# zsc/MOSS-TTSD

Hardware: AMD Instinct MI355X
Metric: audio codec tokens/sec/node (decode, bf16, batch 32 @ 4k ctx) (higher is better)
Workload: dtype bf16; 1 GPU; configs[2]: batch 32 synthetic dialogues/GPU, 4k-token KV context, top-k/top-p sampling on 8 channels, decode steps at full context; batch_per_gpu=32, context=4096, prompt=512, layers=28, hidden=2048, parallelism=dp1 (batch shard, no per-step collective)

## Files before the change

### include/mtts.h

```cpp
#ifndef MTTS_H
#define MTTS_H

#include <stdint.h>

#ifdef __cplusplus
extern "C" {
#endif

#define MTTS_OK 0
#define MTTS_EINVAL (-1)
#define MTTS_EHIP (-2)
#define MTTS_ENOMEM (-3)
#define MTTS_ESTATE (-4)

#define MTTS_CHANNELS 8

typedef struct MttsConfig {
    int32_t vocab_size;
    int32_t hidden_size;
    int32_t intermediate_size;
    int32_t num_hidden_layers;
    int32_t num_attention_heads;
    int32_t num_key_value_heads;
    int32_t head_dim;
// ... 17 lines not shown
typedef struct MttsSamplerCfg {
    int32_t do_sample;
    int32_t top_k;
    float top_p;
    float one_minus_top_p;
    float temperature;
    float repetition_penalty;
} MttsSamplerCfg;

typedef struct MttsEngine MttsEngine;

const char* mtts_last_error(void);
int32_t mtts_version(void);

int32_t mtts_engine_create(const MttsConfig* cfg, int32_t device, MttsEngine** out);
int32_t mtts_engine_destroy(MttsEngine* e);

int32_t mtts_bind_weight(MttsEngine* e, const char* name, const void* dev_bf16,
                         int64_t rows, int64_t cols, void* stream);
int32_t mtts_bind_weight_lora(MttsEngine* e, const char* name, const void* dev_base, int64_t rows, int64_t cols,
                              const float* dev_lora_a, const float* dev_lora_b, int32_t r, float scaling, void* stream);
#define MTTS_MAX_ADAPTERS 16
#define MTTS_LORA_MAX_RANK 64
int32_t mtts_adapter_load(MttsEngine* e, int32_t adapter, const char* name, const float* dev_lora_a, const float* dev_lora_b,
                          int64_t rows, int64_t cols, int32_t r, float scaling, void* stream);
int32_t mtts_adapter_clear(MttsEngine* e, int32_t adapter);
int32_t mtts_set_row_adapters(MttsEngine* e, const int32_t* host_ids, int32_t n);
int32_t mtts_set_slot_adapter(MttsEngine* e, int32_t slot, int32_t adapter);
int32_t mtts_bind_rope(MttsEngine* e, const void* dev_cos_bf16, const void* dev_sin_bf16,
                       int32_t rows, void* stream);
int32_t mtts_weights_ready(MttsEngine* e);

int32_t mtts_generate(MttsEngine* e, const int64_t* host_input_ids, const uint8_t* host_attention_mask,
                      int32_t B, int32_t T, int32_t max_length,
                      const MttsSamplerCfg* sampler, uint64_t seed,
                      int64_t* host_out_ids, int32_t out_capacity, int32_t* out_len,
                      const int64_t* host_forced, int32_t forced_len, int64_t* host_decisions,
                      void* stream);

int32_t mtts_begin(MttsEngine* e, const int64_t* host_input_ids, const uint8_t* host_attention_mask,
                   int32_t B, int32_t T, int32_t max_length,
                   const MttsSamplerCfg* sampler, uint64_t seed, void* stream);
int32_t mtts_step(MttsEngine* e, int32_t n_steps, void* stream);
int32_t mtts_sync_state(MttsEngine* e, int32_t* steps_done, int32_t* all_finished, void* stream);
int32_t mtts_read_generated(MttsEngine* e, int64_t* host_gen, int32_t capacity_steps, int32_t* n_steps);
int32_t mtts_set_output_scores(MttsEngine* e, int32_t on);
int32_t mtts_read_scores(MttsEngine* e, float* host_lp, int32_t capacity_steps, int32_t* n_steps);
int32_t mtts_slot_read_scores(MttsEngine* e, int32_t slot, float* host_rows, int32_t capacity_steps, int32_t* n_steps);
int32_t mtts_score(MttsEngine* e, const int64_t* host_input_ids, const uint8_t* host_attention_mask,
                   const int64_t* host_labels, int32_t B, int32_t T, float* host_logp, void* stream);
#define MTTS_SCORE_MAX_TOPK 16
#define MTTS_SCORE_TOPK_ROWS 512
int32_t mtts_score_topk(MttsEngine* e, const int64_t* host_input_ids, const uint8_t* host_attention_mask,
                        const int64_t* host_labels, int32_t B, int32_t T, float* host_logp, int32_t k,
                        int32_t* host_top_ids, float* host_top_logp, void* stream);
int32_t mtts_read_logits(MttsEngine* e, uint16_t* host_logits0, uint16_t* host_logits17, void* stream);
int32_t mtts_read_logits_f32(MttsEngine* e, float* host_logits0, float* host_logits17, void* stream);
int32_t mtts_sched_open(MttsEngine* e, int32_t B, int32_t gen_cap, const MttsSamplerCfg* sampler, void* stream);
int32_t mtts_slot_submit(MttsEngine* e, int32_t slot, const int64_t* host_ids, int32_t T, int32_t max_length, uint64_t seed,
                         void* stream);
int32_t mtts_slot_submit_row(MttsEngine* e, int32_t slot, const int64_t* host_ids, int32_t T, int32_t max_length, uint64_t seed,
                             int32_t row_id, void* stream);
int32_t mtts_set_row_ids(MttsEngine* e, const int32_t* host_row_ids, int32_t n);
int32_t mtts_set_takes(MttsEngine* e, int32_t n);
int32_t mtts_slot_fork(MttsEngine* e, int32_t src_slot, int32_t dst_slot, uint64_t seed, int32_t row_id, void* stream);
int32_t mtts_slot_states(MttsEngine* e, int32_t* host_state, void* stream);
int32_t mtts_slot_read(MttsEngine* e, int32_t slot, int64_t* host_rows, int32_t capacity_steps, int32_t* n_steps);
int32_t mtts_read_seq_state(MttsEngine* e, int32_t* host_nas, int32_t* host_unfinished, int32_t* host_kv_len, void* stream);
int32_t mtts_slot_evict(MttsEngine* e, int32_t slot, void* stream);
int32_t mtts_kv_pool_state(MttsEngine* e, int32_t* total_pages, int32_t* free_pages, int32_t* max_pages_per_seq);
int32_t mtts_read_page_table(MttsEngine* e, int32_t* host_table, int32_t* host_n_pages);
int32_t mtts_set_forced_mode(MttsEngine* e, int32_t as_draw);
int32_t mtts_debug_read_device_page_table(MttsEngine* e, int32_t* host_table, void* stream);
int32_t mtts_export_codes(MttsEngine* e, int32_t first, int32_t n, int64_t* dev_codes, void* stream);
int32_t mtts_profile_enable(MttsEngine* e, int32_t on);
int32_t mtts_profile_read(MttsEngine* e, int32_t which, double* total_ms, int64_t* launches, int64_t* bytes);

int32_t mtts_debug_set_kv_len(MttsEngine* e, int32_t kv_len);
int32_t mtts_debug_kv_pack_stats(MttsEngine* e, int64_t* out6);
int32_t mtts_k_attn_bench(MttsEngine* e, int32_t phase, int32_t iters, float* avg_ms, int64_t* bytes_per_launch);
int32_t mtts_k_gemm_bench(int32_t N, int32_t K, int32_t epi, int32_t ksplit, int32_t waves, int32_t copies,
                          int32_t iters, float* avg_us);

int32_t mtts_k_gemm_bf16(const void* dev_w, const void* dev_x, void* dev_y,
                         int32_t M, int32_t N, int32_t K, int32_t ksplit, void* stream);
int64_t mtts_debug_gemm_depth_launches(void);
int64_t mtts_debug_attn_row_launches(void);
int32_t mtts_k_attn_section(const float* dev_slabs, int32_t ksplit, const void* dev_qnw, const void* dev_knw, const void* dev_cos,
                            const void* dev_sin, float eps, const void* dev_k, const void* dev_v, const int32_t* host_lens,
                            const int32_t* host_page_table, int32_t R, int32_t Lmax, int32_t nq, int32_t nkv, int32_t sealed,
                            int32_t path, void* dev_out, void* dev_kcache, void* dev_vcache, void* dev_kpack, void* dev_vpack,
                            void* stream);
int32_t mtts_k_attn_prefill(const float* dev_slabs, int32_t ksplit, const void* dev_qnw, const void* dev_knw, const void* dev_cos,
                            const void* dev_sin, float eps, const void* dev_k, const void* dev_v, const int32_t* host_lens,
                            const int32_t* host_cached, const int32_t* host_page_table, int32_t B, int32_t Lmax, int32_t nq,
                            int32_t nkv, void* dev_out, void* dev_q, void* dev_kcache, void* dev_vcache, void* stream);
int32_t mtts_k_gemm_swiglu_bf16(const void* dev_w, const void* dev_x, void* dev_y,
                                int32_t M, int32_t N, int32_t K, void* stream);
int32_t mtts_k_rmsnorm(const void* dev_x, const void* dev_w, void* dev_y,
                       int32_t rows, int32_t n, float eps, void* stream);
int32_t mtts_k_embed_norm(const int32_t* host_tokens, const int32_t* host_seq, const void* const* host_tables,
                          const int32_t* host_vocab, const void* dev_norm_w, int32_t R, int32_t H, float eps,
                          void* dev_x, void* dev_xn, void* stream);
int32_t mtts_k_resid_norm(const float* dev_slabs, int32_t ksplit, int32_t Npad, void* dev_x, const void* dev_norm_w,
                          const int32_t* host_seq, const int32_t* host_last, int32_t R, int32_t H, int32_t nseq, float eps,
                          void* dev_xn, void* dev_hlast, void* stream);
int32_t mtts_k_gemv_small(int32_t epi, int32_t pro, const void* dev_w, int32_t rows, int32_t N, int32_t K, int32_t want_ksplit,
                          const void* dev_x_in, const float* dev_slabs, int32_t slab_ksplit, const void* dev_norm_w, float eps,
                          void* dev_x_out, const float* dev_opart, const int32_t* host_seq, const int32_t* host_pos, int32_t nq,
                          int32_t nchunks_max, const void* dev_xrows, void* dev_y, int32_t* out_plan, void* stream);
int32_t mtts_k_gemm_tile(int32_t epi, const void* dev_w, const void* dev_x, void* dev_y, int32_t M, int32_t N, int32_t K,
                         int32_t ksplit, void* stream);
int32_t mtts_k_rope_kvwrite(const void* dev_qkv, const int32_t* host_pos, const void* dev_qnorm, const void* dev_knorm,
                            const void* dev_cos, const void* dev_sin, int32_t R, int32_t nq, int32_t nkv, float eps,
                            void* dev_q, void* dev_k, void* dev_v, void* stream);
int32_t mtts_k_paged_attn_decode(const void* dev_q, const void* dev_k, const void* dev_v, const int32_t* host_lens,
                                 const int32_t* host_page_table, int32_t R, int32_t Lmax, int32_t nq, int32_t nkv,
                                 void* dev_out, void* stream);
int32_t mtts_k_kv_seal(const void* dev_pages, int32_t npages, void* dev_sealed, int32_t as_k, void* stream);
int32_t mtts_k_head_ce(const void* dev_w, const void* dev_x, const int32_t* host_labels, int32_t M, int32_t N, int32_t K,
                       int32_t n_valid, int32_t segments, float* dev_logp, void* stream);
int32_t mtts_k_head_topk(const void* dev_w, const void* dev_x, int32_t M, int32_t N, int32_t K, int32_t n_valid,
                         int32_t segments, int32_t k, int32_t* dev_ids, float* dev_logp, void* stream);
int32_t mtts_k_lora_pack(const void* dev_base, int32_t rows, int32_t cols, const float* dev_lora_a, const float* dev_lora_b,
                         int32_t r, float scaling, int32_t rows_pad, int32_t row_mul, int32_t row_off, int32_t dtype,
                         void* dev_out, void* stream);
int32_t mtts_k_lora_delta(const void* dev_x, int32_t R, int32_t K, int32_t Npad, int32_t nseg, const int32_t* host_segs,
                          int32_t n_adapters, const void* const* host_a, const void* const* host_b, const int32_t* host_r,
                          const float* host_scaling, const int32_t* host_row_adapter, float* dev_slabs, int32_t ks, void* stream);
int32_t mtts_k_swiglu_slabs(const void* dev_w, const void* dev_x, const float* dev_delta, void* dev_y, float* dev_slab0_out,
                            int32_t M, int32_t N, int32_t K, void* stream);
int32_t mtts_k_sample(const void* dev_logits_bf16, int32_t rows, int32_t vocab,
                      const void* dev_history_bitmap, const MttsSamplerCfg* cfg,
                      int32_t mask_id, uint64_t seed, int32_t step, int32_t channel,
                      int32_t* dev_tokens, void* stream);
int32_t mtts_k_sample_scores(const void* dev_logits_bf16, int32_t rows, int32_t vocab,
                             const void* dev_history_bitmap, const MttsSamplerCfg* cfg,
                             int32_t mask_id, uint64_t seed, int32_t step, int32_t channel,
                             int32_t* dev_tokens, float* dev_logp, void* stream);

typedef struct MttsCodecConfig {
    int32_t nq, codebook_size, rvq_dim, quant_out_dim;
    int32_t adapter_layers, adapter_dim, adapter_heads, adapter_ffn, adapter_max_pos;
    int32_t up_stride;
    int32_t dec_layers, dec_dim, dec_heads, dec_ffn, dec_max_pos, mel_bins;
    int32_t voc_dim, voc_inter, voc_layers, n_fft, hop;
    int32_t mel_n_fft, mel_hop, mel_frames;
    int32_t enc_layers, enc_dim, enc_heads, enc_ffn, enc_max_pos;
    int32_t sem_adapter_layers, pre_rvq_layers, down_pool;
} MttsCodecConfig;

typedef struct MttsCodec MttsCodec;
const char* mtts_codec_last_error(void);
int32_t mtts_codec_create(const MttsCodecConfig* cfg, int32_t device, MttsCodec** out);
int32_t mtts_codec_destroy(MttsCodec* c);
int32_t mtts_codec_bind(MttsCodec* c, const char* role, const float* dev_f32, int64_t n, void* stream);
int32_t mtts_codec_detokenize(MttsCodec* c, const int64_t* dev_codes, const int32_t* host_lens, int32_t B, int32_t T,
                              float* dev_wav, void* stream);
int32_t mtts_codec_detokenize_async(MttsCodec* c, const int64_t* dev_codes, const int32_t* host_lens, int32_t B, int32_t T,
                                    float* dev_wav, void* stream);
int32_t mtts_codec_check(MttsCodec* c, void* stream);
int32_t mtts_codec_tokenize(MttsCodec* c, const float* dev_wav, const int32_t* host_lens, int32_t B, int32_t nsamp,
                            int64_t* dev_codes, int32_t* host_code_lens, void* stream);
int32_t mtts_k_gemm_f32(const float* dev_a, const float* dev_w, const float* dev_bias, float* dev_c,
                        int32_t M, int32_t N, int32_t K, int32_t act, void* stream);
int32_t mtts_k_gemm_planes_bench(int32_t M, int32_t N, int32_t K, int32_t flags, int32_t tile_code, int32_t iters,
// ... 7 lines not shown
```

### moss-ttsd_amd/build.py

```python
import os
import subprocess
import sys
from concurrent.futures import ThreadPoolExecutor

HERE = os.path.dirname(os.path.abspath(__file__))
SRC = ["gemm.hip", "layer.hip", "attn.hip", "sampler.hip", "f32path.hip", "score.hip", "adapter.hip", "multilora.hip", "engine.hip", "hooks.hip", "codec.hip", "codec_fused.hip"]
OUT = os.path.join(HERE, "lib", "libmtts.so")
OBJ = os.path.join(HERE, "build")
FLAGS = ["--offload-arch=gfx950", "-O3", "-std=c++17", "-fPIC", "-fno-gpu-rdc", "-Wno-unused-result", "-Wno-unused-value"]
FLAGS += os.environ.get("MTTS_BUILD_FLAGS", "").split()


def _newer(target, deps):
    return os.path.exists(target) and all(os.path.getmtime(target) >= os.path.getmtime(d) for d in deps)


def build(force=False, verbose=True):
    srcs = [os.path.join(HERE, "csrc", s) for s in SRC if os.path.exists(os.path.join(HERE, "csrc", s))]
    hdrs = [os.path.join(HERE, "csrc", "common.h"), os.path.join(HERE, "..", "include", "mtts.h")]
    hdrs += [os.path.join(HERE, "csrc", h) for h in os.listdir(os.path.join(HERE, "csrc")) if h.endswith(".h") and h != "common.h"]
    if not force and _newer(OUT, srcs + hdrs):
        return OUT
    os.makedirs(os.path.dirname(OUT), exist_ok=True)
    os.makedirs(OBJ, exist_ok=True)
    objs, jobs = [], []
    for s in srcs:
        o = os.path.join(OBJ, os.path.basename(s) + ".o")
        objs.append(o)
        if force or not _newer(o, [s] + hdrs):
            jobs.append(["hipcc"] + FLAGS + ["-c", s, "-o", o])

    def run(cmd):
        if verbose:
            print(" ".join(cmd), flush=True)
        subprocess.check_call(cmd)

    with ThreadPoolExecutor(max_workers=min(6, max(1, len(jobs)))) as ex:
        list(ex.map(run, jobs))
    run(["hipcc", "--offload-arch=gfx950", "-shared", "-fPIC", "-fno-gpu-rdc", "-o", OUT] + objs)
    return OUT


if __name__ == "__main__":
    build(force="--force" in sys.argv)
```

### moss-ttsd_amd/csrc/attn.hip

```cpp
#include "launch.h"
#include <algorithm>
#include <atomic>
#include <cstdlib>
#ifndef MTTS_PK_WAVES
#define MTTS_PK_WAVES 0
#endif
#if MTTS_PK_WAVES
#define PK_OCC(PK) __attribute__((amdgpu_waves_per_eu((PK) ? MTTS_PK_WAVES : 1, (PK) ? MTTS_PK_WAVES : 8)))
#else
#define PK_OCC(PK)
#endif

__device__ __forceinline__ uint32_t u4c(const u32x4_t& v, int c) { return c == 0 ? v.x : c == 1 ? v.y : c == 2 ? v.z : v.w; }
__device__ __forceinline__ void pk_unit(const u32x4_t* pk, int j, uint32_t w[4]) {
    const uint32_t L0 = u4c(pk[j >> 1], 2 * (j & 1)), L1 = u4c(pk[j >> 1], 2 * (j & 1) + 1);
    const uint32_t N = u4c(pk[8 + (j >> 2)], j & 3);
    const uint32_t lo = pk[12].x, hi = pk[12].y;
    const uint32_t HA = ((N & 0x08080808u) << 4) | __builtin_amdgcn_perm(hi, lo, N & 0x07070707u);
    const uint32_t HB = (N & 0x80808080u) | __builtin_amdgcn_perm(hi, lo, (N >> 4) & 0x07070707u);
    w[0] = __builtin_amdgcn_perm(HA, L0, 0x05010400u);
    w[1] = __builtin_amdgcn_perm(HA, L0, 0x07030602u);
    w[2] = __builtin_amdgcn_perm(HB, L1, 0x05010400u);
    w[3] = __builtin_amdgcn_perm(HB, L1, 0x07030602u);
}

__host__ __device__ constexpr int pk_order(int i) { return i == 0 ? 12 : (i - 1) % 3 == 0 ? 8 + (i - 1) / 3 : 2 * ((i - 1) / 3) + (i - 1) % 3 - 1; }
__device__ bool seal_encode(const u32x4_t (&v)[16], u32x4_t* __restrict__ pk, uint32_t spare, bool unfit) {
    unsigned long long b0 = 0ull, b1 = 0ull;
#pragma unroll
    for (int j = 0; j < 16; ++j)
#pragma unroll
        for (int c = 0; c < 4; ++c)
#pragma unroll
            for (int h = 0; h < 2; ++h) {
                const uint32_t e = (u4c(v[j], c) >> (8 + 16 * h)) & 0x7fu;
                if (e & 64u) b1 |= 1ull << (e & 63u);
                else b0 |= 1ull << e;
            }
    const int n0 = __popcll(b0), n = n0 + __popcll(b1);
    if (n > 8 || unfit) {
        pk[12 * 64] = u32x4_t{0u, 0u, spare, 1u};
        return false;
    }
    unsigned long long dict = 0ull;
    {
        unsigned long long t0 = b0, t1 = b1;
        for (int i = 0; i < n; ++i) {
            uint32_t e;
            if (t0) { e = __ffsll((long long)t0) - 1; t0 &= t0 - 1; }
            else { e = 64 + __ffsll((long long)t1) - 1; t1 &= t1 - 1; }
            dict |= (unsigned long long)e << (8 * i);
        }
    }
    auto code = [&](uint32_t half) -> uint32_t {
        const uint32_t e = (half >> 8) & 0x7fu;
        const uint32_t rank = (e & 64u) ? n0 + __popcll(b1 & ((1ull << (e & 63u)) - 1ull)) : __popcll(b0 & ((1ull << e) - 1ull));
        return ((half >> 12) & 8u) | rank;
    };
    uint32_t lowp[32], nib[16];
#pragma unroll
    for (int j = 0; j < 16; ++j) {
        uint32_t N = 0u;
#pragma unroll
        for (int g = 0; g < 2; ++g) {
            uint32_t L = 0u;
#pragma unroll
            for (int k = 0; k < 4; ++k) {
                const uint32_t half = (u4c(v[j], 2 * g + (k >> 1)) >> (16 * (k & 1))) & 0xffffu;
                L |= (half & 0xffu) << (8 * k);
                N |= code(half) << (8 * k + 4 * g);
            }
            lowp[2 * j + g] = L;
        }
        nib[j] = N;
    }
#pragma unroll
    for (int u = 0; u < 8; ++u) pk[u * 64] = u32x4_t{lowp[4 * u], lowp[4 * u + 1], lowp[4 * u + 2], lowp[4 * u + 3]};
#pragma unroll
    for (int u = 0; u < 4; ++u) pk[(8 + u) * 64] = u32x4_t{nib[4 * u], nib[4 * u + 1], nib[4 * u + 2], nib[4 * u + 3]};
    pk[12 * 64] = u32x4_t{(uint32_t)dict, (uint32_t)(dict >> 32), spare, 0u};
    return true;
}
__device__ bool seal_lane(const u32x4_t* __restrict__ raw, u32x4_t* __restrict__ pk) {
    u32x4_t v[16];
#pragma unroll
    for (int j = 0; j < 16; ++j) v[j] = raw[j * 64];
    return seal_encode(v, pk, 0u, false);
}
__device__ bool seal_lane_k(const u32x4_t* __restrict__ raw, u32x4_t* __restrict__ pk, uint8_t* __restrict__ lds, int lane) {
    u32x4_t v[16];
#pragma unroll
    for (int j = 0; j < 16; ++j) v[j] = raw[j * 64];
    __builtin_amdgcn_wave_barrier();
    uint32_t* row = (uint32_t*)(lds + lane * 128);
#pragma unroll
    for (int j = 0; j < 16; ++j)
#pragma unroll
        for (int c = 0; c < 4; c += 2) {
            const uint32_t a = u4c(v[j], c), b = u4c(v[j], c + 1);
            row[2 * j + (c >> 1)] = ((a >> 7) & 0xffu) | (((a >> 23) & 0xffu) << 8) | (((b >> 7) & 0xffu) << 16) | (((b >> 23) & 0xffu) << 24);
        }
    __builtin_amdgcn_wave_barrier();
    uint32_t a0 = 0u, a1 = 0u, n0 = 0u, n1 = 0u;
    for (int t = 0; t < 64; ++t) {
        const uint32_t e = *(const uint16_t*)(lds + t * 128 + 2 * lane);
        a0 += e & 0xffu; n0 += (e & 0xffu) ? 1u : 0u;
        a1 += e >> 8; n1 += (e >> 8) ? 1u : 0u;
    }
    const int s0 = n0 ? min(max((int)((a0 + n0 / 2) / n0) - 125, -127), 127) : 0;
    const int s1 = n1 ? min(max((int)((a1 + n1 / 2) / n1) - 125, -127), 127) : 0;
    int8_t* sv = (int8_t*)(lds + 8192);
    sv[2 * lane] = (int8_t)s0;
    sv[2 * lane + 1] = (int8_t)s1;
    __builtin_amdgcn_wave_barrier();
    bool unfit = false;
#pragma unroll
    for (int j = 0; j < 16; ++j) {
        uint32_t w[4] = {v[j].x, v[j].y, v[j].z, v[j].w};
#pragma unroll
        for (int c = 0; c < 4; ++c) {
            const uint32_t sh = *(const uint16_t*)(sv + 8 * j + 2 * c);
            uint32_t out = 0u;
#pragma unroll
            for (int h = 0; h < 2; ++h) {
                uint32_t b = (w[c] >> (16 * h)) & 0xffffu;
                const int sft = (int)(int8_t)((sh >> (8 * h)) & 0xffu);
                const int e = (int)((b >> 7) & 0xffu);
                if (e == 0) {
                    if ((b & 0x7fu) && sft) unfit = true;
                } else {
                    const int e2 = e - sft;
                    if (e == 255 ? sft != 0 : (e2 < 1 || e2 > 254)) unfit = true;
                    else b = (b - ((uint32_t)sft << 7)) & 0xffffu;
                }
                out |= b << (16 * h);
            }
            w[c] = out;
        }
        v[j] = u32x4_t{w[0], w[1], w[2], w[3]};
    }
    return seal_encode(v, pk, ((uint32_t)s0 & 0xffu) | (((uint32_t)s1 & 0xffu) << 8), unfit);
}
__device__ bool seal_lane_v(const u32x4_t* __restrict__ raw, u32x4_t* __restrict__ pk, uint8_t* __restrict__ lds, int lane) {
    u32x4_t v[16];
#pragma unroll
    for (int j = 0; j < 16; ++j) v[j] = raw[j * 64];
    const int sub = lane >> 5;
    __builtin_amdgcn_wave_barrier();
    uint32_t* row = (uint32_t*)(lds + lane * 128);
#pragma unroll
    for (int it = 0; it < 16; ++it)
#pragma unroll
        for (int h = 0; h < 2; ++h) {
            uint32_t sum = 0u, cnt = 0u;
#pragma unroll
            for (int c = 0; c < 4; ++c) {
                const uint32_t e = (u4c(v[it], c) >> (7 + 16 * h)) & 0xffu;
                sum += e;
                cnt += e ? 1u : 0u;
            }
            row[2 * it + h] = sum | (cnt << 16);
        }
    __builtin_amdgcn_wave_barrier();
    int mean;
    {
        const int t = lane, st = (t >> 1) & 1, j = 2 * (t >> 2) + (t & 1);
        uint32_t tot = 0u, cn = 0u;
        for (int d = 0; d < 32; ++d) {
            const uint32_t w = ((const uint32_t*)(lds + (st * 32 + d) * 128))[j];
            tot += w & 0xffffu;
            cn += w >> 16;
// ... 1214 lines not shown
```

### moss-ttsd_amd/csrc/engine.h

```cpp
#pragma once
#include <hip/hip_runtime.h>

#include <algorithm>
#include <cstdarg>
#include <cstdio>
#include <cstdlib>
#include <cstring>
#include <memory>
#include <string>
#include <vector>

#include "launch.h"

#define MTTS_LOCAL __attribute__((visibility("hidden")))
extern MTTS_LOCAL thread_local char g_err[512];
#define HIPCHK(x)                                                                          \
    do {                                                                                   \
        hipError_t _e = (x);                                                               \
        if (_e != hipSuccess) return fail(MTTS_EHIP, "%s: %s (%s:%d)", #x, hipGetErrorString(_e), __FILE__, __LINE__); \
    } while (0)
#define TRY(x)             \
    do {                   \
        int _r = (x);      \
        if (_r) return _r; \
    } while (0)

static inline int round_up(int a, int b) { return (a + b - 1) / b * b; }
static inline hipStream_t S(void* s) { return (hipStream_t)s; }
static inline int gemm_depth_env() {
    const char* g = getenv("MTTS_GEMM_DEPTH");
    return (g && atoi(g) == 0) ? 0 : 1;
}

template <typename T>
static int dalloc(T** p, size_t n, bool zero = true) {
    HIPCHK(hipMalloc((void**)p, n * sizeof(T)));
    if (zero) HIPCHK(hipMemset(*p, 0, n * sizeof(T)));
    return 0;
}

struct DevBufs {
    struct Buf { void* p; bool pinned; };
    std::vector<Buf> bufs;
    std::string free_error;
    DevBufs() = default;
    DevBufs(const DevBufs&) = delete;
    DevBufs& operator=(const DevBufs&) = delete;
    ~DevBufs() { free_all(); }
    template <typename T>
    int get(T** out, size_t n, bool zero = true) {
        TRY(dalloc(out, n, zero));
        bufs.push_back({(void*)*out, false});
        return 0;
    }
    template <typename T>
    int get_pinned(T** out, size_t n) {
        HIPCHK(hipHostMalloc((void**)out, n * sizeof(T)));
        bufs.push_back({(void*)*out, true});
        memset((void*)*out, 0, n * sizeof(T));
        return 0;
    }
    template <typename T>
    void release(T*& p) {
        if (!p) return;
        auto it = std::find_if(bufs.begin(), bufs.end(), [&](const Buf& b) { return b.p == (void*)p; });
        if (it == bufs.end()) note(hipErrorInvalidValue, (void*)p);
        else { free_one(*it); bufs.erase(it); }
        p = nullptr;
    }
    void free_all() {
        for (const Buf& b : bufs) free_one(b);
        bufs.clear();
    }
private:
    void free_one(const Buf& b) {
        const hipError_t r = b.pinned ? hipHostFree(b.p) : hipFree(b.p);
        if (r != hipSuccess) note(r, b.p);
    }
    void note(hipError_t r, void* p) {
        if (!free_error.empty()) return;
        char msg[160];
        snprintf(msg, sizeof(msg), "freeing %p: %s", p, hipGetErrorString(r));
        free_error = msg;
    }
};

static inline int full_cap_for(int vocab) { int p = 1; while (p < vocab) p <<= 1; return vocab > SAMP_CAND ? p : 0; }
static inline int alloc_scratch(DevBufs& m, SampleScratch& sc, int rows, int vocab) {
    const int fc = full_cap_for(vocab);
    TRY(m.get(&sc.overflow, (size_t)rows));
    if (fc) {
        TRY(m.get(&sc.full_val, (size_t)rows * fc, false));
        TRY(m.get(&sc.full_idx, (size_t)rows * fc, false));
        TRY(m.get(&sc.nuc_cnt, (size_t)rows * 2048));
        TRY(m.get(&sc.nuc_mass, (size_t)rows * 2048));
    }
    TRY(m.get(&sc.hist, (size_t)rows * 2048));
    TRY(m.get(&sc.slice_val, (size_t)rows * SAMP_NS));
    TRY(m.get(&sc.slice_idx, (size_t)rows * SAMP_NS));
    TRY(m.get(&sc.cand_val, (size_t)rows * SAMP_CAND));
    TRY(m.get(&sc.cand_idx, (size_t)rows * SAMP_CAND));
    TRY(m.get(&sc.cand_n, (size_t)rows));
    return 0;
}
static inline int alloc_lp_scratch(DevBufs& m, SampleScratch& sc, int rows) {
    if (sc.lp) return 0;
    TRY(m.get(&sc.slice_sum, (size_t)rows * SAMP_NS));
    TRY(m.get(&sc.lp, (size_t)rows * 8));
    return 0;
}

struct Layer {
    void *wqkv = nullptr, *wo = nullptr, *wgu = nullptr, *wd = nullptr;
    void *ln_in = nullptr, *ln_post = nullptr, *qn = nullptr, *kn = nullptr;
    int bound = 0;
};

enum { PROF_SCORES = 0, PROF_PV = 1, PROF_GEMM = 2, PROF_STEP = 3,
       PROF_CE = 4,
       PROF_N = 5 };

struct MttsEngine {
    DevBufs mem;
    MttsConfig cfg;
    int device = 0;
    int H, I, L, nq, nkv, V0, Vs, Vs_pad, V0_pad, qkv_rows;
    std::vector<Layer> layers;
    void* emb[8] = {nullptr};
    void* head0 = nullptr;
    void* heads17 = nullptr;
    void* final_norm = nullptr;
    uint16_t *rope_cos = nullptr, *rope_sin = nullptr;
    int rope_rows = 0;
    int emb_bound = 0, norm_bound = 0;
    const uint16_t** d_tables = nullptr;
    GemmPlan p_qkv, p_o, p_gu, p_d, p_h0, p_h17;
    float* partial = nullptr;
    float* partial2 = nullptr;
    void *x2 = nullptr, *act_rm = nullptr;
    int small_rows = SMALL_RP;
    int gemm_depth = 1;
    void *x = nullptr, *xn = nullptr, *attn_p = nullptr, *act_p = nullptr, *qbuf = nullptr, *hlast = nullptr, *xh = nullptr;
    void *logits0 = nullptr, *logits17 = nullptr, *join_logits0 = nullptr, *join_logits17 = nullptr;
    void* scores = nullptr;
    float *stats = nullptr, *opart = nullptr;
    void *kcache = nullptr, *vcache = nullptr;
    size_t layer_stride = 0;
    int total_pages = 0, max_pages = 0, nchunks_max = 0;
    int32_t* d_page_table = nullptr;
    KvPool pool;
    std::vector<char> slot_live;
    int forced_draw = 0;
    std::vector<int32_t> next_row_ids;
    int next_takes = 1;
    int takes = 1;
    bool f32 = false;
    int h16 = 0;
    struct LayerF32 { float *wqkv = nullptr, *wo = nullptr, *wgu = nullptr, *wd = nullptr, *ln_in = nullptr, *ln_post = nullptr, *qn = nullptr, *kn = nullptr; };
    std::vector<LayerF32> lf;
    float* embf[8] = {nullptr};
    const float** d_tables_f = nullptr;
    float *final_norm_f = nullptr, *rope_cos_f = nullptr, *rope_sin_f = nullptr;
    float *kcache_f = nullptr, *vcache_f = nullptr;
    float *xf = nullptr, *xnf = nullptr, *qkvf = nullptr, *qbuf_f = nullptr, *attnf = nullptr, *yf = nullptr, *guf = nullptr,
          *actf = nullptr, *hlast_f = nullptr, *scores_f = nullptr;
    SeqState* d_seqs = nullptr;
    RowMeta* d_meta = nullptr;
    LoopState* d_ls = nullptr;
    LoopState* h_ls = nullptr;
    SeqState* h_seqs = nullptr;
    int32_t *d_decisions = nullptr, *d_cur = nullptr, *d_gen = nullptr, *d_declog = nullptr, *d_forced = nullptr,
            *d_tf = nullptr;
    uint32_t* d_bitmaps = nullptr;
    int bm_words = 0;
    MttsSamplerCfg* d_scfg = nullptr;
    SampleScratch sscr;
    int ch0_sampled = 0;
    float* d_lp = nullptr;
    int lp_cap = 0;
    int scores_next = 0;
    int scores_on = 0;
    bool run_open = false;
    int32_t* d_sc_labels = nullptr;
    float* d_sc_logp = nullptr;
    size_t sc_cap_rows = 0;
    float* sc_part = nullptr;
    float* sc_logits = nullptr;
    int32_t* d_sc_top_ids = nullptr;
    float* d_sc_top_logp = nullptr;
    size_t sc_top_cap = 0;
    uint32_t* sc_cand = nullptr;
    std::vector<LoraEnt> bank;
    LoraEnt* d_bank = nullptr;
    int bank_pairs[MTTS_MAX_ADAPTERS] = {0};
    int32_t* d_seq_adapter = nullptr;
    std::vector<int32_t> seq_adapter = std::vector<int32_t>(MTTS_RCAP, -1);
    std::vector<int32_t> next_slot_adapter = std::vector<int32_t>(MTTS_RCAP, -1);
    std::vector<int32_t> next_row_adapters;
    bool row_adapters_pending = false;
    int32_t* d_pf_tokens = nullptr;
    RowMeta* d_pf_meta = nullptr;
    size_t pf_cap_rows = 0;
    int gen_cap = 0;
    int B = 0, T = 0, base_length = 0, max_length = 0, max_steps = 0, steps_issued = 0;
    bool continuous = false;
    std::vector<int> join_step;
    std::vector<int> n_real;
    int max_real = 0;
    uint64_t seed = 0;
    bool began = false, has_forced = false;
    struct StepGraph { int B, pages, forced, ch0, scores, row, lora; hipGraphExec_t exec; };
    std::vector<StepGraph> graphs;
    hipStream_t cap_stream = nullptr;
    bool use_graphs = true;
    int kv_pack = 1;
    void *kpack = nullptr, *vpack = nullptr;
    size_t pk_layer_stride = 0;
    unsigned long long *d_seal_cnt = nullptr, *h_seal_cnt = nullptr;
    std::vector<char> pack_k_on, pack_v_on;
    int pack_min_work = 512;
    int fuse_qkv_max = 2560;
    int attn_row = 1;
    int n_cus = 0;
    int pf_mfma_pages = 0;
// ... 22 lines not shown
```

### moss-ttsd_amd/csrc/engine.hip

```cpp
#include "engine.h"
#include "staging.h"

#define FLUSH_STEPS 7
#define LINGER_STEPS 14
static inline int linger_bound(int B) { return 6 * B + 8; }

thread_local char g_err[512] = "";
int fail(int code, const char* fmt, ...) {
    va_list ap;
    va_start(ap, fmt);
    vsnprintf(g_err, sizeof(g_err), fmt, ap);
    va_end(ap);
    return code;
}

const char* mtts_last_error(void) { return g_err; }
int32_t mtts_version(void) { return 202; }

static auto ship_on(MttsEngine* e, hipStream_t st) {
    return [e, st](const PageEdits& ed) -> int {
        launch_set_pages(e->d_page_table, ed, st);
        HIPCHK(hipGetLastError());
        return 0;
    };
// ... 60 lines not shown

static void drop_graphs(MttsEngine* e) {
    for (auto& g : e->graphs) hipGraphExecDestroy(g.exec);
    e->graphs.clear();
}

int32_t mtts_engine_create(const MttsConfig* c, int32_t device, MttsEngine** out) {
    if (!c || !out) return fail(MTTS_EINVAL, "null argument");
    if (c->head_dim != MTTS_HD) return fail(MTTS_EINVAL, "head_dim must be 128 (got %d)", c->head_dim);
    if (c->channels != 8) return fail(MTTS_EINVAL, "channels must be 8");
    if (c->hidden_size % 16 || c->intermediate_size % 16) return fail(MTTS_EINVAL, "hidden/intermediate must be multiples of 16");
    if (c->hidden_size > 8192) return fail(MTTS_EINVAL, "hidden_size > 8192 not built (resid_norm keeps a row in registers)");
    if (c->num_attention_heads % c->num_key_value_heads) return fail(MTTS_EINVAL, "bad GQA ratio");
    int G = c->num_attention_heads / c->num_key_value_heads;
    if (G != 1 && G != 2 && G != 4) return fail(MTTS_EINVAL, "GQA group %d not built (1,2,4)", G);
    if (c->max_batch < 1 || c->max_batch > MTTS_RCAP) return fail(MTTS_EINVAL, "max_batch must be 1..128");
    if (c->vocab_size <= 152694 || c->speech_vocab_size <= 1024)
        return fail(MTTS_EINVAL, "vocab too small for the reference's hard-coded mask ids 152694 / 1024");
    if (c->dtype != MTTS_DTYPE_BF16 && c->dtype != MTTS_DTYPE_F32 && c->dtype != MTTS_DTYPE_F16)
        return fail(MTTS_EINVAL, "dtype %d not built (bf16 = 0, fp32 = 1, fp16 = 2)", c->dtype);
    if (c->kv_pool_pages < 0) return fail(MTTS_EINVAL, "kv_pool_pages must be >= 0");
    HIPCHK(hipSetDevice(device));
    struct Destroy {
        void operator()(MttsEngine* p) const {
            const std::string keep = g_err;
            mtts_engine_destroy(p);
            snprintf(g_err, sizeof(g_err), "%s", keep.c_str());
        }
    };
    std::unique_ptr<MttsEngine, Destroy> holder(new MttsEngine());
    MttsEngine* e = holder.get();
    DevBufs& m = e->mem;
    e->cfg = *c;
    e->device = device;
    if (const char* g = getenv("MTTS_GRAPHS")) e->use_graphs = atoi(g) != 0;
    if (const char* g = getenv("MTTS_FUSE_QKV_MAX")) e->fuse_qkv_max = atoi(g);
    if (const char* g = getenv("MTTS_KV_PACK")) e->kv_pack = atoi(g);
    if (const char* g = getenv("MTTS_KV_PACK_MIN")) e->pack_min_work = atoi(g);
    if (const char* g = getenv("MTTS_PREFILL_MFMA_PAGES")) e->pf_mfma_pages = atoi(g);
    if (const char* g = getenv("MTTS_ATTN_ROW")) e->attn_row = std::min(std::max(atoi(g), 0), 2);
    HIPCHK(hipDeviceGetAttribute(&e->n_cus, hipDeviceAttributeMultiprocessorCount, device));
    if (e->attn_row && attn_row_prepare()) {
        if (e->attn_row == 2) return fail(MTTS_EINVAL, "attn_row_kernel: the dynamic LDS limit could not be raised");
        e->attn_row = 0;
    }
    if (const char* g = getenv("MTTS_SMALL_ROWS")) e->small_rows = std::min(std::max(atoi(g), 0), SMALL_RP);
    e->gemm_depth = gemm_depth_env();
    e->H = c->hidden_size; e->I = c->intermediate_size; e->L = c->num_hidden_layers;
    e->nq = c->num_attention_heads; e->nkv = c->num_key_value_heads;
    e->V0 = c->vocab_size; e->Vs = c->speech_vocab_size;
    e->V0_pad = round_up(e->V0, 32); e->Vs_pad = round_up(e->Vs, 32);
    e->qkv_rows = (e->nq + 2 * e->nkv) * MTTS_HD;
    e->layers.resize(e->L);
    const int H = e->H, I = e->I;
    e->f32 = c->dtype != MTTS_DTYPE_BF16;
    e->h16 = c->dtype == MTTS_DTYPE_F16;
    if (e->f32) TRY(create_f32(e));
    if (!e->f32) {
        for (auto& l : e->layers) {
            TRY(m.get((uint16_t**)&l.wqkv, (size_t)e->qkv_rows * H));
            TRY(m.get((uint16_t**)&l.wo, (size_t)H * e->nq * MTTS_HD));
            TRY(m.get((uint16_t**)&l.wgu, (size_t)2 * I * H));
            TRY(m.get((uint16_t**)&l.wd, (size_t)round_up(H, 32) * I));
            TRY(m.get((uint16_t**)&l.ln_in, (size_t)H));
            TRY(m.get((uint16_t**)&l.ln_post, (size_t)H));
            TRY(m.get((uint16_t**)&l.qn, (size_t)MTTS_HD));
            TRY(m.get((uint16_t**)&l.kn, (size_t)MTTS_HD));
        }
        TRY(m.get((uint16_t**)&e->emb[0], (size_t)e->V0 * H, false));
        for (int ch = 1; ch < 8; ++ch) TRY(m.get((uint16_t**)&e->emb[ch], (size_t)e->Vs * H, false));
        TRY(m.get((uint16_t**)&e->head0, (size_t)e->V0_pad * H));
        TRY(m.get((uint16_t**)&e->heads17, (size_t)7 * e->Vs_pad * H));
        TRY(m.get((uint16_t**)&e->final_norm, (size_t)H));
        TRY(m.get(&e->d_tables, 8));
        HIPCHK(hipMemcpy((void*)e->d_tables, e->emb, 8 * sizeof(void*), hipMemcpyHostToDevice));
    }
    e->p_qkv = mtts_plan_gemm(e->qkv_rows, H, 0);
    e->p_o = mtts_plan_gemm(round_up(H, 32), e->nq * MTTS_HD, 0);
    e->p_gu = mtts_plan_gemm(2 * I, H, 1);
    e->p_d = mtts_plan_gemm(round_up(H, 32), I, 0);
    e->p_h0 = mtts_plan_gemm(e->V0_pad, H, 1);
    e->p_h17 = mtts_plan_gemm(7 * e->Vs_pad, H, 1);
    for (GemmPlan* p : {&e->p_qkv, &e->p_o, &e->p_gu, &e->p_d, &e->p_h0, &e->p_h17}) p->depth = e->gemm_depth;
    size_t pmax = (size_t)8 * std::max(e->qkv_rows, round_up(H, 32));
    if (!e->f32) {
        TRY(m.get(&e->partial, pmax * MTTS_PFCAP));
        TRY(m.get(&e->partial2, (size_t)8 * round_up(H, 32) * MTTS_PFCAP));
        TRY(m.get((uint16_t**)&e->x2, (size_t)MTTS_MAXR * H));
        TRY(m.get((uint16_t**)&e->act_rm, (size_t)MTTS_MAXR * I));
        TRY(m.get((uint16_t**)&e->x, (size_t)MTTS_PFCAP * H));
        TRY(m.get((uint16_t**)&e->xn, (size_t)MTTS_PFCAP * H));
        TRY(m.get((uint16_t**)&e->xh, (size_t)MTTS_RCAP * H));
        TRY(m.get((uint16_t**)&e->hlast, (size_t)MTTS_RCAP * H));
        TRY(m.get((uint16_t**)&e->attn_p, (size_t)MTTS_PFCAP * e->nq * MTTS_HD));
        TRY(m.get((uint16_t**)&e->act_p, (size_t)MTTS_PFCAP * I));
        TRY(m.get((uint16_t**)&e->qbuf, (size_t)MTTS_PFCAP * e->nq * MTTS_HD));
        TRY(m.get((uint16_t**)&e->logits0, (size_t)MTTS_RCAP * e->V0_pad));
        TRY(m.get((uint16_t**)&e->logits17, (size_t)MTTS_RCAP * 7 * e->Vs_pad));
        TRY(m.get((uint16_t**)&e->join_logits0, (size_t)MTTS_MAXR * e->V0_pad));
        TRY(m.get((uint16_t**)&e->join_logits17, (size_t)MTTS_MAXR * 7 * e->Vs_pad));
    }
    e->max_pages = pages_for(c->max_seq_len) + 1;
    e->total_pages = c->kv_pool_pages > 0 ? c->kv_pool_pages : e->max_pages * c->max_batch;
    e->nchunks_max = (e->max_pages + ATT_PB - 1) / ATT_PB;
    e->layer_stride = (size_t)e->total_pages * e->nkv * MTTS_PAGE * MTTS_HD;
    if (e->f32) {
        TRY(m.get(&e->kcache_f, e->layer_stride * e->L));
        TRY(m.get(&e->vcache_f, e->layer_stride * e->L));
        TRY(m.get(&e->scores_f, (size_t)MTTS_PF32CAP * e->nq * e->max_pages * MTTS_PAGE, false));
    } else {
        TRY(m.get((uint16_t**)&e->kcache, e->layer_stride * e->L));
        TRY(m.get((uint16_t**)&e->vcache, e->layer_stride * e->L));
        if (e->kv_pack) {
            e->pk_layer_stride = (size_t)e->total_pages * e->nkv * MTTS_PKU * 64 * 16;
            size_t free_b = 0, total_b = 0;
            const size_t need = 2 * e->pk_layer_stride * e->L;
            if (hipMemGetInfo(&free_b, &total_b) != hipSuccess || need + ((size_t)8 << 30) > free_b) {
                fprintf(stderr, "mtts: sealed KV pages off: %.1f GB needed, %.1f GB free (8 GB kept for the run)\n", need / 1e9, free_b / 1e9);
                e->kv_pack = 0;
            }
        }
        if (e->kv_pack) {
            TRY(m.get((uint8_t**)&e->kpack, e->pk_layer_stride * e->L));
            TRY(m.get((uint8_t**)&e->vpack, e->pk_layer_stride * e->L));
            TRY(m.get(&e->d_seal_cnt, (size_t)e->L * 4));
            TRY(m.get_pinned(&e->h_seal_cnt, (size_t)e->L * 4));
            e->pack_k_on.assign(e->L, 1);
            e->pack_v_on.assign(e->L, 1);
        }
    }
    TRY(m.get(&e->d_page_table, (size_t)c->max_batch * e->max_pages));
    e->slot_live.assign(c->max_batch, 0);
    const char* shuffle = getenv("MTTS_PAGE_SHUFFLE");
    const uint64_t shuffle_seed = shuffle ? (uint64_t)atoll(shuffle) : 0;
    e->pool.init(e->total_pages, e->max_pages, c->max_batch, c->max_seq_len, shuffle ? &shuffle_seed : nullptr);
    if (!e->f32) {
        TRY(m.get((uint16_t**)&e->scores, (size_t)MTTS_PFCAP * e->nq * e->max_pages * MTTS_PAGE));
        TRY(m.get(&e->stats, (size_t)MTTS_PFCAP * e->nq * e->max_pages * 2));
        TRY(m.get(&e->opart, (size_t)MTTS_PFCAP * e->nq * ((e->max_pages + ATT_PF - 1) / ATT_PF) * MTTS_HD));
    }
    TRY(m.get(&e->d_seqs, MTTS_RCAP));
    TRY(m.get(&e->d_meta, MTTS_RCAP));
    TRY(m.get(&e->d_ls, 1));
    TRY(m.get_pinned(&e->h_ls, 1));
    TRY(m.get_pinned(&e->h_seqs, MTTS_RCAP));
    TRY(m.get(&e->d_decisions, MTTS_RCAP * 8));
    TRY(m.get(&e->d_cur, MTTS_RCAP * 8));
    TRY(m.get(&e->d_tf, MTTS_RCAP * 7 * 8));
    e->bm_words = (e->V0 + 31) / 32;
    TRY(m.get(&e->d_bitmaps, (size_t)MTTS_RCAP * 8 * e->bm_words));
    TRY(m.get(&e->d_scfg, 8));
    TRY(alloc_scratch(m, e->sscr, c->max_batch, e->V0));
    *out = holder.release();
    return MTTS_OK;
}

int32_t mtts_engine_destroy(MttsEngine* e) {
    if (!e) return MTTS_OK;
    hipSetDevice(e->device);
    hipDeviceSynchronize();
    drop_graphs(e);
    if (e->cap_stream) hipStreamDestroy(e->cap_stream);
    for (int w = 0; w < PROF_N; ++w) for (auto& pr : e->ev[w]) { hipEventDestroy(pr.first); hipEventDestroy(pr.second); }
    e->mem.free_all();
    const std::string err = e->mem.free_error;
    delete e;
    return err.empty() ? MTTS_OK : fail(MTTS_EHIP, "mtts_engine_destroy: %s", err.c_str());
}

struct WeightSlot {
    int64_t rows = 0, cols = 0;
    void* copy_to = nullptr;
    void* pack_to = nullptr;
    int rows_pad = 0, row_mul = 1, row_off = 0;
    float* f32_to = nullptr;
    int64_t f32_row = 0;
    int* bound = nullptr;
    int bit = 0;
    bool proj = false;
    int layer = -1, proj_idx = -1;
};

static int resolve_weight(MttsEngine* e, const char* name_c, WeightSlot& w) {
    const std::string name(name_c);
    const int64_t H = e->H, I = e->I, D = MTTS_HD, Hp = round_up(e->H, 32), QD = e->nq * D, KD = e->nkv * D;
    int ch = -1;
    if (sscanf(name_c, "model.embedding_list.%d.weight", &ch) == 1 && name.size() > 7 && name.compare(name.size() - 7, 7, ".weight") == 0) {
        if (ch < 0 || ch > 7) return fail(MTTS_EINVAL, "bad channel in %s", name_c);
        w.rows = ch == 0 ? e->V0 : e->Vs; w.cols = H;
        w.copy_to = e->emb[ch]; w.f32_to = e->embf[ch];
        w.pack_to = ch == 0 ? e->head0 : e->heads17;
        w.rows_pad = ch == 0 ? e->V0_pad : 7 * e->Vs_pad;
        w.row_off = ch == 0 ? 0 : (ch - 1) * e->Vs_pad;
        w.bound = &e->emb_bound; w.bit = 1 << ch;
        return MTTS_OK;
    }
    if (name == "model.language_model.norm.weight") {
        w.rows = H; w.cols = 1; w.copy_to = e->final_norm; w.f32_to = e->final_norm_f; w.bound = &e->norm_bound; w.bit = 1;
        return MTTS_OK;
    }
    if (name.find("lm_heads.") == 0 || name == "model.language_model.embed_tokens.weight") return MTTS_OK;
    int n = -1;
    char rest[128];
    if (sscanf(name_c, "model.language_model.layers.%d.%127s", &n, rest) != 2) return fail(MTTS_EINVAL, "unknown tensor %s", name_c);
    if (n < 0 || n >= e->L) return fail(MTTS_EINVAL, "layer index out of range in %s", name_c);
    Layer& l = e->layers[n];
    const MttsEngine::LayerF32 f = e->f32 ? e->lf[n] : MttsEngine::LayerF32{};
    const struct { const char* name; int64_t rows, cols; void* bf; float* f32; int rows_pad, row_mul, row_off; int64_t f32_row; } t[] = {
        {"input_layernorm.weight", H, 1, l.ln_in, f.ln_in, 0, 1, 0, 0},
        {"post_attention_layernorm.weight", H, 1, l.ln_post, f.ln_post, 0, 1, 0, 0},
        {"self_attn.q_norm.weight", D, 1, l.qn, f.qn, 0, 1, 0, 0},
        {"self_attn.k_norm.weight", D, 1, l.kn, f.kn, 0, 1, 0, 0},
        {"self_attn.q_proj.weight", QD, H, l.wqkv, f.wqkv, e->qkv_rows, 1, 0, 0},
        {"self_attn.k_proj.weight", KD, H, l.wqkv, f.wqkv, e->qkv_rows, 1, (int)QD, QD},
        {"self_attn.v_proj.weight", KD, H, l.wqkv, f.wqkv, e->qkv_rows, 1, (int)(QD + KD), QD + KD},
        {"self_attn.o_proj.weight", H, QD, l.wo, f.wo, (int)Hp, 1, 0, 0},
        {"mlp.gate_proj.weight", I, H, l.wgu, f.wgu, (int)(2 * I), 2, 0, 0},
        {"mlp.up_proj.weight", I, H, l.wgu, f.wgu, (int)(2 * I), 2, 1, I},
        {"mlp.down_proj.weight", H, I, l.wd, f.wd, (int)Hp, 1, 0, 0},
    };
    for (int i = 0; i < 11; ++i)
        if (!strcmp(rest, t[i].name)) {
            w.rows = t[i].rows; w.cols = t[i].cols;
            (t[i].cols == 1 ? w.copy_to : w.pack_to) = t[i].bf;
            w.rows_pad = t[i].rows_pad; w.row_mul = t[i].row_mul; w.row_off = t[i].row_off;
            w.f32_to = t[i].f32; w.f32_row = t[i].f32_row;
            w.bound = &l.bound; w.bit = 1 << i;
            w.proj = t[i].cols != 1;
            w.layer = n; w.proj_idx = i - 4;
            return MTTS_OK;
        }
    return fail(MTTS_EINVAL, "unknown tensor %s", name_c);
}

int32_t mtts_bind_weight(MttsEngine* e, const char* name_c, const void* src, int64_t rows, int64_t cols, void* stream) {
    if (!e || !name_c || !src) return fail(MTTS_EINVAL, "null argument");
    HIPCHK(hipSetDevice(e->device));
    drop_graphs(e);
    hipStream_t st = S(stream);
    WeightSlot w;
    TRY(resolve_weight(e, name_c, w));
    if (!w.bound) return MTTS_OK;
    const bool shape_ok = w.cols == 1 ? (rows == w.rows && cols == 1) || (rows == 1 && cols == w.rows) : rows == w.rows && cols == w.cols;
    if (!shape_ok)
        return fail(MTTS_EINVAL, "%s: expected [%lld,%lld] got [%lld,%lld]", name_c, (long long)w.rows, (long long)w.cols, (long long)rows, (long long)cols);
    const size_t n = (size_t)w.rows * w.cols;
    if (e->f32) {
        HIPCHK(hipMemcpyAsync(w.f32_to + w.f32_row * w.cols, src, n * 4, hipMemcpyDeviceToDevice, st));
    } else {
        if (w.copy_to) HIPCHK(hipMemcpyAsync(w.copy_to, src, n * 2, hipMemcpyDeviceToDevice, st));
        if (w.pack_to) launch_pack_weight(src, w.pack_to, (int)w.rows, (int)w.cols, w.rows_pad, w.row_mul, w.row_off, st);
        HIPCHK(hipGetLastError());
    }
    *w.bound |= w.bit;
    return MTTS_OK;
}

static int run_still_open(MttsEngine* e, bool* open);
int32_t mtts_bind_weight_lora(MttsEngine* e, const char* name_c, const void* base, int64_t rows, int64_t cols, const float* lora_a,
                              const float* lora_b, int32_t r, float scaling, void* stream) {
    if (!e || !name_c || !base || !lora_a || !lora_b) return fail(MTTS_EINVAL, "null argument");
    if (r < 1 || r > 256) return fail(MTTS_EINVAL, "%s: adapter rank %d outside 1..256", name_c, r);
    if (((uintptr_t)base | (uintptr_t)lora_a | (uintptr_t)lora_b) & 15) return fail(MTTS_EINVAL, "%s: tensors must be 16-byte aligned", name_c);
    HIPCHK(hipSetDevice(e->device));
    WeightSlot w;
    TRY(resolve_weight(e, name_c, w));
    if (!w.proj) return fail(MTTS_EINVAL, "%s is not a projection weight of a layer: an adapter cannot target it", name_c);
    if (rows != w.rows || cols != w.cols)
        return fail(MTTS_EINVAL, "%s: expected [%lld,%lld] got [%lld,%lld]", name_c, (long long)w.rows, (long long)w.cols, (long long)rows, (long long)cols);
    bool open = false;
    TRY(run_still_open(e, &open));
    if (open) return fail(MTTS_ESTATE, "weights cannot change while a run is open (the rule of mtts_set_output_scores)");
    drop_graphs(e);
    hipStream_t st = S(stream);
    if (e->f32)
        launch_lora_rows_f32((const float*)base, lora_a, lora_b, r, scaling, w.f32_to + w.f32_row * w.cols, (int)w.rows, (int)w.cols,
                             e->h16 ? 1 : 0, st);
    else
        launch_lora_pack(base, lora_a, lora_b, r, scaling, w.pack_to, (int)w.rows, (int)w.cols, w.row_mul, w.row_off, st);
    HIPCHK(hipGetLastError());
    *w.bound |= w.bit;
    return MTTS_OK;
}

static size_t bank_partial_elems(const MttsEngine* e) {
    const size_t lin = std::max(e->qkv_rows, round_up(e->H, 32));
    return std::max(9 * lin, (size_t)4 * e->I) * MTTS_PFCAP;
}
static int bank_check(MttsEngine* e, int adapter, const char* what) {
    if (e->f32) return fail(MTTS_EINVAL, "%s: resident adapters exist on the bf16 engine only (this one is %s); merge one with mtts_bind_weight_lora", what, e->h16 ? "fp16" : "fp32");
    if (adapter < 0 || adapter >= MTTS_MAX_ADAPTERS) return fail(MTTS_EINVAL, "%s: adapter index %d outside 0..%d", what, adapter, MTTS_MAX_ADAPTERS - 1);
    bool open = false;
    TRY(run_still_open(e, &open));
    if (open) return fail(MTTS_ESTATE, "%s: the adapter bank cannot change while a run is open (the rule of mtts_bind_weight_lora)", what);
    return MTTS_OK;
}
static int adapter_id_check(MttsEngine* e, int id, const char* what, int at) {
    if (id == -1) return MTTS_OK;
    if (id < -1 || id >= MTTS_MAX_ADAPTERS) return fail(MTTS_EINVAL, "%s %d: adapter id %d outside -1..%d", what, at, id, MTTS_MAX_ADAPTERS - 1);
    if (!e->bank_pairs[id]) return fail(MTTS_EINVAL, "%s %d: adapter %d is empty (mtts_adapter_load)", what, at, id);
    return MTTS_OK;
}
static int bank_upload(MttsEngine* e, size_t first, size_t n, hipStream_t st) {
    HIPCHK(hipMemcpyAsync(e->d_bank + first, e->bank.data() + first, n * sizeof(LoraEnt), hipMemcpyHostToDevice, st));
    HIPCHK(hipStreamSynchronize(st));
    return MTTS_OK;
}

int32_t mtts_adapter_load(MttsEngine* e, int32_t adapter, const char* name_c, const float* lora_a, const float* lora_b, int64_t rows,
                          int64_t cols, int32_t r, float scaling, void* stream) {
    if (!e || !name_c || !lora_a || !lora_b) return fail(MTTS_EINVAL, "null argument");
    HIPCHK(hipSetDevice(e->device));
    TRY(bank_check(e, adapter, "mtts_adapter_load"));
    if (r < 1 || r > MTTS_LORA_MAX_RANK) return fail(MTTS_EINVAL, "%s: adapter rank %d outside 1..%d", name_c, r, MTTS_LORA_MAX_RANK);
    if (((uintptr_t)lora_a | (uintptr_t)lora_b) & 15) return fail(MTTS_EINVAL, "%s: tensors must be 16-byte aligned", name_c);
    WeightSlot w;
    TRY(resolve_weight(e, name_c, w));
    if (!w.proj) return fail(MTTS_EINVAL, "%s is not a projection weight of a layer: an adapter cannot target it", name_c);
    if (rows != w.rows || cols != w.cols)
        return fail(MTTS_EINVAL, "%s: expected [%lld,%lld] got [%lld,%lld]", name_c, (long long)w.rows, (long long)w.cols, (long long)rows, (long long)cols);
    if (cols > LORA_MAX_K) return fail(MTTS_EINVAL, "%s: rows of %lld elements, the delta kernel stages at most %d", name_c, (long long)cols, LORA_MAX_K);
    drop_graphs(e);
    hipStream_t st = S(stream);
    const size_t per = (size_t)e->L * 7;
    if (!e->d_bank) {
        HIPCHK(hipDeviceSynchronize());
        float* wider = nullptr;
        int32_t* ids = nullptr;
        LoraEnt* tab = nullptr;
        int rc = e->mem.get(&wider, bank_partial_elems(e));
        if (!rc) rc = e->mem.get(&ids, MTTS_RCAP, false);
        if (!rc) rc = e->mem.get(&tab, MTTS_MAX_ADAPTERS * per);
        if (!rc && hipMemset(ids, 0xff, MTTS_RCAP * sizeof(int32_t)) != hipSuccess) rc = fail(MTTS_EHIP, "mtts_adapter_load: hipMemset of the per-slot adapter ids failed");
        if (rc) { e->mem.release(wider); e->mem.release(ids); e->mem.release(tab); return rc; }
        e->mem.release(e->partial);
        e->partial = wider;
        e->d_seq_adapter = ids;
        e->bank.assign(MTTS_MAX_ADAPTERS * per, LoraEnt{nullptr, nullptr, 0, 0.f});
        e->d_bank = tab;
    }
    float *a = nullptr, *b = nullptr;
    TRY(e->mem.get(&a, (size_t)r * cols, false));
    if (const int rc = e->mem.get(&b, (size_t)rows * r, false)) { e->mem.release(a); return rc; }
    if (hipMemcpyAsync(a, lora_a, (size_t)r * cols * 4, hipMemcpyDeviceToDevice, st) != hipSuccess ||
        hipMemcpyAsync(b, lora_b, (size_t)rows * r * 4, hipMemcpyDeviceToDevice, st) != hipSuccess) {
        e->mem.release(a); e->mem.release(b);
        return fail(MTTS_EHIP, "%s: copying the adapter matrices failed", name_c);
    }
    const size_t at = adapter * per + (size_t)w.layer * 7 + w.proj_idx;
    LoraEnt& ent = e->bank[at];
    if (ent.r) {
        HIPCHK(hipDeviceSynchronize());
        float *oa = const_cast<float*>(ent.A), *ob = const_cast<float*>(ent.B);
        e->mem.release(oa); e->mem.release(ob);
    } else e->bank_pairs[adapter]++;
    ent = LoraEnt{a, b, r, scaling};
    return bank_upload(e, at, 1, st);
}

int32_t mtts_adapter_clear(MttsEngine* e, int32_t adapter) {
    if (!e) return fail(MTTS_EINVAL, "null engine");
    HIPCHK(hipSetDevice(e->device));
    TRY(bank_check(e, adapter, "mtts_adapter_clear"));
    drop_graphs(e);
    if (!e->d_bank || !e->bank_pairs[adapter]) return MTTS_OK;
    HIPCHK(hipDeviceSynchronize());
    const size_t per = (size_t)e->L * 7;
    for (size_t i = adapter * per; i < (adapter + 1) * per; ++i) {
        float *oa = const_cast<float*>(e->bank[i].A), *ob = const_cast<float*>(e->bank[i].B);
        e->mem.release(oa); e->mem.release(ob);
        e->bank[i] = LoraEnt{nullptr, nullptr, 0, 0.f};
    }
    e->bank_pairs[adapter] = 0;
    return bank_upload(e, adapter * per, per, nullptr);
}

int32_t mtts_set_row_adapters(MttsEngine* e, const int32_t* host_ids, int32_t n) {
    if (!e || (n > 0 && !host_ids) || n < 0 || n > MTTS_RCAP) return fail(MTTS_EINVAL, "set_row_adapters: bad argument");
    if (e->f32) return fail(MTTS_EINVAL, "mtts_set_row_adapters: resident adapters exist on the bf16 engine only (this one is %s)", e->h16 ? "fp16" : "fp32");
    e->next_row_adapters.assign(host_ids, host_ids + n);
    e->row_adapters_pending = n > 0;
    return MTTS_OK;
}

int32_t mtts_set_slot_adapter(MttsEngine* e, int32_t slot, int32_t adapter) {
    if (!e) return fail(MTTS_EINVAL, "null engine");
    if (e->f32) return fail(MTTS_EINVAL, "mtts_set_slot_adapter: resident adapters exist on the bf16 engine only (this one is %s)", e->h16 ? "fp16" : "fp32");
    if (slot < 0 || slot >= MTTS_RCAP) return fail(MTTS_EINVAL, "set_slot_adapter: slot %d out of range", slot);
    if (adapter < -1 || adapter >= MTTS_MAX_ADAPTERS) return fail(MTTS_EINVAL, "set_slot_adapter: adapter id %d outside -1..%d", adapter, MTTS_MAX_ADAPTERS - 1);
    e->next_slot_adapter[slot] = adapter;
    return MTTS_OK;
}
static int set_seq_adapter(MttsEngine* e, int slot, int id, hipStream_t st) {
    e->seq_adapter[slot] = id;
    if (e->d_seq_adapter) HIPCHK(hipMemcpyAsync(e->d_seq_adapter + slot, &e->seq_adapter[slot], sizeof(int32_t), hipMemcpyHostToDevice, st));
    return MTTS_OK;
}
static std::vector<int32_t> take_row_adapters(MttsEngine* e) {
    std::vector<int32_t> v;
    v.swap(e->next_row_adapters);
    e->row_adapters_pending = false;
    return v;
}
static bool rows_carry_adapters(const MttsEngine* e) {
    for (int b = 0; b < e->B; ++b)
        if (e->seq_adapter[b] >= 0) return true;
    return false;
}

template <typename T>
static int bind_rope_tables(MttsEngine* e, T*& c, T*& s, const void* cosb, const void* sinb, int rows, hipStream_t st) {
    e->mem.release(c);
    e->mem.release(s);
    TRY(e->mem.get(&c, (size_t)rows * 64, false));
    TRY(e->mem.get(&s, (size_t)rows * 64, false));
    HIPCHK(hipMemcpyAsync(c, cosb, (size_t)rows * 64 * sizeof(T), hipMemcpyDeviceToDevice, st));
    HIPCHK(hipMemcpyAsync(s, sinb, (size_t)rows * 64 * sizeof(T), hipMemcpyDeviceToDevice, st));
    e->rope_rows = rows;
    return MTTS_OK;
}
int32_t mtts_bind_rope(MttsEngine* e, const void* cosb, const void* sinb, int32_t rows, void* stream) {
    if (!e || !cosb || !sinb || rows < 1) return fail(MTTS_EINVAL, "bad rope table");
    HIPCHK(hipSetDevice(e->device));
    drop_graphs(e);
    if (e->f32) return bind_rope_tables(e, e->rope_cos_f, e->rope_sin_f, cosb, sinb, rows, S(stream));
    return bind_rope_tables(e, e->rope_cos, e->rope_sin, cosb, sinb, rows, S(stream));
}

int32_t mtts_weights_ready(MttsEngine* e) {
    if (!e) return fail(MTTS_EINVAL, "null engine");
    if (e->emb_bound != 0xff) return fail(MTTS_ESTATE, "embedding tables missing (mask %x)", e->emb_bound);
    if (!e->norm_bound) return fail(MTTS_ESTATE, "final norm missing");
    if (!e->rope_rows) return fail(MTTS_ESTATE, "rope table missing");
    for (int n = 0; n < e->L; ++n)
        if (e->layers[n].bound != 2047) return fail(MTTS_ESTATE, "layer %d incomplete (mask %x)", n, e->layers[n].bound);
    return MTTS_OK;
}

static void prof_begin(MttsEngine* e, int which, hipStream_t st, hipEvent_t* a) {
    if (!e->prof) return;
    hipEvent_t s0, s1;
    hipEventCreate(&s0); hipEventCreate(&s1);
    hipEventRecord(s0, st);
    e->ev[which].push_back({s0, s1});
    *a = s1;
}
static void prof_end(MttsEngine* e, hipStream_t st, hipEvent_t a) {
    if (!e->prof) return;
    hipEventRecord(a, st);
}

static int pack_policy_reset(MttsEngine* e, hipStream_t st) {
    if (!e->d_seal_cnt) return 0;
    HIPCHK(hipMemsetAsync(e->d_seal_cnt, 0, (size_t)e->L * 4 * sizeof(unsigned long long), st));
    bool changed = false;
    for (int n = 0; n < e->L; ++n) { changed |= !e->pack_k_on[n] || !e->pack_v_on[n]; e->pack_k_on[n] = 1; e->pack_v_on[n] = 1; }
    if (changed) drop_graphs(e);
    return 0;
}
static int attend_layer(MttsEngine* e, int n, const RowMeta* d_meta, int R, int pages_bound, int ks_qkv, int nphases, bool prefill,
                        bool fused, bool sealed, hipStream_t st, int64_t kv_tokens_hint) {
    static const AttnPhase decode_ph[3] = {ATTN_SCORES, ATTN_PV, ATTN_COMBINE}, prefill_ph[3] = {ATTN_PF_SCORES, ATTN_PF_PV, ATTN_PF_COMBINE};
    Layer& l = e->layers[n];
    const float eps = e->cfg.rms_norm_eps, scale = 1.0f / sqrtf((float)MTTS_HD);
    uint16_t* kc = (uint16_t*)e->kcache + e->layer_stride * n;
    uint16_t* vc = (uint16_t*)e->vcache + e->layer_stride * n;
    const QkvFuse fz{e->partial, ks_qkv, e->qkv_rows, (const uint16_t*)l.qn, (const uint16_t*)l.kn, e->rope_cos, e->rope_sin, eps};
    const KvPack pk = layer_pack(e, n, pages_bound);
    const KvPack* pkp = (sealed && (pk.k || pk.v)) ? &pk : nullptr;
    if (!prefill && sealed && nphases == 3 && attn_row_shape(e, pages_bound) && attn_row_fits(e->nq / e->nkv, &fz, pkp, pages_bound)) {
        hipEvent_t ev = nullptr;
        prof_begin(e, PROF_SCORES, st, &ev);
        if (const int rc = launch_attn(e->qbuf, kc, vc, e->d_page_table, d_meta, e->scores, e->stats, e->opart, e->attn_p, R, pages_bound,
                                       e->max_pages, e->total_pages, e->nchunks_max, e->nq, e->nkv, scale, &fz, ATTN_ROW, st, pkp))
            return fail(MTTS_EINVAL, rc == -2 ? "the whole-row attention kernel does not take this launch" : "attention group size not built");
        prof_end(e, st, ev);
        if (e->prof) e->prof_bytes[PROF_SCORES] += 2 * kv_tokens_hint * e->nkv * MTTS_HD * 2;
        return 0;
    }
    if (!fused)
        launch_qkv_post(e->partial, ks_qkv, e->qkv_rows, d_meta, l.qn, l.kn, e->rope_cos, e->rope_sin, e->qbuf,
                        kc, vc, e->d_page_table, e->max_pages, e->total_pages, R, e->nq, e->nkv, eps, st);
    for (int i = 0; i < nphases; ++i) {
        hipEvent_t ev = nullptr;
        if (i < 2) prof_begin(e, i == 0 ? PROF_SCORES : PROF_PV, st, &ev);
        if (launch_attn(e->qbuf, kc, vc, e->d_page_table, d_meta, e->scores, e->stats, e->opart, e->attn_p, R,
                        pages_bound, e->max_pages, e->total_pages, e->nchunks_max, e->nq, e->nkv, scale,
                        fused ? &fz : nullptr, (prefill ? prefill_ph : decode_ph)[i], st, pkp))
            return fail(MTTS_EINVAL, "attention group size not built");
        if (i < 2) prof_end(e, st, ev);
    }
    if (e->prof) {
        e->prof_bytes[PROF_SCORES] += kv_tokens_hint * e->nkv * MTTS_HD * 2;
        e->prof_bytes[PROF_PV] += kv_tokens_hint * e->nkv * MTTS_HD * 2;
    }
    return 0;
}
static bool small_path_fits(MttsEngine* e) {
    const int H = e->H;
    if (H > 8192 || H % 8 || e->I % 8) return false;
    const int lim = 64 * 1024 - 33 * 1024;
    return mtts_small_lds_bytes(e->p_qkv, H, PRO_NORM) <= lim && mtts_small_lds_bytes(e->p_d, e->I, PRO_ROWS) <= lim &&
           mtts_small_lds_bytes(e->p_o, e->nq * MTTS_HD, PRO_COMBINE) <= lim;
}
static int forward_small(MttsEngine* e, const RowMeta* d_meta, int pages_bound, hipStream_t st, int64_t kv_tokens_hint) {
    const int H = e->H, I = e->I, nq = e->nq, nkv = e->nkv, Hp = round_up(H, 32), R = MTTS_MAXR;
    const float eps = e->cfg.rms_norm_eps;
    uint16_t* xa = (uint16_t*)e->x;
    uint16_t* xb = (uint16_t*)e->x2;
    SmallPro base{};
    base.rows = e->B; base.eps = eps; base.slab_npad = Hp;
    for (int n = 0; n < e->L; ++n) {
        Layer& l = e->layers[n];
        SmallPro pq = base;
        pq.x_in = xa; pq.x_out = xb; pq.slabs = e->partial2; pq.ksplit = n ? e->p_d.ksplit : 0; pq.norm_w = (const uint16_t*)l.ln_in;
        launch_gemv_small(EPI_PARTIAL, PRO_NORM, e->p_qkv, l.wqkv, H, e->qkv_rows, e->qkv_rows, e->partial, nullptr, pq, st);
        TRY(attend_layer(e, n, d_meta, R, pages_bound, e->p_qkv.ksplit, 2, false, e->B * pages_bound <= e->fuse_qkv_max, true, st,
                         kv_tokens_hint));
        SmallPro po = base;
        po.opart = e->opart; po.meta = d_meta; po.nchunks_max = e->nchunks_max; po.nq = nq; po.pages_per_chunk = ATT_PB;
        launch_gemv_small(EPI_PARTIAL, PRO_COMBINE, e->p_o, l.wo, nq * MTTS_HD, Hp, Hp, e->partial2, nullptr, po, st);
        SmallPro pg = base;
        pg.x_in = xb; pg.x_out = xa; pg.slabs = e->partial2; pg.ksplit = e->p_o.ksplit; pg.norm_w = (const uint16_t*)l.ln_post;
        launch_gemv_small(EPI_SILU_RM, PRO_NORM, e->p_gu, l.wgu, H, 2 * I, 2 * I, nullptr, (uint16_t*)e->act_rm, pg, st);
        SmallPro pd = base;
        pd.xrows = (const uint16_t*)e->act_rm;
        launch_gemv_small(EPI_PARTIAL, PRO_ROWS, e->p_d, l.wd, I, Hp, Hp, e->partial2, nullptr, pd, st);
    }
    if (e->kpack)
        launch_kv_seal_rows(e->kcache, e->vcache, e->kpack, e->vpack, e->d_page_table, d_meta, R, e->max_pages, e->total_pages, nkv, e->L, e->d_seal_cnt, st);
    SmallPro ph = base;
    ph.x_in = xa; ph.x_out = nullptr; ph.slabs = e->partial2; ph.ksplit = e->p_d.ksplit; ph.norm_w = (const uint16_t*)e->final_norm;
    launch_gemv_small(EPI_BF16, PRO_NORM, e->p_h0, e->head0, H, e->V0_pad, e->V0, nullptr, (uint16_t*)e->logits0, ph, st);
    launch_gemv_small(EPI_BF16, PRO_NORM, e->p_h17, e->heads17, H, 7 * e->Vs_pad, 7 * e->Vs_pad, nullptr, (uint16_t*)e->logits17, ph, st);
    HIPCHK(hipGetLastError());
    return MTTS_OK;
}

static int forward_rows(MttsEngine* e, const int32_t* d_tokens, const RowMeta* d_meta, int R, int pages_bound,
                        int heads, bool lora, hipStream_t st, int64_t kv_tokens_hint) {
    const int H = e->H, I = e->I, nq = e->nq, nkv = e->nkv;
    const float eps = e->cfg.rms_norm_eps;
    const int Hp = round_up(H, 32);
    const int mb = (R + 31) / 32;
    const bool tiled = heads != 1;
    if (e->f32) return forward_rows_f32(e, d_tokens, d_meta, heads == 1 ? e->B : R, heads, st);
    launch_embed_norm(d_tokens, d_meta, e->d_tables, e->layers[0].ln_in, e->x, e->xn, R, H, eps, st);
    if (heads == 1 && !lora && e->B <= e->small_rows && small_path_fits(e)) return forward_small(e, d_meta, pages_bound, st, kv_tokens_hint);
    if (lora && !e->d_bank) return fail(MTTS_ESTATE, "a pass with adapters on an engine without a bank");
    const int QD = nq * MTTS_HD, KD = nkv * MTTS_HD, EL = e->L * 7;
    const LoraJob j_qkv{3, e->qkv_rows, H, EL, {{0, QD, 1, 0}, {QD, KD, 1, 1}, {QD + KD, KD, 1, 2}}};
    const LoraJob j_o{1, Hp, QD, EL, {{0, H, 1, 3}}}, j_gu{2, 2 * I, H, EL, {{0, I, 2, 4}, {1, I, 2, 5}}}, j_d{1, Hp, I, EL, {{0, H, 1, 6}}};
    for (int n = 0; n < e->L; ++n) {
        Layer& l = e->layers[n];
        auto delta = [&](const LoraJob& job, const void* xp, int ks) {
            launch_lora_delta(xp, d_meta, e->d_seq_adapter, e->d_bank + (size_t)n * 7, job, e->partial + (size_t)ks * MTTS_PFCAP * job.Npad, R, st);
        };
        const int ex = lora ? 1 : 0;
        const int ks_qkv = tiled ? mtts_tile_ksplit(e->qkv_rows, H, 1024) : e->p_qkv.ksplit;
        const int ks_o = tiled ? mtts_tile_ksplit(Hp, nq * MTTS_HD, 1024) : e->p_o.ksplit;
        const int ks_d = tiled ? mtts_tile_ksplit(Hp, I, 1024) : e->p_d.ksplit;
        if (tiled) launch_gemm_tile(EPI_PARTIAL, R, ks_qkv, l.wqkv, e->xn, H, e->qkv_rows, e->qkv_rows, e->partial, nullptr, st);
        else launch_gemm(EPI_PARTIAL, mb, e->p_qkv, l.wqkv, e->xn, H, e->qkv_rows, e->qkv_rows, e->partial, nullptr, st);
        if (lora) delta(j_qkv, e->xn, ks_qkv);
        TRY(attend_layer(e, n, d_meta, R, pages_bound, ks_qkv + ex, 3, heads != 1 && pages_bound >= e->pf_mfma_pages,
                         heads == 1 && e->B * pages_bound <= e->fuse_qkv_max, heads == 1, st, kv_tokens_hint));
        if (tiled) launch_gemm_tile(EPI_PARTIAL, R, ks_o, l.wo, e->attn_p, nq * MTTS_HD, Hp, Hp, e->partial, nullptr, st);
        else launch_gemm(EPI_PARTIAL, mb, e->p_o, l.wo, e->attn_p, nq * MTTS_HD, Hp, Hp, e->partial, nullptr, st);
        if (lora) delta(j_o, e->attn_p, ks_o);
        launch_resid_norm(e->partial, ks_o + ex, Hp, e->x, l.ln_post, e->xn, nullptr, d_meta, R, H, eps, st);
        const int gu_epi = lora ? EPI_PARTIAL : EPI_SILU;
        float* gu_slab = lora ? e->partial : nullptr;
        if (tiled) launch_gemm_tile(gu_epi, R, 1, l.wgu, e->xn, H, 2 * I, 2 * I, gu_slab, (uint16_t*)e->act_p, st);
        else launch_gemm(gu_epi, mb, e->p_gu, l.wgu, e->xn, H, 2 * I, 2 * I, gu_slab, (uint16_t*)e->act_p, st);
        if (lora) {
            delta(j_gu, e->xn, 1);
            launch_swiglu_slabs(e->partial, e->partial + (size_t)MTTS_PFCAP * 2 * I, e->act_p, mb * 32, I, st);
        }
        if (tiled) launch_gemm_tile(EPI_PARTIAL, R, ks_d, l.wd, e->act_p, I, Hp, Hp, e->partial, nullptr, st);
        else launch_gemm(EPI_PARTIAL, mb, e->p_d, l.wd, e->act_p, I, Hp, Hp, e->partial, nullptr, st);
        if (lora) delta(j_d, e->act_p, ks_d);
        const bool lastl = (n == e->L - 1);
        const void* nw = lastl ? e->final_norm : e->layers[n + 1].ln_in;
        launch_resid_norm(e->partial, ks_d + ex, Hp, e->x, nw, e->xn, lastl ? e->hlast : nullptr, d_meta, R, H, eps, st);
    }
    if (e->kpack)
        launch_kv_seal_rows(e->kcache, e->vcache, e->kpack, e->vpack, e->d_page_table, d_meta, R, e->max_pages, e->total_pages, nkv, e->L, e->d_seal_cnt, st);
    if (heads) {
        const void* xin = e->xn;
        int hmb = mb;
        if (heads == 2) {
            hmb = (e->B + 31) / 32;
            launch_pack_rows(e->hlast, e->xh, e->B, H, hmb, st);
            xin = e->xh;
        }
        launch_gemm(EPI_BF16, hmb, e->p_h0, e->head0, xin, H, e->V0_pad, e->V0, nullptr, (uint16_t*)e->logits0, st);
        launch_gemm(EPI_BF16, hmb, e->p_h17, e->heads17, xin, H, 7 * e->Vs_pad, 7 * e->Vs_pad, nullptr, (uint16_t*)e->logits17, st);
    }
    HIPCHK(hipGetLastError());
    return MTTS_OK;
}

static int prefill_staged(MttsEngine* e, size_t Mpad, int pages_bound, int last_heads, bool lora, hipStream_t st) {
    const size_t pfcap = e->f32 ? MTTS_PF32CAP : MTTS_PFCAP;
    for (size_t off = 0; off < Mpad; off += pfcap) {
        const int rows = (int)std::min<size_t>(pfcap, Mpad - off);
        TRY(forward_rows(e, e->d_pf_tokens + off * 8, e->d_pf_meta + off, rows, pages_bound, off + rows >= Mpad ? last_heads : 0, lora, st, 0));
    }
    return 0;
}

static int ensure_gen_storage(MttsEngine* e, int steps) {
    if (steps <= e->gen_cap) return 0;
    e->mem.release(e->d_gen); e->mem.release(e->d_declog); e->mem.release(e->d_forced);
    drop_graphs(e);
    e->gen_cap = steps;
    const size_t n = (size_t)e->cfg.max_batch * steps * 8;
    TRY(e->mem.get(&e->d_gen, n));
    TRY(e->mem.get(&e->d_declog, n));
    TRY(e->mem.get(&e->d_forced, n, false));
    return 0;
}

static int start_scores(MttsEngine* e, hipStream_t st) {
    e->scores_on = e->scores_next;
    if (!e->scores_on) return 0;
    if (!e->sscr.lp) {
        drop_graphs(e);
        TRY(alloc_lp_scratch(e->mem, e->sscr, e->cfg.max_batch));
    }
    const size_t n = (size_t)e->cfg.max_batch * e->gen_cap * 8;
    if (!e->d_lp || e->lp_cap != e->gen_cap) {
        e->mem.release(e->d_lp);
        drop_graphs(e);
        TRY(e->mem.get(&e->d_lp, n, false));
        e->lp_cap = e->gen_cap;
    }
    HIPCHK(hipMemsetAsync(e->d_lp, 0xff, n * sizeof(float), st));
    return 0;
}

static int upload_staged(MttsEngine* e, const StagedRows& sr, bool on_stream, hipStream_t st) {
    if (sr.Mpad > e->pf_cap_rows) {
        e->mem.release(e->d_pf_tokens); e->mem.release(e->d_pf_meta);
        e->pf_cap_rows = 0;
        TRY(e->mem.get(&e->d_pf_tokens, sr.Mpad * 8, false));
        TRY(e->mem.get(&e->d_pf_meta, sr.Mpad, false));
        e->pf_cap_rows = sr.Mpad;
    }
    const size_t tb = sr.Mpad * 8 * 4, mb = sr.Mpad * sizeof(RowMeta);
    if (on_stream) {
        HIPCHK(hipMemcpyAsync(e->d_pf_tokens, sr.toks.data(), tb, hipMemcpyHostToDevice, st));
        HIPCHK(hipMemcpyAsync(e->d_pf_meta, sr.metas.data(), mb, hipMemcpyHostToDevice, st));
    } else {
        HIPCHK(hipMemcpy(e->d_pf_tokens, sr.toks.data(), tb, hipMemcpyHostToDevice));
        HIPCHK(hipMemcpy(e->d_pf_meta, sr.metas.data(), mb, hipMemcpyHostToDevice));
    }
    return 0;
}

static const SeqState IDLE_SEQ{-1, 0, 0, 0, 0, 0, 0, 0, 0};
static int reset_run_state(MttsEngine* e, const std::vector<SeqState>& seqs, bool continuous, const MttsSamplerCfg* sampler, hipStream_t st) {
    HIPCHK(hipMemcpyAsync(e->d_seqs, seqs.data(), seqs.size() * sizeof(SeqState), hipMemcpyHostToDevice, st));
    if (continuous) e->forced_draw = 0;
    LoopState ls{0, 0, continuous ? 1 : 0, e->B, 0, e->gen_cap, e->forced_draw, e->f32 ? 1 : 0};
    e->continuous = continuous;
    e->join_step.assign(MTTS_RCAP, 0);
    HIPCHK(hipMemcpyAsync(e->d_ls, &ls, sizeof(ls), hipMemcpyHostToDevice, st));
    *e->h_ls = ls;
    std::vector<RowMeta> dm(MTTS_RCAP, RowMeta{-1, 0, 0, 0});
    HIPCHK(hipMemcpyAsync(e->d_meta, dm.data(), dm.size() * sizeof(RowMeta), hipMemcpyHostToDevice, st));
    HIPCHK(hipMemcpyAsync(e->d_scfg, sampler, 8 * sizeof(MttsSamplerCfg), hipMemcpyHostToDevice, st));
    e->ch0_sampled = sampler[0].do_sample ? 1 : 0;
    HIPCHK(hipMemsetAsync(e->sscr.hist, 0, (size_t)e->cfg.max_batch * 2048 * 4, st));
    HIPCHK(hipMemsetAsync(e->sscr.cand_n, 0, (size_t)e->cfg.max_batch * 4, st));
    HIPCHK(hipMemsetAsync(e->sscr.overflow, 0, (size_t)e->cfg.max_batch * 4, st));
    HIPCHK(hipStreamSynchronize(st));
    return 0;
}

// ... 829 lines not shown
```

### moss-ttsd_amd/csrc/gemm.hip

```cpp
#include "launch.h"


template <int WAVES, int EPI, int MB>
__global__ __launch_bounds__(WAVES * 64) void gemm_skinny_kernel(
    const u32x4_t* __restrict__ Wp, const u32x4_t* __restrict__ Xp, int KT, int kt_per_split,
    int kt_per_wave, float* __restrict__ partial, uint16_t* __restrict__ out, int Npad, int n_valid) {
    __shared__ float red[WAVES][16][64];
    const int nt = blockIdx.x, ks = blockIdx.y;
    const int wave = threadIdx.x >> 6, lane = threadIdx.x & 63;
    int kt0 = ks * kt_per_split + wave * kt_per_wave;
    int kt1 = min(min(kt0 + kt_per_wave, (ks + 1) * kt_per_split), KT);
    f32x16_t acc[MB];
#pragma unroll
    for (int mb = 0; mb < MB; ++mb)
#pragma unroll
        for (int i = 0; i < 16; ++i) acc[mb][i] = 0.f;
    const u32x4_t* wp = Wp + ((size_t)nt * KT + kt0) * 64 + lane;
    const u32x4_t* xp = Xp + (size_t)kt0 * 64 + lane;
    const size_t xtile = (size_t)KT * 64;
    constexpr int U = (MB == 1) ? 8 : 4;
    int n = kt1 - kt0;
    int i = 0;
    for (; i + U <= n; i += U) {
        u32x4_t a[U], b[U][MB];
#pragma unroll
        for (int u = 0; u < U; ++u) a[u] = __builtin_nontemporal_load(wp + (size_t)(i + u) * 64);
#pragma unroll
        for (int u = 0; u < U; ++u)
#pragma unroll
            for (int mb = 0; mb < MB; ++mb) b[u][mb] = xp[(size_t)(i + u) * 64 + mb * xtile];
#pragma unroll
        for (int u = 0; u < U; ++u)
#pragma unroll
            for (int mb = 0; mb < MB; ++mb)
                acc[mb] = __builtin_amdgcn_mfma_f32_32x32x16_bf16(*(bf16x8_t*)&a[u], *(bf16x8_t*)&b[u][mb], acc[mb], 0, 0, 0);
    }
    for (; i < n; ++i) {
        u32x4_t a = __builtin_nontemporal_load(wp + (size_t)i * 64);
#pragma unroll
        for (int mb = 0; mb < MB; ++mb) {
            u32x4_t b = xp[(size_t)i * 64 + mb * xtile];
            acc[mb] = __builtin_amdgcn_mfma_f32_32x32x16_bf16(*(bf16x8_t*)&a, *(bf16x8_t*)&b, acc[mb], 0, 0, 0);
        }
    }
    const int l2 = threadIdx.x & 63;
#pragma unroll
    for (int mb = 0; mb < MB; ++mb) {
        if (mb) __syncthreads();
#pragma unroll
        for (int r = 0; r < 16; ++r) red[wave][r][lane] = acc[mb][r];
        __syncthreads();
        for (int q = threadIdx.x >> 6; q < 4; q += WAVES) {
            float v[4];
#pragma unroll
            for (int j = 0; j < 4; ++j) {
                float s = red[0][4 * q + j][l2];
#pragma unroll
                for (int w = 1; w < WAVES; ++w) s += red[w][4 * q + j][l2];
                v[j] = s;
            }
            const int row = mb * 32 + (l2 & 31);
            const int nl = 8 * q + 4 * (l2 >> 5);
            const int n0 = nt * 32 + nl;
            if (EPI == EPI_PARTIAL) {
                float4 o = make_float4(v[0], v[1], v[2], v[3]);
                *(float4*)(partial + ((size_t)ks * MTTS_PFCAP + row) * Npad + n0) = o;
            } else if (EPI == EPI_BF16) {
                uint16_t* o = out + (size_t)row * Npad + n0;
                if (n0 + 3 < n_valid) *(u32x2_t*)o = u32x2_t{pack2(v[0], v[1]), pack2(v[2], v[3])};
                else {
#pragma unroll
                    for (int j = 0; j < 4; ++j)
                        if (n0 + j < n_valid) o[j] = f2bf(v[j]);
                }
            } else {
#pragma unroll
                for (int j = 0; j < 2; ++j) {
                    float g = rbf(v[2 * j]), u = rbf(v[2 * j + 1]);
                    float a = rbf(g / (1.0f + expf(-g)));
                    int idx = (n0 >> 1) + j;
                    out[xpack_off(row, idx, Npad >> 1)] = f2bf(a * u);
                }
            }
        }
    }
}

template <int EPI>
__device__ __forceinline__ void skinny_store(const float (&v)[4], int row, int n0, int ks, float* __restrict__ partial,
                                             uint16_t* __restrict__ out, int Npad, int n_valid) {
    if (EPI == EPI_PARTIAL) {
        *(float4*)(partial + ((size_t)ks * MTTS_PFCAP + row) * Npad + n0) = make_float4(v[0], v[1], v[2], v[3]);
    } else if (EPI == EPI_BF16) {
        uint16_t* o = out + (size_t)row * Npad + n0;
        if (n0 + 3 < n_valid) *(u32x2_t*)o = u32x2_t{pack2(v[0], v[1]), pack2(v[2], v[3])};
        else {
#pragma unroll
            for (int j = 0; j < 4; ++j)
                if (n0 + j < n_valid) o[j] = f2bf(v[j]);
        }
    } else {
#pragma unroll
        for (int j = 0; j < 2; ++j) {
            float g = rbf(v[2 * j]), u = rbf(v[2 * j + 1]);
            float a = rbf(g / (1.0f + expf(-g)));
            out[xpack_off(row, (n0 >> 1) + j, Npad >> 1)] = f2bf(a * u);
        }
    }
}

template <int WAVES, int KTW, int EPI>
__global__ __launch_bounds__(WAVES * 64) void gemm_depth_kernel(
    const u32x4_t* __restrict__ Wp, const u32x4_t* __restrict__ Xp, int KT, float* __restrict__ partial,
    uint16_t* __restrict__ out, int Npad, int n_valid) {
    __shared__ float red[WAVES][16][64];
    const int nt = blockIdx.x, ks = blockIdx.y;
    const int wave = threadIdx.x >> 6, lane = threadIdx.x & 63;
    const int kt0 = (ks * WAVES + wave) * KTW;
    const u32x4_t* wp = Wp + ((size_t)nt * KT + kt0) * 64 + lane;
    const u32x4_t* xp = Xp + (size_t)kt0 * 64 + lane;
    u32x4_t a[KTW], b[KTW];
#pragma unroll
    for (int u = 0; u < KTW; ++u) b[u] = xp[(size_t)u * 64];
    __builtin_amdgcn_sched_barrier(0);
#pragma unroll
    for (int u = 0; u < KTW; ++u) {
        a[u] = __builtin_nontemporal_load(wp + (size_t)u * 64);
        __builtin_amdgcn_sched_barrier(0);
    }
    f32x16_t acc;
#pragma unroll
    for (int i = 0; i < 16; ++i) acc[i] = 0.f;
#pragma unroll
    for (int u = 0; u < KTW; ++u)
        acc = __builtin_amdgcn_mfma_f32_32x32x16_bf16(*(bf16x8_t*)&a[u], *(bf16x8_t*)&b[u], acc, 0, 0, 0);
#pragma unroll
    for (int r = 0; r < 16; ++r) red[wave][r][lane] = acc[r];
    __syncthreads();
    for (int q = wave; q < 4; q += WAVES) {
        float v[4];
#pragma unroll
        for (int j = 0; j < 4; ++j) {
            float s = red[0][4 * q + j][lane];
#pragma unroll
            for (int w = 1; w < WAVES; ++w) s += red[w][4 * q + j][lane];
            v[j] = s;
        }
        skinny_store<EPI>(v, lane & 31, nt * 32 + 8 * q + 4 * (lane >> 5), ks, partial, out, Npad, n_valid);
    }
}

template <int WAVES, int KTW>
__global__ __launch_bounds__(WAVES * 64) void gemm_gateup48_kernel(
    const u32x4_t* __restrict__ Wp, const u32x4_t* __restrict__ Xp, int KT, uint16_t* __restrict__ out, int Npad) {
    __shared__ float red[WAVES][24][64];
    const int p = blockIdx.x >> 1, o = blockIdx.x & 1;
    const int tf = 3 * p + 2 * o, th = 3 * p + 1;
    const int wave = threadIdx.x >> 6, lane = threadIdx.x & 63;
    const int kt0 = wave * KTW;
    const int hl = (((lane >> 4) & 1) == o) ? lane : (lane ^ 16);
    const u32x4_t* wp = Wp + ((size_t)tf * KT + kt0) * 64 + lane;
    const u32x4_t* hp = Wp + ((size_t)th * KT + kt0) * 64 + hl;
    const u32x4_t* xp = Xp + (size_t)kt0 * 64 + lane;
    u32x4_t a[KTW], h[KTW], b[KTW];
#pragma unroll
    for (int u = 0; u < KTW; ++u) b[u] = xp[(size_t)u * 64];
    __builtin_amdgcn_sched_barrier(0);
#pragma unroll
    for (int u = 0; u < KTW; ++u) {
        a[u] = __builtin_nontemporal_load(wp + (size_t)u * 64);
        h[u] = __builtin_nontemporal_load(hp + (size_t)u * 64);
        __builtin_amdgcn_sched_barrier(0);
    }
    f32x16_t acc, acch;
#pragma unroll
    for (int i = 0; i < 16; ++i) acc[i] = acch[i] = 0.f;
#pragma unroll
    for (int u = 0; u < KTW; ++u) {
        acc = __builtin_amdgcn_mfma_f32_32x32x16_bf16(*(bf16x8_t*)&a[u], *(bf16x8_t*)&b[u], acc, 0, 0, 0);
        acch = __builtin_amdgcn_mfma_f32_32x32x16_bf16(*(bf16x8_t*)&h[u], *(bf16x8_t*)&b[u], acch, 0, 0, 0);
    }
#pragma unroll
    for (int r = 0; r < 16; ++r) red[wave][r][lane] = acc[r];
#pragma unroll
    for (int r = 0; r < 8; ++r) red[wave][16 + r][lane] = o ? acch[8 + r] : acch[r];
    __syncthreads();
    for (int q6 = wave; q6 < 6; q6 += WAVES) {
        float v[4];
#pragma unroll
// ... 273 lines not shown
        size_t t = g >> 6;
        int kt = (int)(t % KT);
        int nt = (int)(t / KT);
        int p = nt * 32 + (lane & 31) - row_off;
        int k = kt * 16 + 8 * (lane >> 5);
        if (p < 0 || (p % row_mul) != 0) continue;
        int srow = p / row_mul;
        if (srow >= rows) continue;
        *(u32x4_t*)(dst + g * 8) = *(const u32x4_t*)(src + (size_t)srow * cols + k);
    }
}

__global__ void pack_rows_kernel(const uint16_t* __restrict__ src, uint16_t* __restrict__ dst, int R, int K, int tiles) {
    int per_tile = (K >> 4) * 64;
    int total = per_tile * tiles;
    for (int g = blockIdx.x * blockDim.x + threadIdx.x; g < total; g += gridDim.x * blockDim.x) {
        int tile = g / per_tile, gi = g % per_tile;
        int lane = gi & 63, kt = gi >> 6;
        int r = tile * 32 + (lane & 31), k = kt * 16 + 8 * (lane >> 5);
        u32x4_t v = {0u, 0u, 0u, 0u};
        if (r < R) v = *(const u32x4_t*)(src + (size_t)r * K + k);
        *(u32x4_t*)(dst + (size_t)g * 8) = v;
    }
}

__global__ void reduce_partial_bf16_kernel(const float* __restrict__ partial, uint16_t* __restrict__ out,
                                           int ksplit, int Npad, int n_valid, int R) {
    int idx = blockIdx.x * blockDim.x + threadIdx.x;
    if (idx >= R * n_valid) return;
    int r = idx / n_valid, n = idx % n_valid;
    float s = 0.f;
    for (int k = 0; k < ksplit; ++k) s += partial[((size_t)k * MTTS_PFCAP + r) * Npad + n];
    out[idx] = f2bf(s);
}

static GemmPlan plan_gemm(int Npad, int K, int want_ksplit) {
    GemmPlan p;
    int KT = K / 16, ntiles = Npad / 32;
    int ks = want_ksplit;
    if (ks <= 0) {
        ks = 1;
        while (ntiles * ks < 256 && ks < 8 && KT / (ks * 2) >= 16) ks *= 2;
    }
    p.ksplit = ks;
    p.kt_per_split = (KT + ks - 1) / ks;
    int w = 8;
    while (w > 1 && p.kt_per_split / w < 4) w >>= 1;
    p.waves = w;
    p.kt_per_wave = (p.kt_per_split + w - 1) / w;
    p.depth = 1;
    return p;
}

template <int EPI, int MB>
static void launch_gemm_epi(const GemmPlan& p, const void* Wp, const void* Xp, int K, int Npad, int n_valid,
                            float* partial, uint16_t* out, hipStream_t st) {
    dim3 grid(Npad / 32, p.ksplit);
    int KT = K / 16;
#define MTTS_GEMM_CASE(WV)                                                                            \
    case WV:                                                                                          \
        hipLaunchKernelGGL((gemm_skinny_kernel<WV, EPI, MB>), grid, dim3(WV * 64), 0, st,             \
                           (const u32x4_t*)Wp, (const u32x4_t*)Xp, KT, p.kt_per_split, p.kt_per_wave, \
                           partial, out, Npad, n_valid);                                              \
        break;
    switch (p.waves) {
        MTTS_GEMM_CASE(8)
        MTTS_GEMM_CASE(4)
        MTTS_GEMM_CASE(2)
        MTTS_GEMM_CASE(1)
    }
#undef MTTS_GEMM_CASE
}

template <int EPI>
static void launch_gemm_mb(int mb, const GemmPlan& p, const void* Wp, const void* Xp, int K, int Npad, int n_valid,
                           float* partial, uint16_t* out, hipStream_t st) {
    if (mb <= 1) launch_gemm_epi<EPI, 1>(p, Wp, Xp, K, Npad, n_valid, partial, out, st);
    else if (mb == 2) launch_gemm_epi<EPI, 2>(p, Wp, Xp, K, Npad, n_valid, partial, out, st);
    else launch_gemm_epi<EPI, 4>(p, Wp, Xp, K, Npad, n_valid, partial, out, st);
}

static long long g_depth_launches = 0;
long long mtts_gemm_depth_launches() { return g_depth_launches; }
static bool launch_gemm_depth(int epi, int mb, const GemmPlan& p, const void* Wp, const void* Xp, int K, int Npad,
                              int n_valid, float* partial, uint16_t* out, hipStream_t st) {
    const int KT = K / 16;
    if (!p.depth || mb > 1 || p.waves != 8 || K % 16 || KT != p.ksplit * 8 * p.kt_per_wave || p.kt_per_split != 8 * p.kt_per_wave)
        return false;
    if (epi == EPI_PARTIAL) {
        dim3 grid(Npad / 32, p.ksplit);
#define MTTS_DEPTH_CASE(KTW)                                                                                        \
    case KTW:                                                                                                       \
        hipLaunchKernelGGL((gemm_depth_kernel<8, KTW, EPI_PARTIAL>), grid, dim3(512), 0, st, (const u32x4_t*)Wp,    \
                           (const u32x4_t*)Xp, KT, partial, out, Npad, n_valid);                                    \
        ++g_depth_launches;                                                                                         \
        return true;
        switch (p.kt_per_wave) {
            MTTS_DEPTH_CASE(4)
            MTTS_DEPTH_CASE(12)
        }
#undef MTTS_DEPTH_CASE
        return false;
    }
    if (epi == EPI_SILU && p.ksplit == 1 && p.kt_per_wave == 16 && Npad % 96 == 0 && n_valid == Npad) {
        hipLaunchKernelGGL((gemm_gateup48_kernel<8, 16>), dim3(Npad / 48), dim3(512), 0, st, (const u32x4_t*)Wp,
                           (const u32x4_t*)Xp, KT, out, Npad);
        ++g_depth_launches;
        return true;
    }
    return false;
}

void launch_gemm(int epi, int mb, const GemmPlan& p, const void* Wp, const void* Xp, int K, int Npad, int n_valid,
                 float* partial, uint16_t* out, hipStream_t st) {
    if (launch_gemm_depth(epi, mb, p, Wp, Xp, K, Npad, n_valid, partial, out, st)) return;
    if (epi == EPI_PARTIAL) launch_gemm_mb<EPI_PARTIAL>(mb, p, Wp, Xp, K, Npad, n_valid, partial, out, st);
    else if (epi == EPI_BF16) launch_gemm_mb<EPI_BF16>(mb, p, Wp, Xp, K, Npad, n_valid, partial, out, st);
    else launch_gemm_mb<EPI_SILU>(mb, p, Wp, Xp, K, Npad, n_valid, partial, out, st);
}


int mtts_small_lds_bytes(const GemmPlan& p, int K, int pro) {
    const int kts = pro == PRO_NORM ? K / 16 : p.kt_per_split;
    return kts * 2 * SMALL_RP * 16;
}
template <int EPI, int PRO>
static void launch_small_epi(const GemmPlan& p0, const void* Wp, int K, int Npad, int n_valid, float* partial, uint16_t* out,
                             const SmallPro& pr, hipStream_t st) {
    GemmPlan p = p0;
    if (p.waves < 4) { p.waves = 4; p.kt_per_wave = (p.kt_per_split + 3) / 4; }
    dim3 grid(Npad / 32, p.ksplit);
    const int KT = K / 16;
    const size_t lds = (size_t)mtts_small_lds_bytes(p, K, PRO);
    if (p.waves == 8)
        hipLaunchKernelGGL((gemv_small_kernel<8, EPI, PRO>), grid, dim3(512), lds, st, (const u32x4_t*)Wp, KT, p.kt_per_split,
                           p.kt_per_wave, partial, out, Npad, n_valid, pr);
    else
        hipLaunchKernelGGL((gemv_small_kernel<4, EPI, PRO>), grid, dim3(256), lds, st, (const u32x4_t*)Wp, KT, p.kt_per_split,
                           p.kt_per_wave, partial, out, Npad, n_valid, pr);
}
void launch_gemv_small(int epi, int pro, const GemmPlan& p, const void* Wp, int K, int Npad, int n_valid, float* partial,
                       uint16_t* out, const SmallPro& pr, hipStream_t st) {
    if (epi == EPI_PARTIAL && pro == PRO_NORM) launch_small_epi<EPI_PARTIAL, PRO_NORM>(p, Wp, K, Npad, n_valid, partial, out, pr, st);
    else if (epi == EPI_PARTIAL && pro == PRO_COMBINE) launch_small_epi<EPI_PARTIAL, PRO_COMBINE>(p, Wp, K, Npad, n_valid, partial, out, pr, st);
    else if (epi == EPI_PARTIAL && pro == PRO_ROWS) launch_small_epi<EPI_PARTIAL, PRO_ROWS>(p, Wp, K, Npad, n_valid, partial, out, pr, st);
    else if (epi == EPI_SILU_RM && pro == PRO_NORM) launch_small_epi<EPI_SILU_RM, PRO_NORM>(p, Wp, K, Npad, n_valid, partial, out, pr, st);
    else if (epi == EPI_BF16 && pro == PRO_NORM) launch_small_epi<EPI_BF16, PRO_NORM>(p, Wp, K, Npad, n_valid, partial, out, pr, st);
}

int mtts_tile_ksplit(int Npad, int K, int R) {
    int blocks = ((Npad + 127) / 128) * ((R + 127) / 128), ks = 1;
    while (blocks * ks < 512 && ks < 8 && (K / 16) / (ks * 2) >= 16) ks *= 2;
    return ks;
}
void launch_gemm_tile(int epi, int R, int ksplit, const void* Wp, const void* Xp, int K, int Npad, int n_valid,
                      float* partial, uint16_t* out, hipStream_t st) {
    const int KT = K / 16, ntiles = Npad / 32, rtiles = (R + 31) / 32;
    const int kps = (KT + ksplit - 1) / ksplit;
    dim3 grid((ntiles + 3) / 4, (rtiles + 3) / 4, ksplit);
#define MTTS_TILE_CASE(E)                                                                                     \
    hipLaunchKernelGGL((gemm_tile_kernel<E>), grid, dim3(256), 0, st, (const u32x4_t*)Wp, (const u32x4_t*)Xp, \
                       KT, kps, ntiles, rtiles, partial, out, Npad, n_valid)
    if (epi == EPI_PARTIAL) MTTS_TILE_CASE(EPI_PARTIAL);
    else if (epi == EPI_BF16) MTTS_TILE_CASE(EPI_BF16);
    else MTTS_TILE_CASE(EPI_SILU);
#undef MTTS_TILE_CASE
// ... 32 lines not shown
```

### moss-ttsd_amd/csrc/hooks.hip

```cpp
#include "engine.h"

int32_t mtts_k_gemm_bf16(const void* w, const void* x, void* y, int32_t M, int32_t N, int32_t K, int32_t ksplit, void* stream) {
    if (!w || !x || !y || M < 1 || M > MTTS_PFCAP || K % 16 || N < 1) return fail(MTTS_EINVAL, "gemm: need 1<=M<=MTTS_PFCAP, K%%16==0");
    hipStream_t st = S(stream);
    int Npad = round_up(N, 32);
    void *wp = nullptr, *xp = nullptr;
    float* part = nullptr;
    GemmPlan p = mtts_plan_gemm(Npad, K, ksplit);
    p.depth = gemm_depth_env();
    DevBufs hb;
    TRY(hb.get((uint16_t**)&wp, (size_t)Npad * K));
    const bool tiled = M > MTTS_RCAP;
    const int ks = tiled ? (ksplit > 0 ? ksplit : mtts_tile_ksplit(Npad, K, M)) : p.ksplit;
    TRY(hb.get((uint16_t**)&xp, (size_t)MTTS_PFCAP * K));
    TRY(hb.get(&part, (size_t)ks * MTTS_PFCAP * Npad));
    launch_pack_weight(w, wp, N, K, Npad, 1, 0, st);
    const int tiles = (M + 31) / 32;
    launch_pack_rows(x, xp, M, K, tiles == 3 ? 4 : tiles, st);
    if (tiled) launch_gemm_tile(EPI_PARTIAL, M, ks, wp, xp, K, Npad, Npad, part, nullptr, st);
    else launch_gemm(EPI_PARTIAL, tiles, p, wp, xp, K, Npad, Npad, part, nullptr, st);
    launch_reduce_partial_bf16(part, y, ks, Npad, N, M, st);
    HIPCHK(hipGetLastError());
    HIPCHK(hipStreamSynchronize(st));
    return MTTS_OK;
// ... 684 lines not shown
    HIPCHK(hipDeviceSynchronize());
    const float scale = 1.0f / sqrtf((float)MTTS_HD);
    const int R = round_up(e->B, 32);
    const int len_bound = e->max_real + e->steps_issued + 1;
    const int pages_bound = pages_for(len_bound);
    if (phase == ATTN_ROW) {
        if (attn_row_prepare()) return fail(MTTS_EINVAL, "attn_row_kernel: the dynamic LDS limit could not be raised");
        const QkvFuse f0{e->partial, e->p_qkv.ksplit, e->qkv_rows, nullptr, nullptr, nullptr, nullptr, 0.f};
        for (int n = 0; n < e->L; ++n) {
            const KvPack pk = layer_pack(e, n, pages_bound);
            if (!attn_row_fits(e->nq / e->nkv, &f0, (pk.k || pk.v) ? &pk : nullptr, pages_bound))
                return fail(MTTS_EINVAL, "attn_bench: the whole-row kernel does not take this shape");
        }
    }
    hipEvent_t e0, e1;
    hipEventCreate(&e0); hipEventCreate(&e1);
    auto run = [&](int n) {
        for (int i = 0; i < n; ++i) {
            const int layer = i % e->L;
            uint16_t* kc = (uint16_t*)e->kcache + e->layer_stride * layer;
            uint16_t* vc = (uint16_t*)e->vcache + e->layer_stride * layer;
            const QkvFuse fz{e->partial, e->p_qkv.ksplit, e->qkv_rows, (const uint16_t*)e->layers[layer].qn,
                             (const uint16_t*)e->layers[layer].kn, e->rope_cos, e->rope_sin, e->cfg.rms_norm_eps};
            const KvPack pk = layer_pack(e, layer, pages_bound);
            launch_attn(e->qbuf, kc, vc, e->d_page_table, e->d_meta, e->scores, e->stats, e->opart, e->attn_p, R, pages_bound,
                        e->max_pages, e->total_pages, e->nchunks_max, e->nq, e->nkv, scale, (phase == ATTN_ROW || e->B * pages_bound <= e->fuse_qkv_max) ? &fz : nullptr, (AttnPhase)phase, nullptr,
                        (pk.k || pk.v) ? &pk : nullptr);
        }
    };
    run(e->L);
    hipEventRecord(e0, nullptr);
    run(iters);
    hipEventRecord(e1, nullptr);
    HIPCHK(hipEventSynchronize(e1));
    float ms = 0;
    hipEventElapsedTime(&ms, e0, e1);
    *avg_ms = ms / iters;
    if (bytes_per_launch) {
        std::vector<RowMeta> m(MTTS_RCAP);
        HIPCHK(hipMemcpy(m.data(), e->d_meta, m.size() * sizeof(RowMeta), hipMemcpyDeviceToHost));
        int64_t tok = 0;
        for (int b = 0; b < R; ++b) if (m[b].seq >= 0) tok += m[b].pos + 1;
        *bytes_per_launch = phase == ATTN_COMBINE ? 0 : tok * e->nkv * MTTS_HD * 2 * ((phase == ATTN_ALL || phase == ATTN_ROW) ? 2 : 1);
    }
    hipEventDestroy(e0); hipEventDestroy(e1);
    return MTTS_OK;
}

int32_t mtts_k_gemm_bench(int32_t N, int32_t K, int32_t epi, int32_t ksplit, int32_t waves, int32_t copies,
                                     int32_t iters, float* avg_us) {
    if (N % 32 || K % 16 || copies < 1 || iters < 1 || !avg_us) return fail(MTTS_EINVAL, "gemm_bench: bad argument");
    const int tile_rows = waves < 0 ? -waves : 0;
    if (tile_rows > MTTS_PFCAP) return fail(MTTS_EINVAL, "gemm_bench: at most MTTS_PFCAP rows");
    GemmPlan p = (ksplit > 0 && waves > 0) ? mtts_plan_gemm_forced(N, K, ksplit, waves) : mtts_plan_gemm(N, K, tile_rows ? std::max(ksplit, 1) : ksplit);
    if (tile_rows) p.ksplit = std::max(ksplit, 1);
    p.depth = gemm_depth_env();
    DevBufs hb;
    std::vector<uint16_t*> w(copies, nullptr);
    for (auto& q : w) { TRY(hb.get(&q, (size_t)N * K, false)); HIPCHK(hipMemset(q, 0x3c, (size_t)N * K * 2)); }
    uint16_t *x = nullptr, *out = nullptr;
    float* part = nullptr;
    TRY(hb.get(&x, (size_t)MTTS_PFCAP * K, false));
    HIPCHK(hipMemset(x, 0x3c, (size_t)MTTS_PFCAP * K * 2));
    TRY(hb.get(&out, (size_t)MTTS_PFCAP * N));
    TRY(hb.get(&part, (size_t)p.ksplit * MTTS_PFCAP * N));
    hipEvent_t e0, e1;
    hipEventCreate(&e0); hipEventCreate(&e1);
    auto go = [&](int i) {
        if (tile_rows) launch_gemm_tile(epi, tile_rows, p.ksplit, w[i % copies], x, K, N, N, part, out, nullptr);
        else launch_gemm(epi, 1, p, w[i % copies], x, K, N, N, part, out, nullptr);
    };
    for (int i = 0; i < copies; ++i) go(i);
    HIPCHK(hipDeviceSynchronize());
    hipEventRecord(e0, nullptr);
    for (int i = 0; i < iters; ++i) go(i);
    hipEventRecord(e1, nullptr);
    HIPCHK(hipEventSynchronize(e1));
    float ms = 0;
    hipEventElapsedTime(&ms, e0, e1);
    *avg_us = ms * 1000.f / iters;
    hipEventDestroy(e0); hipEventDestroy(e1);
    return MTTS_OK;
}
```

### moss-ttsd_amd/csrc/launch.h

```cpp
#pragma once
#include <type_traits>

#include "../../include/mtts.h"
#include "common.h"
#include "kvpool.h"

enum { EPI_PARTIAL = 0, EPI_BF16 = 1, EPI_SILU = 2,
       EPI_SILU_RM = 3 };
struct GemmPlan {
    int waves, ksplit, kt_per_split, kt_per_wave;
    int depth;
};
GemmPlan mtts_plan_gemm(int Npad, int K, int want_ksplit);
GemmPlan mtts_plan_gemm_forced(int Npad, int K, int ksplit, int waves);
void launch_gemm(int epi, int mb, const GemmPlan& p, const void* Wp, const void* Xp, int K, int Npad, int n_valid,
                 float* partial, uint16_t* out, hipStream_t st);
int mtts_tile_ksplit(int Npad, int K, int R);
void launch_gemm_tile(int epi, int R, int ksplit, const void* Wp, const void* Xp, int K, int Npad, int n_valid,
                      float* partial, uint16_t* out, hipStream_t st);
int mtts_small_lds_bytes(const GemmPlan& p, int K, int pro);
void launch_gemv_small(int epi, int pro, const GemmPlan& p, const void* Wp, int K, int Npad, int n_valid, float* partial,
                       uint16_t* out, const SmallPro& pr, hipStream_t st);
long long mtts_gemm_depth_launches();
void launch_pack_weight(const void* src, void* dst, int rows, int cols, int rows_pad, int row_mul, int row_off, hipStream_t st);
void launch_pack_rows(const void* src, void* dst, int R, int K, int tiles, hipStream_t st);
void launch_reduce_partial_bf16(const float* partial, void* out, int ksplit, int Npad, int n_valid, int R, hipStream_t st);

void launch_embed_norm(const int32_t* tokens, const RowMeta* meta, const uint16_t* const* tables, const void* norm_w,
                       void* x, void* xn_packed, int R, int H, float eps, hipStream_t st);
void launch_resid_norm(const float* partial, int ksplit, int Npad, void* x, const void* norm_w, void* xn_packed,
                       void* hlast, const RowMeta* meta, int R, int H, float eps, hipStream_t st);
void launch_qkv_post(const float* partial, int ksplit, int Npad, const RowMeta* meta, const void* qnw, const void* knw,
                     const void* cosb, const void* sinb, void* qbuf, void* kcache, void* vcache,
                     const int32_t* page_table, int max_pages, int total_pages, int R, int nq, int nkv, float eps,
                     hipStream_t st);
void launch_rmsnorm_rows(const void* x, const void* w, void* y, int rows, int n, float eps, hipStream_t st);
void launch_fill_random_bf16(void* p, size_t n, uint32_t seed, hipStream_t st);
void launch_set_pages(int32_t* table, const PageEdits& ed, hipStream_t st);
void launch_fork(void* kc, void* vc, size_t layer_bytes, size_t head_bytes, int blk_bytes, int L, int nkv, const ForkJob& job,
                 hipStream_t st);
void launch_pack_kv_pages(const void* K, const void* V, void* kcache, void* vcache, const int32_t* page_table, const int32_t* lens,
                          int S, int Lmax, int nkv, int max_pages, int total_pages, hipStream_t st);
void launch_bf16_to_f32(const void* a, float* b, size_t n, hipStream_t st);
void launch_unpack_rows(const void* packed, void* out, int R, int K, hipStream_t st);

enum AttnPhase { ATTN_ALL = 0, ATTN_SCORES = 1, ATTN_PV = 2, ATTN_COMBINE = 3,
                 ATTN_ROW = 4,
                 ATTN_PF_SCORES = 11, ATTN_PF_PV = 12, ATTN_PF_COMBINE = 13 };
int launch_attn(const void* qbuf, void* kcache, void* vcache, const int32_t* page_table,
                const RowMeta* meta, void* scores, float* stats, float* opart, void* out_packed, int R,
                int pages_bound, int max_pages, int total_pages, int nchunks_max, int nq, int nkv, float scale,
                const QkvFuse* fuse, AttnPhase phase, hipStream_t st, const KvPack* pack = nullptr);
bool attn_row_fits(int G, const QkvFuse* fuse, const KvPack* pack, int pages_bound);
int attn_row_prepare();
int attn_row_lds_limit();
long long mtts_attn_row_launches();
void launch_kv_seal_rows(const void* kcache, const void* vcache, void* kpack, void* vpack, const int32_t* page_table,
                         const RowMeta* meta, int R, int max_pages, int total_pages, int nkv, int L, unsigned long long* cnt, hipStream_t st);
void launch_kv_seal_all(const void* kcache, const void* vcache, void* kpack, void* vpack, int total_pages, int nkv, int L,
                        unsigned long long* cnt, hipStream_t st);
void launch_kv_seal_pages(const void* raw, void* pk, int npages, int as_k, hipStream_t st);
void launch_kv_pack_count(const void* kpack, const void* vpack, const int32_t* page_table, const int32_t* complete, int B, int max_pages,
                          int total_pages, int nkv, int L, unsigned long long* out, hipStream_t st);

struct SeqState {
    int32_t nas;
    int32_t unfinished;
    int32_t kv_len;
    int32_t step;
    int32_t base_length;
    int32_t max_length;
    int32_t row_id;
    int32_t active;
    uint64_t seed;
};

struct LoopState {
    int32_t step;
    int32_t done;
    int32_t continuous;
    int32_t B;
    int32_t error;
    int32_t gen_cap;
    int32_t forced_draw;
    int32_t logits_f32;
};
static_assert(sizeof(SeqState) == 40 && std::is_trivially_copyable<SeqState>::value, "SeqState layout");
static_assert(sizeof(LoopState) == 32 && std::is_trivially_copyable<LoopState>::value, "LoopState layout");

#define SAMP_CAND 4096
#define SAMP_NS 32
struct SampleScratch {
    uint32_t* hist = nullptr;
    float* slice_val = nullptr;
    int32_t* slice_idx = nullptr;
    float* cand_val = nullptr;
    int32_t* cand_idx = nullptr;
    uint32_t* cand_n = nullptr;
    int32_t* overflow = nullptr;
    float* full_val = nullptr;
    int32_t* full_idx = nullptr;
    uint32_t* nuc_cnt = nullptr;
    unsigned long long* nuc_mass = nullptr;
    float* slice_sum = nullptr;
    float* lp = nullptr;
};
void launch_sample(const void* logits0, const void* logits17, int V0, int Vs, int Vs_pad, const uint32_t* bitmaps,
                   int bm_words, const MttsSamplerCfg* cfgs, const LoopState* ls, const SeqState* seqs, uint64_t seed,
                   int32_t* decisions, int32_t* err, int B, const SampleScratch& sc, int ch0_sampled, int full_cap,
// ... 58 lines not shown
```

### moss-ttsd_amd/mtts/capi.py

```python
from __future__ import annotations

import ctypes as C
import os

_HERE = os.path.dirname(os.path.abspath(__file__))
LIB_PATH = os.path.join(os.path.dirname(_HERE), "lib", "libmtts.so")


class MttsConfig(C.Structure):
    _fields_ = [(n, C.c_int32) for n in (
        "vocab_size", "hidden_size", "intermediate_size", "num_hidden_layers", "num_attention_heads",
        "num_key_value_heads", "head_dim", "channels", "speech_vocab_size", "speech_pad_token",
        "speech_range_lo", "speech_range_hi", "eos_token_id", "max_position")] + [
        ("rms_norm_eps", C.c_float), ("max_batch", C.c_int32), ("max_seq_len", C.c_int32), ("kv_pool_pages", C.c_int32), ("dtype", C.c_int32)]


class MttsSamplerCfg(C.Structure):
    _fields_ = [("do_sample", C.c_int32), ("top_k", C.c_int32), ("top_p", C.c_float),
                ("one_minus_top_p", C.c_float), ("temperature", C.c_float), ("repetition_penalty", C.c_float)]


class MttsCodecConfig(C.Structure):
    _fields_ = [(n, C.c_int32) for n in (
        "nq", "codebook_size", "rvq_dim", "quant_out_dim",
        "adapter_layers", "adapter_dim", "adapter_heads", "adapter_ffn", "adapter_max_pos", "up_stride",
        "dec_layers", "dec_dim", "dec_heads", "dec_ffn", "dec_max_pos", "mel_bins",
        "voc_dim", "voc_inter", "voc_layers", "n_fft", "hop",
        "mel_n_fft", "mel_hop", "mel_frames", "enc_layers", "enc_dim", "enc_heads", "enc_ffn", "enc_max_pos",
        "sem_adapter_layers", "pre_rvq_layers", "down_pool")]


class MttsError(RuntimeError):
    def __init__(self, msg, code=0):
        super().__init__(msg)
        self.code = code


EINVAL = -1
ENOMEM = -3
ESTATE = -4


_lib = None

_SIGS = {
    "mtts_last_error": (C.c_char_p, []),
    "mtts_version": (C.c_int32, []),
    "mtts_engine_create": (C.c_int32, [C.POINTER(MttsConfig), C.c_int32, C.POINTER(C.c_void_p)]),
    "mtts_engine_destroy": (C.c_int32, [C.c_void_p]),
    "mtts_bind_weight": (C.c_int32, [C.c_void_p, C.c_char_p, C.c_void_p, C.c_int64, C.c_int64, C.c_void_p]),
    "mtts_bind_weight_lora": (C.c_int32, [C.c_void_p, C.c_char_p, C.c_void_p, C.c_int64, C.c_int64, C.c_void_p, C.c_void_p,
                                          C.c_int32, C.c_float, C.c_void_p]),
    "mtts_k_lora_pack": (C.c_int32, [C.c_void_p, C.c_int32, C.c_int32, C.c_void_p, C.c_void_p, C.c_int32, C.c_float,
                                     C.c_int32, C.c_int32, C.c_int32, C.c_int32, C.c_void_p, C.c_void_p]),
    "mtts_adapter_load": (C.c_int32, [C.c_void_p, C.c_int32, C.c_char_p, C.c_void_p, C.c_void_p, C.c_int64, C.c_int64, C.c_int32,
                                      C.c_float, C.c_void_p]),
    "mtts_adapter_clear": (C.c_int32, [C.c_void_p, C.c_int32]),
    "mtts_set_row_adapters": (C.c_int32, [C.c_void_p, C.c_void_p, C.c_int32]),
    "mtts_set_slot_adapter": (C.c_int32, [C.c_void_p, C.c_int32, C.c_int32]),
    "mtts_k_lora_delta": (C.c_int32, [C.c_void_p, C.c_int32, C.c_int32, C.c_int32, C.c_int32, C.c_void_p, C.c_int32] +
                          [C.c_void_p] * 6 + [C.c_int32, C.c_void_p]),
    "mtts_k_swiglu_slabs": (C.c_int32, [C.c_void_p] * 5 + [C.c_int32] * 3 + [C.c_void_p]),
    "mtts_bind_rope": (C.c_int32, [C.c_void_p, C.c_void_p, C.c_void_p, C.c_int32, C.c_void_p]),
    "mtts_weights_ready": (C.c_int32, [C.c_void_p]),
    "mtts_generate": (C.c_int32, [C.c_void_p, C.c_void_p, C.c_void_p, C.c_int32, C.c_int32, C.c_int32,
                                  C.POINTER(MttsSamplerCfg), C.c_uint64, C.c_void_p, C.c_int32,
                                  C.POINTER(C.c_int32), C.c_void_p, C.c_int32, C.c_void_p, C.c_void_p]),
    "mtts_begin": (C.c_int32, [C.c_void_p, C.c_void_p, C.c_void_p, C.c_int32, C.c_int32, C.c_int32,
                               C.POINTER(MttsSamplerCfg), C.c_uint64, C.c_void_p]),
    "mtts_step": (C.c_int32, [C.c_void_p, C.c_int32, C.c_void_p]),
    "mtts_sync_state": (C.c_int32, [C.c_void_p, C.POINTER(C.c_int32), C.POINTER(C.c_int32), C.c_void_p]),
    "mtts_read_generated": (C.c_int32, [C.c_void_p, C.c_void_p, C.c_int32, C.POINTER(C.c_int32)]),
    "mtts_set_output_scores": (C.c_int32, [C.c_void_p, C.c_int32]),
    "mtts_read_scores": (C.c_int32, [C.c_void_p, C.c_void_p, C.c_int32, C.POINTER(C.c_int32)]),
    "mtts_slot_read_scores": (C.c_int32, [C.c_void_p, C.c_int32, C.c_void_p, C.c_int32, C.POINTER(C.c_int32)]),
    "mtts_score": (C.c_int32, [C.c_void_p, C.c_void_p, C.c_void_p, C.c_void_p, C.c_int32, C.c_int32, C.c_void_p, C.c_void_p]),
    "mtts_score_topk": (C.c_int32, [C.c_void_p, C.c_void_p, C.c_void_p, C.c_void_p, C.c_int32, C.c_int32, C.c_void_p, C.c_int32,
                                    C.c_void_p, C.c_void_p, C.c_void_p]),
    "mtts_read_logits": (C.c_int32, [C.c_void_p, C.c_void_p, C.c_void_p, C.c_void_p]),
    "mtts_read_logits_f32": (C.c_int32, [C.c_void_p, C.c_void_p, C.c_void_p, C.c_void_p]),
    "mtts_sched_open": (C.c_int32, [C.c_void_p, C.c_int32, C.c_int32, C.POINTER(MttsSamplerCfg), C.c_void_p]),
    "mtts_slot_submit": (C.c_int32, [C.c_void_p, C.c_int32, C.c_void_p, C.c_int32, C.c_int32, C.c_uint64, C.c_void_p]),
    "mtts_slot_submit_row": (C.c_int32, [C.c_void_p, C.c_int32, C.c_void_p, C.c_int32, C.c_int32, C.c_uint64, C.c_int32, C.c_void_p]),
    "mtts_set_row_ids": (C.c_int32, [C.c_void_p, C.c_void_p, C.c_int32]),
    "mtts_set_takes": (C.c_int32, [C.c_void_p, C.c_int32]),
    "mtts_slot_fork": (C.c_int32, [C.c_void_p, C.c_int32, C.c_int32, C.c_uint64, C.c_int32, C.c_void_p]),
    "mtts_slot_states": (C.c_int32, [C.c_void_p, C.c_void_p, C.c_void_p]),
    "mtts_slot_read": (C.c_int32, [C.c_void_p, C.c_int32, C.c_void_p, C.c_int32, C.POINTER(C.c_int32)]),
    "mtts_read_seq_state": (C.c_int32, [C.c_void_p, C.c_void_p, C.c_void_p, C.c_void_p, C.c_void_p]),
    "mtts_slot_evict": (C.c_int32, [C.c_void_p, C.c_int32, C.c_void_p]),
    "mtts_kv_pool_state": (C.c_int32, [C.c_void_p, C.POINTER(C.c_int32), C.POINTER(C.c_int32), C.POINTER(C.c_int32)]),
    "mtts_read_page_table": (C.c_int32, [C.c_void_p, C.c_void_p, C.c_void_p]),
    "mtts_set_forced_mode": (C.c_int32, [C.c_void_p, C.c_int32]),
    "mtts_debug_read_device_page_table": (C.c_int32, [C.c_void_p, C.c_void_p, C.c_void_p]),
    "mtts_export_codes": (C.c_int32, [C.c_void_p, C.c_int32, C.c_int32, C.c_void_p, C.c_void_p]),
    "mtts_profile_enable": (C.c_int32, [C.c_void_p, C.c_int32]),
    "mtts_profile_read": (C.c_int32, [C.c_void_p, C.c_int32, C.POINTER(C.c_double), C.POINTER(C.c_int64),
                                      C.POINTER(C.c_int64)]),
    "mtts_debug_set_kv_len": (C.c_int32, [C.c_void_p, C.c_int32]),
    "mtts_debug_kv_pack_stats": (C.c_int32, [C.c_void_p, C.c_void_p]),
    "mtts_k_kv_seal": (C.c_int32, [C.c_void_p, C.c_int32, C.c_void_p, C.c_int32, C.c_void_p]),
    "mtts_k_attn_bench": (C.c_int32, [C.c_void_p, C.c_int32, C.c_int32, C.POINTER(C.c_float), C.POINTER(C.c_int64)]),
    "mtts_k_gemm_bench": (C.c_int32, [C.c_int32] * 7 + [C.POINTER(C.c_float)]),
    "mtts_k_gemm_bf16": (C.c_int32, [C.c_void_p, C.c_void_p, C.c_void_p, C.c_int32, C.c_int32, C.c_int32,
                                     C.c_int32, C.c_void_p]),
    "mtts_debug_gemm_depth_launches": (C.c_int64, []),
    "mtts_debug_attn_row_launches": (C.c_int64, []),
    "mtts_k_attn_section": (C.c_int32, [C.c_void_p, C.c_int32] + [C.c_void_p] * 4 + [C.c_float] + [C.c_void_p] * 4 +
                            [C.c_int32] * 6 + [C.c_void_p] * 6),
    "mtts_k_attn_prefill": (C.c_int32, [C.c_void_p, C.c_int32] + [C.c_void_p] * 4 + [C.c_float] + [C.c_void_p] * 5 +
                            [C.c_int32] * 4 + [C.c_void_p] * 5),
    "mtts_k_gemm_swiglu_bf16": (C.c_int32, [C.c_void_p, C.c_void_p, C.c_void_p, C.c_int32, C.c_int32, C.c_int32, C.c_void_p]),
    "mtts_k_rmsnorm": (C.c_int32, [C.c_void_p, C.c_void_p, C.c_void_p, C.c_int32, C.c_int32, C.c_float, C.c_void_p]),
    "mtts_k_embed_norm": (C.c_int32, [C.c_void_p] * 5 + [C.c_int32, C.c_int32, C.c_float] + [C.c_void_p] * 3),
    "mtts_k_resid_norm": (C.c_int32, [C.c_void_p, C.c_int32, C.c_int32] + [C.c_void_p] * 4 + [C.c_int32] * 3 + [C.c_float] +
                          [C.c_void_p] * 3),
    "mtts_k_gemv_small": (C.c_int32, [C.c_int32, C.c_int32, C.c_void_p] + [C.c_int32] * 4 + [C.c_void_p, C.c_void_p, C.c_int32,
                                      C.c_void_p, C.c_float] + [C.c_void_p] * 4 + [C.c_int32, C.c_int32] + [C.c_void_p] * 4),
    "mtts_k_gemm_tile": (C.c_int32, [C.c_int32] + [C.c_void_p] * 3 + [C.c_int32] * 4 + [C.c_void_p]),
    "mtts_k_rope_kvwrite": (C.c_int32, [C.c_void_p] * 6 + [C.c_int32, C.c_int32, C.c_int32, C.c_float] + [C.c_void_p] * 4),
    "mtts_k_paged_attn_decode": (C.c_int32, [C.c_void_p] * 5 + [C.c_int32] * 4 + [C.c_void_p, C.c_void_p]),
    "mtts_k_head_ce": (C.c_int32, [C.c_void_p, C.c_void_p, C.c_void_p] + [C.c_int32] * 5 + [C.c_void_p, C.c_void_p]),
    "mtts_k_head_topk": (C.c_int32, [C.c_void_p, C.c_void_p] + [C.c_int32] * 6 + [C.c_void_p, C.c_void_p, C.c_void_p]),
    "mtts_k_sample": (C.c_int32, [C.c_void_p, C.c_int32, C.c_int32, C.c_void_p, C.POINTER(MttsSamplerCfg),
                                  C.c_int32, C.c_uint64, C.c_int32, C.c_int32, C.c_void_p, C.c_void_p]),
    "mtts_k_sample_scores": (C.c_int32, [C.c_void_p, C.c_int32, C.c_int32, C.c_void_p, C.POINTER(MttsSamplerCfg),
                                         C.c_int32, C.c_uint64, C.c_int32, C.c_int32, C.c_void_p, C.c_void_p, C.c_void_p]),
    "mtts_codec_last_error": (C.c_char_p, []),
    "mtts_codec_create": (C.c_int32, [C.POINTER(MttsCodecConfig), C.c_int32, C.POINTER(C.c_void_p)]),
    "mtts_codec_destroy": (C.c_int32, [C.c_void_p]),
    "mtts_codec_bind": (C.c_int32, [C.c_void_p, C.c_char_p, C.c_void_p, C.c_int64, C.c_void_p]),
    "mtts_codec_detokenize": (C.c_int32, [C.c_void_p, C.c_void_p, C.c_void_p, C.c_int32, C.c_int32, C.c_void_p, C.c_void_p]),
    "mtts_codec_detokenize_async": (C.c_int32, [C.c_void_p, C.c_void_p, C.c_void_p, C.c_int32, C.c_int32, C.c_void_p, C.c_void_p]),
    "mtts_codec_check": (C.c_int32, [C.c_void_p, C.c_void_p]),
    "mtts_codec_tokenize": (C.c_int32, [C.c_void_p, C.c_void_p, C.c_void_p, C.c_int32, C.c_int32, C.c_void_p, C.c_void_p, C.c_void_p]),
    "mtts_k_gemm_f32": (C.c_int32, [C.c_void_p, C.c_void_p, C.c_void_p, C.c_void_p, C.c_int32, C.c_int32, C.c_int32,
                                    C.c_int32, C.c_void_p]),
    "mtts_k_gemm_planes_bench": (C.c_int32, [C.c_int32, C.c_int32, C.c_int32, C.c_int32, C.c_int32, C.c_int32,
                                             C.POINTER(C.c_float), C.POINTER(C.c_int32)]),
}


def exported_symbols():
    return sorted(_SIGS)


def lib():
    global _lib
    if _lib is None:
        if not os.path.exists(LIB_PATH):
            raise MttsError(f"{LIB_PATH} is missing: build it with `python moss-ttsd_amd/build.py` "
                            "(hipcc --offload-arch=gfx950); there is no CPU fallback")
        L = C.CDLL(LIB_PATH)
        for name, (res, args) in _SIGS.items():
            fn = getattr(L, name)
            fn.restype = res
            fn.argtypes = args
        _lib = L
    return _lib


def check(rc):
    if rc != 0:
        raise MttsError(f"libmtts error {rc}: {lib().mtts_last_error().decode()}", rc)
```

### moss-ttsd_amd/mtts/engine.py

```python
from __future__ import annotations

import ctypes as C

import numpy as np
import torch

from . import capi


def sampler_cfgs(layers=None, do_samples=None):
    arr = (capi.MttsSamplerCfg * 8)()
    for i in range(8):
        lc = (layers[i] if layers and i < len(layers) else {}) or {}
        s = arr[i]
        s.do_sample = 1 if (do_samples and do_samples[i]) else 0
        s.top_k = int(lc.get("top_k") or 0)
        tp = lc.get("top_p")
        s.top_p = float(tp) if tp is not None else 0.0
        s.one_minus_top_p = float(np.float32(1.0 - tp)) if tp is not None else 0.0
        t = lc.get("temperature")
        s.temperature = float(t) if t is not None else 0.0
        rp = lc.get("repetition_penalty")
        s.repetition_penalty = float(rp) if rp is not None else 0.0
    return arr
# ... 209 lines not shown
    def read_logits(self):
        V0, Vs = self.cfg["vocab_size"], self.cfg["speech_vocab_size"]
        if self.dtype != "bf16":
            l0 = np.zeros((self._B, V0), dtype=np.float32)
            l17 = np.zeros((7, self._B, Vs), dtype=np.float32)
            capi.check(self.lib.mtts_read_logits_f32(self._h, l0.ctypes.data, l17.ctypes.data, None))
            return l0, l17
        l0 = np.zeros((self._B, V0), dtype=np.uint16)
        l17 = np.zeros((7, self._B, Vs), dtype=np.uint16)
        capi.check(self.lib.mtts_read_logits(self._h, l0.ctypes.data, l17.ctypes.data, None))
        f = lambda u: (u.astype(np.uint32) << 16).view(np.float32)
        return f(l0), f(l17)

    def sched_open(self, slots, gen_cap, layers=None, do_samples=None, output_scores=False):
        self._B = int(slots)
        self.set_output_scores(output_scores)
        capi.check(self.lib.mtts_sched_open(self._h, int(slots), int(gen_cap), sampler_cfgs(layers, do_samples), None))

    def submit(self, slot, ids, max_length, seed=0, row_id=0, adapter=None):
        ids = np.ascontiguousarray(ids, dtype=np.int64)
        assert ids.ndim == 2 and ids.shape[1] == 8
        if adapter is not None and int(adapter) >= 0:
            capi.check(self.lib.mtts_set_slot_adapter(self._h, int(slot), int(adapter)))
        capi.check(self.lib.mtts_slot_submit_row(self._h, int(slot), ids.ctypes.data, ids.shape[0], int(max_length),
                                                 C.c_uint64(seed), int(row_id), None))

    def fork(self, src, dst, seed=0, row_id=0):
        capi.check(self.lib.mtts_slot_fork(self._h, int(src), int(dst), C.c_uint64(seed), int(row_id), None))

    def slot_states(self):
        st = np.zeros((self._B, 4), dtype=np.int32)
        capi.check(self.lib.mtts_slot_states(self._h, st.ctypes.data, None))
        return st

    def slot_read(self, slot, capacity):
        buf = np.zeros((int(capacity), 8), dtype=np.int64)
        n = C.c_int32(0)
        capi.check(self.lib.mtts_slot_read(self._h, int(slot), buf.ctypes.data, int(capacity), C.byref(n)))
        return buf[:n.value].copy()

    def slot_read_scores(self, slot, capacity):
        buf = np.zeros((max(int(capacity), 1), 8), dtype=np.float32)
        n = C.c_int32(0)
        capi.check(self.lib.mtts_slot_read_scores(self._h, int(slot), buf.ctypes.data, buf.shape[0], C.byref(n)))
        return buf[:n.value].copy()

    def evict(self, slot):
        capi.check(self.lib.mtts_slot_evict(self._h, int(slot), None))

    def kv_pool_state(self):
        a, b, c = C.c_int32(0), C.c_int32(0), C.c_int32(0)
        capi.check(self.lib.mtts_kv_pool_state(self._h, C.byref(a), C.byref(b), C.byref(c)))
        return a.value, b.value, c.value

    def page_table(self, max_batch):
        _, _, mp = self.kv_pool_state()
        t = np.zeros((int(max_batch), mp), dtype=np.int32)
        n = np.zeros(int(max_batch), dtype=np.int32)
        capi.check(self.lib.mtts_read_page_table(self._h, t.ctypes.data, n.ctypes.data))
        return t, n

    def device_page_table(self, max_batch):
        _, _, mp = self.kv_pool_state()
        t = np.zeros((int(max_batch), mp), dtype=np.int32)
        capi.check(self.lib.mtts_debug_read_device_page_table(self._h, t.ctypes.data, None))
        return t

    def seq_state(self):
        a, u, k = (np.zeros(self._B, dtype=np.int32) for _ in range(3))
        capi.check(self.lib.mtts_read_seq_state(self._h, a.ctypes.data, u.ctypes.data, k.ctypes.data, None))
        return a, u, k

    def export_codes(self, first, n, stream=None):
        out = torch.empty(8, self._B, n, dtype=torch.int64, device=self.device)
        sp = C.c_void_p(stream.cuda_stream) if stream is not None else None
        capi.check(self.lib.mtts_export_codes(self._h, int(first), int(n), out.data_ptr(), sp))
        return out

    def kv_pack_stats(self):
        o = np.zeros(6, dtype=np.int64)
        capi.check(self.lib.mtts_debug_kv_pack_stats(self._h, o.ctypes.data))
        return dict(zip(("k_pages", "k_unsealed", "v_pages", "v_unsealed", "k_layers_on", "v_layers_on"), (int(x) for x in o)))

    def debug_set_kv_len(self, n):
        capi.check(self.lib.mtts_debug_set_kv_len(self._h, int(n)))

    def attn_bench(self, phase, iters=112):
        ms, by = C.c_float(0), C.c_int64(0)
        capi.check(self.lib.mtts_k_attn_bench(self._h, int(phase), int(iters), C.byref(ms), C.byref(by)))
        return ms.value, by.value

    def profile(self, on=True):
        capi.check(self.lib.mtts_profile_enable(self._h, 1 if on else 0))

    def profile_read(self, which):
        ms, n, by = C.c_double(0), C.c_int64(0), C.c_int64(0)
        capi.check(self.lib.mtts_profile_read(self._h, which, C.byref(ms), C.byref(n), C.byref(by)))
        return ms.value, n.value, by.value
```

Measured before the change: 81630 codec_tokens/s.

## Add lossless sealed (exponent-dictionary compressed) weight format for MLP and head GEMMs

Introduces a compressed 'sealed' weight layout that encodes each bf16 group's exponents through a small per-group dictionary. It reuses the KV-cache sealing encoder, now shared in a header and templated for 12- or 16-unit groups. Gate/up, down and LM-head weights get sealed copies at weight load and LoRA bind time. A policy pass counts groups that do not fit and enables each sealed GEMM only when the unsealed fraction is below a per-kind threshold. The goal is fewer weight bytes read from HBM in the bandwidth-bound decode GEMMs, paid for with extra memory for the sealed copies, decode ALU work in the GEMM, and a fallback path for groups that do not fit.

New measurement: 82680 codec_tokens/s, median of 6. 1.3% higher.

```diff
diff --git a/include/mtts.h b/include/mtts.h
--- a/include/mtts.h
+++ b/include/mtts.h
@@ -123,6 +123,14 @@
 int32_t mtts_k_gemm_bench(int32_t N, int32_t K, int32_t epi, int32_t ksplit, int32_t waves, int32_t copies,
                           int32_t iters, float* avg_us);
 
+int32_t mtts_debug_wseal_stats(MttsEngine* e, int64_t* out12);
+int64_t mtts_debug_wseal_launches(void);
+int32_t mtts_k_gemm_sealed_bench(const void* dev_w, int32_t N, int32_t K, int32_t epi, int32_t ksplit, int32_t copies,
+                                 int32_t iters, int32_t sealed, int32_t head_form, float* avg_us, int64_t* out2);
+
+int32_t mtts_k_wseal(const void* dev_packed, int32_t ntiles, int32_t K, int32_t ktw, void* dev_sealed, void* stream);
+int32_t mtts_k_gemm_sealed(const void* dev_w, const void* dev_x, void* dev_out, int32_t M, int32_t N, int32_t K, int32_t epi,
+                           int32_t ksplit, int32_t sealed, int32_t head_form, int64_t* out2, void* stream);
 int32_t mtts_k_gemm_bf16(const void* dev_w, const void* dev_x, void* dev_y,
                          int32_t M, int32_t N, int32_t K, int32_t ksplit, void* stream);
 int64_t mtts_debug_gemm_depth_launches(void);
diff --git a/moss-ttsd_amd/build.py b/moss-ttsd_amd/build.py
--- a/moss-ttsd_amd/build.py
+++ b/moss-ttsd_amd/build.py
@@ -4,7 +4,7 @@
 from concurrent.futures import ThreadPoolExecutor
 
 HERE = os.path.dirname(os.path.abspath(__file__))
-SRC = ["gemm.hip", "layer.hip", "attn.hip", "sampler.hip", "f32path.hip", "score.hip", "adapter.hip", "multilora.hip", "engine.hip", "hooks.hip", "codec.hip", "codec_fused.hip"]
+SRC = ["gemm.hip", "gemm_sealed.hip", "layer.hip", "attn.hip", "sampler.hip", "f32path.hip", "score.hip", "adapter.hip", "multilora.hip", "engine.hip", "hooks.hip", "codec.hip", "codec_fused.hip"]
 OUT = os.path.join(HERE, "lib", "libmtts.so")
 OBJ = os.path.join(HERE, "build")
 FLAGS = ["--offload-arch=gfx950", "-O3", "-std=c++17", "-fPIC", "-fno-gpu-rdc", "-Wno-unused-result", "-Wno-unused-value"]
diff --git a/moss-ttsd_amd/csrc/attn.hip b/moss-ttsd_amd/csrc/attn.hip
--- a/moss-ttsd_amd/csrc/attn.hip
+++ b/moss-ttsd_amd/csrc/attn.hip
@@ -11,82 +11,8 @@
 #define PK_OCC(PK)
 #endif
 
-__device__ __forceinline__ uint32_t u4c(const u32x4_t& v, int c) { return c == 0 ? v.x : c == 1 ? v.y : c == 2 ? v.z : v.w; }
-__device__ __forceinline__ void pk_unit(const u32x4_t* pk, int j, uint32_t w[4]) {
-    const uint32_t L0 = u4c(pk[j >> 1], 2 * (j & 1)), L1 = u4c(pk[j >> 1], 2 * (j & 1) + 1);
-    const uint32_t N = u4c(pk[8 + (j >> 2)], j & 3);
-    const uint32_t lo = pk[12].x, hi = pk[12].y;
-    const uint32_t HA = ((N & 0x08080808u) << 4) | __builtin_amdgcn_perm(hi, lo, N & 0x07070707u);
-    const uint32_t HB = (N & 0x80808080u) | __builtin_amdgcn_perm(hi, lo, (N >> 4) & 0x07070707u);
-    w[0] = __builtin_amdgcn_perm(HA, L0, 0x05010400u);
-    w[1] = __builtin_amdgcn_perm(HA, L0, 0x07030602u);
-    w[2] = __builtin_amdgcn_perm(HB, L1, 0x05010400u);
-    w[3] = __builtin_amdgcn_perm(HB, L1, 0x07030602u);
-}
-
-__host__ __device__ constexpr int pk_order(int i) { return i == 0 ? 12 : (i - 1) % 3 == 0 ? 8 + (i - 1) / 3 : 2 * ((i - 1) / 3) + (i - 1) % 3 - 1; }
-__device__ bool seal_encode(const u32x4_t (&v)[16], u32x4_t* __restrict__ pk, uint32_t spare, bool unfit) {
-    unsigned long long b0 = 0ull, b1 = 0ull;
-#pragma unroll
-    for (int j = 0; j < 16; ++j)
-#pragma unroll
-        for (int c = 0; c < 4; ++c)
-#pragma unroll
-            for (int h = 0; h < 2; ++h) {
-                const uint32_t e = (u4c(v[j], c) >> (8 + 16 * h)) & 0x7fu;
-                if (e & 64u) b1 |= 1ull << (e & 63u);
-                else b0 |= 1ull << e;
-            }
-    const int n0 = __popcll(b0), n = n0 + __popcll(b1);
-    if (n > 8 || unfit) {
-        pk[12 * 64] = u32x4_t{0u, 0u, spare, 1u};
-        return false;
-    }
-    unsigned long long dict = 0ull;
-    {
-        unsigned long long t0 = b0, t1 = b1;
-        for (int i = 0; i < n; ++i) {
-            uint32_t e;
-            if (t0) { e = __ffsll((long long)t0) - 1; t0 &= t0 - 1; }
-            else { e = 64 + __ffsll((long long)t1) - 1; t1 &= t1 - 1; }
-            dict |= (unsigned long long)e << (8 * i);
-        }
-    }
-    auto code = [&](uint32_t half) -> uint32_t {
-        const uint32_t e = (half >> 8) & 0x7fu;
-        const uint32_t rank = (e & 64u) ? n0 + __popcll(b1 & ((1ull << (e & 63u)) - 1ull)) : __popcll(b0 & ((1ull << e) - 1ull));
-        return ((half >> 12) & 8u) | rank;
-    };
-    uint32_t lowp[32], nib[16];
-#pragma unroll
-    for (int j = 0; j < 16; ++j) {
-        uint32_t N = 0u;
-#pragma unroll
-        for (int g = 0; g < 2; ++g) {
-            uint32_t L = 0u;
-#pragma unroll
-            for (int k = 0; k < 4; ++k) {
-                const uint32_t half = (u4c(v[j], 2 * g + (k >> 1)) >> (16 * (k & 1))) & 0xffffu;
-                L |= (half & 0xffu) << (8 * k);
-                N |= code(half) << (8 * k + 4 * g);
-            }
-            lowp[2 * j + g] = L;
-        }
-        nib[j] = N;
-    }
-#pragma unroll
-    for (int u = 0; u < 8; ++u) pk[u * 64] = u32x4_t{lowp[4 * u], lowp[4 * u + 1], lowp[4 * u + 2], lowp[4 * u + 3]};
-#pragma unroll
-    for (int u = 0; u < 4; ++u) pk[(8 + u) * 64] = u32x4_t{nib[4 * u], nib[4 * u + 1], nib[4 * u + 2], nib[4 * u + 3]};
-    pk[12 * 64] = u32x4_t{(uint32_t)dict, (uint32_t)(dict >> 32), spare, 0u};
-    return true;
-}
-__device__ bool seal_lane(const u32x4_t* __restrict__ raw, u32x4_t* __restrict__ pk) {
-    u32x4_t v[16];
-#pragma unroll
-    for (int j = 0; j < 16; ++j) v[j] = raw[j * 64];
-    return seal_encode(v, pk, 0u, false);
-}
+#include "seal.h"
+
 __device__ bool seal_lane_k(const u32x4_t* __restrict__ raw, u32x4_t* __restrict__ pk, uint8_t* __restrict__ lds, int lane) {
     u32x4_t v[16];
 #pragma unroll
diff --git a/moss-ttsd_amd/csrc/engine.h b/moss-ttsd_amd/csrc/engine.h
--- a/moss-ttsd_amd/csrc/engine.h
+++ b/moss-ttsd_amd/csrc/engine.h
@@ -27,6 +27,7 @@
 
 static inline int round_up(int a, int b) { return (a + b - 1) / b * b; }
 static inline hipStream_t S(void* s) { return (hipStream_t)s; }
+static const double WSEAL_MAX_UNSEALED[4] = {-1.0, 1.0 / 512, 1.0 / 8, 1.0 / 64};
 static inline int gemm_depth_env() {
     const char* g = getenv("MTTS_GEMM_DEPTH");
     return (g && atoi(g) == 0) ? 0 : 1;
@@ -112,6 +113,7 @@
 
 struct Layer {
     void *wqkv = nullptr, *wo = nullptr, *wgu = nullptr, *wd = nullptr;
+    void *wgu_s = nullptr, *wd_s = nullptr;
     void *ln_in = nullptr, *ln_post = nullptr, *qn = nullptr, *kn = nullptr;
     int bound = 0;
 };
@@ -140,6 +142,13 @@
     void *x2 = nullptr, *act_rm = nullptr;
     int small_rows = SMALL_RP;
     int gemm_depth = 1;
+    int w_seal = 1;
+    int w_seal_head = 1;
+    void *head0_s = nullptr, *heads17_s = nullptr;
+    int wseal_ktw[WSEAL_KINDS] = {0, 0, 0, 0};
+    bool wseal_dirty = false;
+    char wseal_on[WSEAL_KINDS] = {0, 0, 0, 0};
+    unsigned long long *d_wseal_cnt = nullptr, *h_wseal_cnt = nullptr;
     void *x = nullptr, *xn = nullptr, *attn_p = nullptr, *act_p = nullptr, *qbuf = nullptr, *hlast = nullptr, *xh = nullptr;
     void *logits0 = nullptr, *logits17 = nullptr, *join_logits0 = nullptr, *join_logits17 = nullptr;
     void* scores = nullptr;
diff --git a/moss-ttsd_amd/csrc/engine.hip b/moss-ttsd_amd/csrc/engine.hip
--- a/moss-ttsd_amd/csrc/engine.hip
+++ b/moss-ttsd_amd/csrc/engine.hip
@@ -166,6 +166,25 @@
     e->p_h0 = mtts_plan_gemm(e->V0_pad, H, 1);
     e->p_h17 = mtts_plan_gemm(7 * e->Vs_pad, H, 1);
     for (GemmPlan* p : {&e->p_qkv, &e->p_o, &e->p_gu, &e->p_d, &e->p_h0, &e->p_h17}) p->depth = e->gemm_depth;
+    if (const char* g = getenv("MTTS_W_SEAL")) e->w_seal = std::min(std::max(atoi(g), 0), 2);
+    if (const char* g = getenv("MTTS_W_SEAL_HEAD")) e->w_seal_head = atoi(g) != 0;
+    if (!e->f32 && e->w_seal && e->gemm_depth) {
+        const int Hp = round_up(H, 32);
+        const auto wanted = [&](int kind) { return e->w_seal == 2 || WSEAL_MAX_UNSEALED[kind] >= 0.0; };
+        if (wanted(WSEAL_GU) && wseal_shape(e->p_gu, H, 2 * I, EPI_SILU)) e->wseal_ktw[WSEAL_GU] = e->p_gu.kt_per_wave;
+        if (wanted(WSEAL_DOWN) && wseal_shape(e->p_d, I, Hp, EPI_PARTIAL)) e->wseal_ktw[WSEAL_DOWN] = e->p_d.kt_per_wave;
+        if (wanted(WSEAL_HEAD0) && wseal_shape(e->p_h0, H, e->V0_pad, EPI_BF16)) e->wseal_ktw[WSEAL_HEAD0] = e->p_h0.kt_per_wave;
+        if (wanted(WSEAL_HEADS) && wseal_shape(e->p_h17, H, 7 * e->Vs_pad, EPI_BF16)) e->wseal_ktw[WSEAL_HEADS] = e->p_h17.kt_per_wave;
+        for (auto& l : e->layers) {
+            if (e->wseal_ktw[WSEAL_GU]) TRY(m.get((uint8_t**)&l.wgu_s, wseal_bytes(2 * I, H, e->wseal_ktw[WSEAL_GU])));
+            if (e->wseal_ktw[WSEAL_DOWN]) TRY(m.get((uint8_t**)&l.wd_s, wseal_bytes(Hp, I, e->wseal_ktw[WSEAL_DOWN])));
+        }
+        if (e->wseal_ktw[WSEAL_HEAD0]) TRY(m.get((uint8_t**)&e->head0_s, wseal_bytes(e->V0_pad, H, e->wseal_ktw[WSEAL_HEAD0])));
+        if (e->wseal_ktw[WSEAL_HEADS]) TRY(m.get((uint8_t**)&e->heads17_s, wseal_bytes(7 * e->Vs_pad, H, e->wseal_ktw[WSEAL_HEADS])));
+        TRY(m.get(&e->d_wseal_cnt, (size_t)WSEAL_KINDS * 2));
+        TRY(m.get_pinned(&e->h_wseal_cnt, (size_t)WSEAL_KINDS * 2));
+        e->wseal_dirty = true;
+    }
     size_t pmax = (size_t)8 * std::max(e->qkv_rows, round_up(H, 32));
     if (!e->f32) {
         TRY(m.get(&e->partial, pmax * MTTS_PFCAP));
@@ -263,7 +282,14 @@
     int bit = 0;
     bool proj = false;
     int layer = -1, proj_idx = -1;
+    void* seal_to = nullptr;
+    int seal_ktw = 0, seal_nt0 = 0, seal_nt = 0;
 };
+static void reseal(MttsEngine* e, const WeightSlot& w, hipStream_t st) {
+    if (!w.seal_to) return;
+    launch_wseal(w.pack_to, w.seal_to, (int)w.cols, w.seal_ktw, w.seal_nt0, w.seal_nt, st);
+    e->wseal_dirty = true;
+}
 
 static int resolve_weight(MttsEngine* e, const char* name_c, WeightSlot& w) {
     const std::string name(name_c);
@@ -276,6 +302,9 @@
         w.pack_to = ch == 0 ? e->head0 : e->heads17;
         w.rows_pad = ch == 0 ? e->V0_pad : 7 * e->Vs_pad;
         w.row_off = ch == 0 ? 0 : (ch - 1) * e->Vs_pad;
+        w.seal_to = ch == 0 ? e->head0_s : e->heads17_s;
+        w.seal_ktw = e->wseal_ktw[ch == 0 ? WSEAL_HEAD0 : WSEAL_HEADS];
+        w.seal_nt0 = w.row_off / 32; w.seal_nt = (ch == 0 ? e->V0_pad : e->Vs_pad) / 32;
         w.bound = &e->emb_bound; w.bit = 1 << ch;
         return MTTS_OK;
     }
@@ -312,6 +341,9 @@
             w.bound = &l.bound; w.bit = 1 << i;
             w.proj = t[i].cols != 1;
             w.layer = n; w.proj_idx = i - 4;
+            if (t[i].bf == l.wgu) { w.seal_to = l.wgu_s; w.seal_ktw = e->wseal_ktw[WSEAL_GU]; }
+            if (t[i].bf == l.wd) { w.seal_to = l.wd_s; w.seal_ktw = e->wseal_ktw[WSEAL_DOWN]; }
+            w.seal_nt0 = 0; w.seal_nt = w.rows_pad / 32;
             return MTTS_OK;
         }
     return fail(MTTS_EINVAL, "unknown tensor %s", name_c);
@@ -334,6 +366,7 @@
     } else {
         if (w.copy_to) HIPCHK(hipMemcpyAsync(w.copy_to, src, n * 2, hipMemcpyDeviceToDevice, st));
         if (w.pack_to) launch_pack_weight(src, w.pack_to, (int)w.rows, (int)w.cols, w.rows_pad, w.row_mul, w.row_off, st);
+        reseal(e, w, st);
         HIPCHK(hipGetLastError());
     }
     *w.bound |= w.bit;
@@ -360,8 +393,10 @@
     if (e->f32)
         launch_lora_rows_f32((const float*)base, lora_a, lora_b, r, scaling, w.f32_to + w.f32_row * w.cols, (int)w.rows, (int)w.cols,
                              e->h16 ? 1 : 0, st);
-    else
+    else {
         launch_lora_pack(base, lora_a, lora_b, r, scaling, w.pack_to, (int)w.rows, (int)w.cols, w.row_mul, w.row_off, st);
+        reseal(e, w, st);
+    }
     HIPCHK(hipGetLastError());
     *w.bound |= w.bit;
     return MTTS_OK;
@@ -511,6 +546,33 @@
     return bind_rope_tables(e, e->rope_cos, e->rope_sin, cosb, sinb, rows, S(stream));
 }
 
+static int wseal_policy(MttsEngine* e) {
+    if (!e->wseal_dirty || !e->d_wseal_cnt) return MTTS_OK;
+    HIPCHK(hipSetDevice(e->device));
+    HIPCHK(hipDeviceSynchronize());
+    HIPCHK(hipMemsetAsync(e->d_wseal_cnt, 0, WSEAL_KINDS * 2 * sizeof(unsigned long long), nullptr));
+    const int H = e->H, I = e->I, Hp = round_up(H, 32);
+    for (auto& l : e->layers) {
+        if (l.wgu_s) launch_wseal_count(l.wgu_s, 2 * I, H, e->wseal_ktw[WSEAL_GU], e->d_wseal_cnt + 2 * WSEAL_GU, nullptr);
+        if (l.wd_s) launch_wseal_count(l.wd_s, Hp, I, e->wseal_ktw[WSEAL_DOWN], e->d_wseal_cnt + 2 * WSEAL_DOWN, nullptr);
+    }
+    if (e->head0_s) launch_wseal_count(e->head0_s, e->V0_pad, H, e->wseal_ktw[WSEAL_HEAD0], e->d_wseal_cnt + 2 * WSEAL_HEAD0, nullptr);
+    if (e->heads17_s) launch_wseal_count(e->heads17_s, 7 * e->Vs_pad, H, e->wseal_ktw[WSEAL_HEADS], e->d_wseal_cnt + 2 * WSEAL_HEADS, nullptr);
+    HIPCHK(hipGetLastError());
+    HIPCHK(hipMemcpyAsync(e->h_wseal_cnt, e->d_wseal_cnt, WSEAL_KINDS * 2 * sizeof(unsigned long long), hipMemcpyDeviceToHost, nullptr));
+    HIPCHK(hipStreamSynchronize(nullptr));
+    bool changed = false;
+    for (int k = 0; k < WSEAL_KINDS; ++k) {
+        const unsigned long long groups = e->h_wseal_cnt[2 * k], bad = e->h_wseal_cnt[2 * k + 1];
+        const char on = e->wseal_ktw[k] && groups && (e->w_seal == 2 || (double)bad <= WSEAL_MAX_UNSEALED[k] * (double)groups);
+        changed |= on != e->wseal_on[k];
+        e->wseal_on[k] = on;
+    }
+    if (changed) drop_graphs(e);
+    e->wseal_dirty = false;
+    return MTTS_OK;
+}
+
 int32_t mtts_weights_ready(MttsEngine* e) {
     if (!e) return fail(MTTS_EINVAL, "null engine");
     if (e->emb_bound != 0xff) return fail(MTTS_ESTATE, "embedding tables missing (mask %x)", e->emb_bound);
@@ -518,7 +580,7 @@
     if (!e->rope_rows) return fail(MTTS_ESTATE, "rope table missing");
     for (int n = 0; n < e->L; ++n)
         if (e->layers[n].bound != 2047) return fail(MTTS_ESTATE, "layer %d incomplete (mask %x)", n, e->layers[n].bound);
-    return MTTS_OK;
+    return wseal_policy(e);
 }
 
 static void prof_begin(MttsEngine* e, int which, hipStream_t st, hipEvent_t* a) {
@@ -641,6 +703,7 @@
             launch_lora_delta(xp, d_meta, e->d_seq_adapter, e->d_bank + (size_t)n * 7, job, e->partial + (size_t)ks * MTTS_PFCAP * job.Npad, R, st);
         };
         const int ex = lora ? 1 : 0;
+        const bool sealed_gu = !lora && e->wseal_on[WSEAL_GU], sealed_d = !lora && e->wseal_on[WSEAL_DOWN];
         const int ks_qkv = tiled ? mtts_tile_ksplit(e->qkv_rows, H, 1024) : e->p_qkv.ksplit;
         const int ks_o = tiled ? mtts_tile_ksplit(Hp, nq * MTTS_HD, 1024) : e->p_o.ksplit;
         const int ks_d = tiled ? mtts_tile_ksplit(Hp, I, 1024) : e->p_d.ksplit;
@@ -656,13 +719,15 @@
         const int gu_epi = lora ? EPI_PARTIAL : EPI_SILU;
         float* gu_slab = lora ? e->partial : nullptr;
         if (tiled) launch_gemm_tile(gu_epi, R, 1, l.wgu, e->xn, H, 2 * I, 2 * I, gu_slab, (uint16_t*)e->act_p, st);
-        else launch_gemm(gu_epi, mb, e->p_gu, l.wgu, e->xn, H, 2 * I, 2 * I, gu_slab, (uint16_t*)e->act_p, st);
+        else if (!sealed_gu || !launch_gemm_sealed(EPI_SILU, mb, e->p_gu, l.wgu_s, l.wgu, e->xn, H, 2 * I, 2 * I, nullptr, (uint16_t*)e->act_p, 0, st))
+            launch_gemm(gu_epi, mb, e->p_gu, l.wgu, e->xn, H, 2 * I, 2 * I, gu_slab, (uint16_t*)e->act_p, st);
         if (lora) {
             delta(j_gu, e->xn, 1);
             launch_swiglu_slabs(e->partial, e->partial + (size_t)MTTS_PFCAP * 2 * I, e->act_p, mb * 32, I, st);
         }
         if (tiled) launch_gemm_tile(EPI_PARTIAL, R, ks_d, l.wd, e->act_p, I, Hp, Hp, e->partial, nullptr, st);
-        else launch_gemm(EPI_PARTIAL, mb, e->p_d, l.wd, e->act_p, I, Hp, Hp, e->partial, nullptr, st);
+        else if (!sealed_d || !launch_gemm_sealed(EPI_PARTIAL, mb, e->p_d, l.wd_s, l.wd, e->act_p, I, Hp, Hp, e->partial, nullptr, 0, st))
+            launch_gemm(EPI_PARTIAL, mb, e->p_d, l.wd, e->act_p, I, Hp, Hp, e->partial, nullptr, st);
         if (lora) delta(j_d, e->act_p, ks_d);
         const bool lastl = (n == e->L - 1);
         const void* nw = lastl ? e->final_norm : e->layers[n + 1].ln_in;
@@ -678,8 +743,12 @@
             launch_pack_rows(e->hlast, e->xh, e->B, H, hmb, st);
             xin = e->xh;
         }
-        launch_gemm(EPI_BF16, hmb, e->p_h0, e->head0, xin, H, e->V0_pad, e->V0, nullptr, (uint16_t*)e->logits0, st);
-        launch_gemm(EPI_BF16, hmb, e->p_h17, e->heads17, xin, H, 7 * e->Vs_pad, 7 * e->Vs_pad, nullptr, (uint16_t*)e->logits17, st);
+        if (lora || !e->wseal_on[WSEAL_HEAD0] ||
+            !launch_gemm_sealed(EPI_BF16, hmb, e->p_h0, e->head0_s, e->head0, xin, H, e->V0_pad, e->V0, nullptr, (uint16_t*)e->logits0, e->w_seal_head, st))
+            launch_gemm(EPI_BF16, hmb, e->p_h0, e->head0, xin, H, e->V0_pad, e->V0, nullptr, (uint16_t*)e->logits0, st);
+        if (lora || !e->wseal_on[WSEAL_HEADS] ||
+            !launch_gemm_sealed(EPI_BF16, hmb, e->p_h17, e->heads17_s, e->heads17, xin, H, 7 * e->Vs_pad, 7 * e->Vs_pad, nullptr, (uint16_t*)e->logits17, e->w_seal_head, st))
+            launch_gemm(EPI_BF16, hmb, e->p_h17, e->heads17, xin, H, 7 * e->Vs_pad, 7 * e->Vs_pad, nullptr, (uint16_t*)e->logits17, st);
     }
     HIPCHK(hipGetLastError());
     return MTTS_OK;
diff --git a/moss-ttsd_amd/csrc/gemm.hip b/moss-ttsd_amd/csrc/gemm.hip
--- a/moss-ttsd_amd/csrc/gemm.hip
+++ b/moss-ttsd_amd/csrc/gemm.hip
@@ -1,4 +1,5 @@
 #include "launch.h"
+#include "gemm_epi.h"
 
 
 template <int WAVES, int EPI, int MB>
@@ -82,29 +83,6 @@
                     out[xpack_off(row, idx, Npad >> 1)] = f2bf(a * u);
                 }
             }
-        }
-    }
-}
-
-template <int EPI>
-__device__ __forceinline__ void skinny_store(const float (&v)[4], int row, int n0, int ks, float* __restrict__ partial,
-                                             uint16_t* __restrict__ out, int Npad, int n_valid) {
-    if (EPI == EPI_PARTIAL) {
-        *(float4*)(partial + ((size_t)ks * MTTS_PFCAP + row) * Npad + n0) = make_float4(v[0], v[1], v[2], v[3]);
-    } else if (EPI == EPI_BF16) {
-        uint16_t* o = out + (size_t)row * Npad + n0;
-        if (n0 + 3 < n_valid) *(u32x2_t*)o = u32x2_t{pack2(v[0], v[1]), pack2(v[2], v[3])};
-        else {
-#pragma unroll
-            for (int j = 0; j < 4; ++j)
-                if (n0 + j < n_valid) o[j] = f2bf(v[j]);
-        }
-    } else {
-#pragma unroll
-        for (int j = 0; j < 2; ++j) {
-            float g = rbf(v[2 * j]), u = rbf(v[2 * j + 1]);
-            float a = rbf(g / (1.0f + expf(-g)));
-            out[xpack_off(row, (n0 >> 1) + j, Npad >> 1)] = f2bf(a * u);
         }
     }
 }
@@ -544,6 +522,7 @@
 
 static long long g_depth_launches = 0;
 long long mtts_gemm_depth_launches() { return g_depth_launches; }
+void mtts_gemm_depth_note() { ++g_depth_launches; }
 static bool launch_gemm_depth(int epi, int mb, const GemmPlan& p, const void* Wp, const void* Xp, int K, int Npad,
                               int n_valid, float* partial, uint16_t* out, hipStream_t st) {
     const int KT = K / 16;
diff --git a/moss-ttsd_amd/csrc/gemm_epi.h b/moss-ttsd_amd/csrc/gemm_epi.h
--- /dev/null
+++ b/moss-ttsd_amd/csrc/gemm_epi.h
@@ -0,0 +1,25 @@
+#pragma once
+#include "launch.h"
+
+template <int EPI>
+__device__ __forceinline__ void skinny_store(const float (&v)[4], int row, int n0, int ks, float* __restrict__ partial,
+                                             uint16_t* __restrict__ out, int Npad, int n_valid) {
+    if (EPI == EPI_PARTIAL) {
+        *(float4*)(partial + ((size_t)ks * MTTS_PFCAP + row) * Npad + n0) = make_float4(v[0], v[1], v[2], v[3]);
+    } else if (EPI == EPI_BF16) {
+        uint16_t* o = out + (size_t)row * Npad + n0;
+        if (n0 + 3 < n_valid) *(u32x2_t*)o = u32x2_t{pack2(v[0], v[1]), pack2(v[2], v[3])};
+        else {
+#pragma unroll
+            for (int j = 0; j < 4; ++j)
+                if (n0 + j < n_valid) o[j] = f2bf(v[j]);
+        }
+    } else {
+#pragma unroll
+        for (int j = 0; j < 2; ++j) {
+            float g = rbf(v[2 * j]), u = rbf(v[2 * j + 1]);
+            float a = rbf(g / (1.0f + expf(-g)));
+            out[xpack_off(row, (n0 >> 1) + j, Npad >> 1)] = f2bf(a * u);
+        }
+    }
+}
diff --git a/moss-ttsd_amd/csrc/gemm_sealed.hip b/moss-ttsd_amd/csrc/gemm_sealed.hip
--- /dev/null
+++ b/moss-ttsd_amd/csrc/gemm_sealed.hip
@@ -0,0 +1,280 @@
+#include "launch.h"
+#include "gemm_epi.h"
+#include "seal.h"
+
+template <int KTW> __host__ __device__ constexpr int su_pos(int u) { return u < 8 ? u : u < 12 ? KTW / 2 + (u - 8) : KTW / 2 + KTW / 4; }
+template <int KTW> __host__ __device__ constexpr int su_count() { return KTW / 2 + KTW / 4 + 1; }
+
+template <int KTW>
+__global__ __launch_bounds__(64) void wseal_kernel(const u32x4_t* __restrict__ Wp, u32x4_t* __restrict__ Ws, int KT, int nt0) {
+    const int nt = nt0 + blockIdx.y, c = blockIdx.x, lane = threadIdx.x;
+    seal_lane<KTW>(Wp + ((size_t)nt * KT + (size_t)c * KTW) * 64 + lane,
+                   Ws + ((size_t)nt * (KT / KTW) + c) * (su_count<KTW>() * 64) + lane);
+}
+__global__ __launch_bounds__(256) void wseal_count_kernel(const u32x4_t* __restrict__ Ws, size_t groups, int nu,
+                                                          unsigned long long* __restrict__ out) {
+    const size_t g = (size_t)blockIdx.x * 4 + (threadIdx.x >> 6);
+    if (g >= groups) return;
+    const int lane = threadIdx.x & 63;
+    const u32x4_t d = Ws[(g * nu + (nu - 1)) * 64 + lane];
+    const bool bad = __ballot(d.w != 0u) != 0ull;
+    if (lane == 0) {
+        atomicAdd(out, 1ull);
+        if (bad) atomicAdd(out + 1, 1ull);
+    }
+}
+
+template <int KTW>
+__device__ __forceinline__ void sealed_request(u32x4_t (&pk)[MTTS_PKU], const u32x4_t* __restrict__ g) {
+#pragma unroll
+    for (int i = 0; i < su_count<KTW>(); ++i) {
+        pk[pk_order(i)] = __builtin_nontemporal_load(g + su_pos<KTW>(pk_order(i)) * 64);
+        __builtin_amdgcn_sched_barrier(0);
+    }
+}
+template <int KTW>
+__device__ __forceinline__ void plain_request(u32x4_t (&a)[KTW], const u32x4_t* __restrict__ w) {
+#pragma unroll
+    for (int u = 0; u < KTW; ++u) {
+        a[u] = __builtin_nontemporal_load(w + (size_t)u * 64);
+        __builtin_amdgcn_sched_barrier(0);
+    }
+}
+template <int KTW>
+__device__ __forceinline__ f32x16_t sealed_chain(const u32x4_t (&pk)[MTTS_PKU], const u32x4_t (&b)[KTW], f32x16_t acc) {
+#pragma unroll
+    for (int u = 0; u < KTW; ++u) {
+        uint32_t w[4];
+        pk_unit(pk, u, w);
+        const u32x4_t a = {w[0], w[1], w[2], w[3]};
+        acc = __builtin_amdgcn_mfma_f32_32x32x16_bf16(*(const bf16x8_t*)&a, *(const bf16x8_t*)&b[u], acc, 0, 0, 0);
+    }
+    return acc;
+}
+template <int KTW>
+__device__ __forceinline__ f32x16_t plain_chain(const u32x4_t (&a)[KTW], const u32x4_t (&b)[KTW], f32x16_t acc) {
+#pragma unroll
+    for (int u = 0; u < KTW; ++u)
+        acc = __builtin_amdgcn_mfma_f32_32x32x16_bf16(*(const bf16x8_t*)&a[u], *(const bf16x8_t*)&b[u], acc, 0, 0, 0);
+    return acc;
+}
+template <int KTW>
+__device__ __forceinline__ f32x16_t plain_halves(const u32x4_t* __restrict__ w, const u32x4_t (&b)[KTW], f32x16_t acc) {
+#pragma unroll
+    for (int h = 0; h < 2; ++h) {
+        u32x4_t a[KTW / 2], bh[KTW / 2];
+#pragma unroll
+        for (int u = 0; u < KTW / 2; ++u) bh[u] = b[h * (KTW / 2) + u];
+        plain_request<KTW / 2>(a, w + (size_t)h * (KTW / 2) * 64);
+        acc = plain_chain<KTW / 2>(a, bh, acc);
+        __builtin_amdgcn_sched_barrier(0);
+    }
+    return acc;
+}
+__device__ __forceinline__ void sealed_touch(const u32x4_t (&pk)[MTTS_PKU]) {
+#pragma unroll
+    for (int i = 0; i < MTTS_PKU; ++i) asm volatile("" ::"v"(pk[i]));
+    __builtin_amdgcn_sched_barrier(0);
+}
+__device__ __forceinline__ f32x16_t zero16() {
+    f32x16_t z;
+#pragma unroll
+    for (int i = 0; i < 16; ++i) z[i] = 0.f;
+    return z;
+}
+template <int WAVES, int EPI>
+__device__ __forceinline__ void reduce_store(float (&red)[WAVES][16][64], int wave, int lane, int nt, int ks, float* __restrict__ partial,
+                                             uint16_t* __restrict__ out, int Npad, int n_valid) {
+    for (int q = wave; q < 4; q += WAVES) {
+        float v[4];
+#pragma unroll
+        for (int j = 0; j < 4; ++j) {
+            float s = red[0][4 * q + j][lane];
+#pragma unroll
+            for (int w = 1; w < WAVES; ++w) s += red[w][4 * q + j][lane];
+            v[j] = s;
+        }
+        skinny_store<EPI>(v, lane & 31, nt * 32 + 8 * q + 4 * (lane >> 5), ks, partial, out, Npad, n_valid);
+    }
+}
+
+template <int WAVES, int KTW, int EPI>
+__global__ __launch_bounds__(WAVES * 64) void depth_sealed_kernel(
+    const u32x4_t* __restrict__ Ws, const u32x4_t* __restrict__ Wp, const u32x4_t* __restrict__ Xp, int KT, float* __restrict__ partial,
+    uint16_t* __restrict__ out, int Npad, int n_valid) {
+    __shared__ float red[WAVES][16][64];
+    const int nt = blockIdx.x, ks = blockIdx.y;
+    const int wave = threadIdx.x >> 6, lane = threadIdx.x & 63;
+    const int c = ks * WAVES + wave, kt0 = c * KTW;
+    const u32x4_t* xp = Xp + (size_t)kt0 * 64 + lane;
+    u32x4_t b[KTW], pk[MTTS_PKU];
+#pragma unroll
+    for (int u = 0; u < KTW; ++u) b[u] = xp[(size_t)u * 64];
+    __builtin_amdgcn_sched_barrier(0);
+    sealed_request<KTW>(pk, Ws + ((size_t)nt * (KT / KTW) + c) * (su_count<KTW>() * 64) + lane);
+    f32x16_t acc = zero16();
+    if (__builtin_expect(__ballot(pk[12].w != 0u) != 0ull, 0)) {
+        u32x4_t a[KTW];
+        plain_request<KTW>(a, Wp + ((size_t)nt * KT + kt0) * 64 + lane);
+        sealed_touch(pk);
+        acc = plain_chain<KTW>(a, b, acc);
+    } else acc = sealed_chain<KTW>(pk, b, acc);
+#pragma unroll
+    for (int r = 0; r < 16; ++r) red[wave][r][lane] = acc[r];
+    __syncthreads();
+    reduce_store<WAVES, EPI>(red, wave, lane, nt, ks, partial, out, Npad, n_valid);
+}
+
+template <int WAVES, int KTW>
+__global__ __launch_bounds__(WAVES * 64) void gateup48_sealed_kernel(
+    const u32x4_t* __restrict__ Ws, const u32x4_t* __restrict__ Wp, const u32x4_t* __restrict__ Xp, int KT, uint16_t* __restrict__ out, int Npad) {
+    __shared__ float red[WAVES][24][64];
+    constexpr int NU = su_count<KTW>();
+    const int p = blockIdx.x >> 1, o = blockIdx.x & 1;
+    const int tf = 3 * p + 2 * o, th = 3 * p + 1;
+    const int wave = threadIdx.x >> 6, lane = threadIdx.x & 63;
+    const int kt0 = wave * KTW;
+    const int hl = (((lane >> 4) & 1) == o) ? lane : (lane ^ 16);
+    const u32x4_t* xp = Xp + (size_t)kt0 * 64 + lane;
+    u32x4_t b[KTW], pw[MTTS_PKU], ph[MTTS_PKU];
+#pragma unroll
+    for (int u = 0; u < KTW; ++u) b[u] = xp[(size_t)u * 64];
+    __builtin_amdgcn_sched_barrier(0);
+    sealed_request<KTW>(pw, Ws + ((size_t)tf * WAVES + wave) * (NU * 64) + lane);
+    sealed_request<KTW>(ph, Ws + ((size_t)th * WAVES + wave) * (NU * 64) + hl);
+    f32x16_t acc = zero16(), acch = zero16();
+    if (__builtin_expect(__ballot((pw[12].w | ph[12].w) != 0u) != 0ull, 0)) {
+        sealed_touch(pw);
+        sealed_touch(ph);
+        acc = plain_halves<KTW>(Wp + ((size_t)tf * KT + kt0) * 64 + lane, b, acc);
+        acch = plain_halves<KTW>(Wp + ((size_t)th * KT + kt0) * 64 + hl, b, acch);
+    } else {
+#pragma unroll
+        for (int u = 0; u < KTW; ++u) {
+            uint32_t w[4], v[4];
+            pk_unit(pw, u, w);
+            pk_unit(ph, u, v);
+            const u32x4_t a = {w[0], w[1], w[2], w[3]}, h = {v[0], v[1], v[2], v[3]};
+            acc = __builtin_amdgcn_mfma_f32_32x32x16_bf16(*(const bf16x8_t*)&a, *(const bf16x8_t*)&b[u], acc, 0, 0, 0);
+            acch = __builtin_amdgcn_mfma_f32_32x32x16_bf16(*(const bf16x8_t*)&h, *(const bf16x8_t*)&b[u], acch, 0, 0, 0);
+        }
+    }
+#pragma unroll
+    for (int r = 0; r < 16; ++r) red[wave][r][lane] = acc[r];
+#pragma unroll
+    for (int r = 0; r < 8; ++r) red[wave][16 + r][lane] = o ? acch[8 + r] : acch[r];
+    __syncthreads();
+    for (int q6 = wave; q6 < 6; q6 += WAVES) {
+        float v[4];
+#pragma unroll
+        for (int j = 0; j < 4; ++j) {
+            float s = red[0][4 * q6 + j][lane];
+#pragma unroll
+            for (int w = 1; w < WAVES; ++w) s += red[w][4 * q6 + j][lane];
+            v[j] = s;
+        }
+        const int nt = q6 < 4 ? tf : th, q = q6 < 4 ? q6 : 2 * o + (q6 - 4);
+        skinny_store<EPI_SILU>(v, lane & 31, nt * 32 + 8 * q + 4 * (lane >> 5), 0, nullptr, out, Npad, Npad);
+    }
+}
+
+template <int WAVES, int KTW, bool NEXT>
+__device__ __forceinline__ void head_tile(float (&red)[WAVES][16][64], const u32x4_t (&b)[KTW], const u32x4_t (&pk)[MTTS_PKU],
+                                          u32x4_t (&nx)[MTTS_PKU], const u32x4_t* __restrict__ Ws, const u32x4_t* __restrict__ Wp, int KT,
+                                          int nt, int nt_next, int wave, int lane, uint16_t* __restrict__ out, int Npad, int n_valid) {
+    const bool bad = __ballot(pk[12].w != 0u) != 0ull;
+    if (NEXT) sealed_request<KTW>(nx, Ws + ((size_t)nt_next * WAVES + wave) * (su_count<KTW>() * 64) + lane);
+    f32x16_t acc = zero16();
+    if (__builtin_expect(bad, 0)) {
+        sealed_touch(pk);
+        acc = plain_halves<KTW>(Wp + ((size_t)nt * KT + (size_t)wave * KTW) * 64 + lane, b, acc);
+    } else acc = sealed_chain<KTW>(pk, b, acc);
+#pragma unroll
+    for (int r = 0; r < 16; ++r) red[wave][r][lane] = acc[r];
+    __syncthreads();
+    reduce_store<WAVES, EPI_BF16>(red, wave, lane, nt, 0, nullptr, out, Npad, n_valid);
+}
+template <int WAVES, int KTW>
+__global__ __launch_bounds__(WAVES * 64) void head_sealed_kernel(
+    const u32x4_t* __restrict__ Ws, const u32x4_t* __restrict__ Wp, const u32x4_t* __restrict__ Xp, int KT, int ntiles,
+    uint16_t* __restrict__ out, int Npad, int n_valid) {
+    __shared__ float red[2][WAVES][16][64];
+    const int wave = threadIdx.x >> 6, lane = threadIdx.x & 63;
+    const int stride = gridDim.x;
+    int nt = blockIdx.x;
+    if (nt >= ntiles) return;
+    const u32x4_t* xp = Xp + (size_t)wave * KTW * 64 + lane;
+    u32x4_t b[KTW], pa[MTTS_PKU], pb[MTTS_PKU];
+#pragma unroll
+    for (int u = 0; u < KTW; ++u) b[u] = xp[(size_t)u * 64];
+    __builtin_amdgcn_sched_barrier(0);
+    sealed_request<KTW>(pa, Ws + ((size_t)nt * WAVES + wave) * (su_count<KTW>() * 64) + lane);
+    for (;;) {
+        if (nt + stride >= ntiles) { head_tile<WAVES, KTW, false>(red[0], b, pa, pb, Ws, Wp, KT, nt, 0, wave, lane, out, Npad, n_valid); break; }
+        head_tile<WAVES, KTW, true>(red[0], b, pa, pb, Ws, Wp, KT, nt, nt + stride, wave, lane, out, Npad, n_valid);
+        nt += stride;
+        if (nt + stride >= ntiles) { head_tile<WAVES, KTW, false>(red[1], b, pb, pa, Ws, Wp, KT, nt, 0, wave, lane, out, Npad, n_valid); break; }
+        head_tile<WAVES, KTW, true>(red[1], b, pb, pa, Ws, Wp, KT, nt, nt + stride, wave, lane, out, Npad, n_valid);
+        nt += stride;
+    }
+}
+
+size_t wseal_bytes(int Npad, int K, int ktw) {
+    const int nu = ktw / 2 + ktw / 4 + 1;
+    return (size_t)(Npad / 32) * (K / 16 / ktw) * nu * 1024;
+}
+bool wseal_shape(const GemmPlan& p, int K, int Npad, int epi) {
+    const int KT = K / 16;
+    if (p.waves != 8 || K % 16 || Npad % 32 || KT != p.ksplit * 8 * p.kt_per_wave || p.kt_per_split != 8 * p.kt_per_wave) return false;
+    if (epi == EPI_PARTIAL) return p.kt_per_wave == 12;
+    if (epi == EPI_SILU) return p.ksplit == 1 && p.kt_per_wave == 16 && Npad % 96 == 0;
+    if (epi == EPI_BF16) return p.ksplit == 1 && p.kt_per_wave == 16;
+    return false;
+}
+void launch_wseal(const void* Wp, void* Ws, int K, int ktw, int nt0, int ntiles, hipStream_t st) {
+    const int KT = K / 16;
+    if (ntiles < 1) return;
+    for (int t = 0; t < ntiles; t += 32768) {
+        const dim3 grid(KT / ktw, std::min(ntiles - t, 32768));
+        if (ktw == 16) hipLaunchKernelGGL((wseal_kernel<16>), grid, dim3(64), 0, st, (const u32x4_t*)Wp, (u32x4_t*)Ws, KT, nt0 + t);
+        else hipLaunchKernelGGL((wseal_kernel<12>), grid, dim3(64), 0, st, (const u32x4_t*)Wp, (u32x4_t*)Ws, KT, nt0 + t);
+    }
+}
+void launch_wseal_count(const void* Ws, int Npad, int K, int ktw, unsigned long long* out2, hipStream_t st) {
+    const size_t groups = (size_t)(Npad / 32) * (K / 16 / ktw);
+    hipLaunchKernelGGL(wseal_count_kernel, dim3((unsigned)((groups + 3) / 4)), dim3(256), 0, st, (const u32x4_t*)Ws, groups,
+                       ktw / 2 + ktw / 4 + 1, out2);
+}
+
+static long long g_wseal_launches = 0;
+long long mtts_wseal_launches() { return g_wseal_launches; }
+static int head_grid(int ntiles) {
+    static int cus = 0;
+    if (!cus) {
+        int dev = 0, n = 0;
+        if (hipGetDevice(&dev) != hipSuccess || hipDeviceGetAttribute(&n, hipDeviceAttributeMultiprocessorCount, dev) != hipSuccess || n < 1) n = 256;
+        cus = n;
+    }
+    return std::min(ntiles, cus);
+}
+bool launch_gemm_sealed(int epi, int mb, const GemmPlan& p, const void* Ws, const void* Wp, const void* Xp, int K, int Npad,
+                        int n_valid, float* partial, uint16_t* out, int head_form, hipStream_t st) {
+    if (!Ws || !p.depth || mb > 1 || !wseal_shape(p, K, Npad, epi)) return false;
+    const int KT = K / 16;
+    if (epi == EPI_PARTIAL)
+        hipLaunchKernelGGL((depth_sealed_kernel<8, 12, EPI_PARTIAL>), dim3(Npad / 32, p.ksplit), dim3(512), 0, st, (const u32x4_t*)Ws,
+                           (const u32x4_t*)Wp, (const u32x4_t*)Xp, KT, partial, out, Npad, n_valid);
+    else if (epi == EPI_SILU) {
+        if (n_valid != Npad) return false;
+        hipLaunchKernelGGL((gateup48_sealed_kernel<8, 16>), dim3(Npad / 48), dim3(512), 0, st, (const u32x4_t*)Ws, (const u32x4_t*)Wp,
+                           (const u32x4_t*)Xp, KT, out, Npad);
+    } else if (head_form)
+        hipLaunchKernelGGL((head_sealed_kernel<8, 16>), dim3(head_form > 1 ? std::min(Npad / 32, head_form) : head_grid(Npad / 32)), dim3(512), 0, st, (const u32x4_t*)Ws,
+                           (const u32x4_t*)Wp, (const u32x4_t*)Xp, KT, Npad / 32, out, Npad, n_valid);
+    else
+        hipLaunchKernelGGL((depth_sealed_kernel<8, 16, EPI_BF16>), dim3(Npad / 32, 1), dim3(512), 0, st, (const u32x4_t*)Ws,
+                           (const u32x4_t*)Wp, (const u32x4_t*)Xp, KT, partial, out, Npad, n_valid);
+    ++g_wseal_launches;
+    mtts_gemm_depth_note();
+    return true;
+}
diff --git a/moss-ttsd_amd/csrc/hooks.hip b/moss-ttsd_amd/csrc/hooks.hip
--- a/moss-ttsd_amd/csrc/hooks.hip
+++ b/moss-ttsd_amd/csrc/hooks.hip
@@ -790,3 +790,130 @@
     hipEventDestroy(e0); hipEventDestroy(e1);
     return MTTS_OK;
 }
+
+int64_t mtts_debug_wseal_launches(void) { return (int64_t)mtts_wseal_launches(); }
+
+int32_t mtts_debug_wseal_stats(MttsEngine* e, int64_t* out12) {
+    if (!e || !out12) return fail(MTTS_EINVAL, "null argument");
+    if (!e->d_wseal_cnt) return fail(MTTS_ESTATE, "the engine keeps no sealed weights (fp32 / fp16 engine, MTTS_W_SEAL=0 or MTTS_GEMM_DEPTH=0)");
+    TRY(mtts_weights_ready(e));
+    for (int k = 0; k < WSEAL_KINDS; ++k) {
+        out12[3 * k] = (int64_t)e->h_wseal_cnt[2 * k];
+        out12[3 * k + 1] = (int64_t)e->h_wseal_cnt[2 * k + 1];
+        out12[3 * k + 2] = e->wseal_on[k];
+    }
+    return MTTS_OK;
+}
+
+int32_t mtts_k_wseal(const void* dev_packed, int32_t ntiles, int32_t K, int32_t ktw, void* dev_sealed, void* stream) {
+    if (!dev_packed || !dev_sealed || ntiles < 1 || (ktw != 16 && ktw != 12) || K < 16 * ktw || K % (16 * ktw))
+        return fail(MTTS_EINVAL, "wseal: need ktw 16 or 12 and K a multiple of 16 ktw");
+    launch_wseal(dev_packed, dev_sealed, K, ktw, 0, ntiles, S(stream));
+    HIPCHK(hipGetLastError());
+    HIPCHK(hipStreamSynchronize(S(stream)));
+    return MTTS_OK;
+}
+
+static int wseal_hook_plan(int epi, int N, int K, int ksplit, GemmPlan* p, int* Npad) {
+    if (epi != EPI_PARTIAL && epi != EPI_BF16 && epi != EPI_SILU) return fail(MTTS_EINVAL, "gemm_sealed: epi 0 (partial), 1 (bf16) or 2 (SwiGLU)");
+    if (N < 1 || K < 16 || K % 16 || ksplit < 1) return fail(MTTS_EINVAL, "gemm_sealed: bad shape");
+    *Npad = round_up(N, 32);
+    *p = mtts_plan_gemm_forced(*Npad, K, ksplit, 8);
+    if (!wseal_shape(*p, K, *Npad, epi)) return fail(MTTS_EINVAL, "gemm_sealed: not a shape the sealed kernels take (8 waves of 16 k-tiles, or 12 with split-K; SwiGLU: N %% 96 == 0)");
+    if (epi == EPI_SILU && N != *Npad) return fail(MTTS_EINVAL, "gemm_sealed: SwiGLU takes whole tiles");
+    return MTTS_OK;
+}
+
+int32_t mtts_k_gemm_sealed(const void* dev_w, const void* dev_x, void* dev_out, int32_t M, int32_t N, int32_t K, int32_t epi,
+                           int32_t ksplit, int32_t sealed, int32_t head_form, int64_t* out2, void* stream) {
+    if (!dev_w || !dev_x || !dev_out || M < 1 || M > 32) return fail(MTTS_EINVAL, "gemm_sealed: null argument or M outside 1..32");
+    GemmPlan p;
+    int Npad = 0;
+    TRY(wseal_hook_plan(epi, N, K, ksplit, &p, &Npad));
+    hipStream_t st = S(stream);
+    DevBufs hb;
+    uint16_t *wp = nullptr, *xp = nullptr, *out = nullptr;
+    uint8_t* ws = nullptr;
+    float* part = nullptr;
+    unsigned long long* cnt = nullptr;
+    const int ktw = p.kt_per_wave;
+    TRY(hb.get(&wp, (size_t)Npad * K));
+    TRY(hb.get(&ws, wseal_bytes(Npad, K, ktw)));
+    TRY(hb.get(&xp, (size_t)32 * K));
+    TRY(hb.get(&out, (size_t)32 * Npad, false));
+    TRY(hb.get(&cnt, 2));
+    if (epi == EPI_PARTIAL) {
+        TRY(hb.get(&part, (size_t)ksplit * MTTS_PFCAP * Npad, false));
+        HIPCHK(hipMemsetAsync(part, 0xa5, (size_t)ksplit * MTTS_PFCAP * Npad * 4, st));
+    }
+    HIPCHK(hipMemsetAsync(out, 0xa5, (size_t)32 * Npad * 2, st));
+    launch_pack_weight(dev_w, wp, N, K, Npad, 1, 0, st);
+    launch_wseal(wp, ws, K, ktw, 0, Npad / 32, st);
+    launch_wseal_count(ws, Npad, K, ktw, cnt, st);
+    launch_pack_rows(dev_x, xp, M, K, 1, st);
+    if (sealed) {
+        if (!launch_gemm_sealed(epi, 1, p, ws, wp, xp, K, Npad, N, part, out, head_form, st)) return fail(MTTS_EINVAL, "gemm_sealed: the sealed launch was refused");
+    } else launch_gemm(epi, 1, p, wp, xp, K, Npad, N, part, out, st);
+    HIPCHK(hipGetLastError());
+    if (epi == EPI_PARTIAL) {
+        for (int ks = 0; ks < ksplit; ++ks)
+            HIPCHK(hipMemcpyAsync((float*)dev_out + (size_t)ks * 32 * Npad, part + (size_t)ks * MTTS_PFCAP * Npad, (size_t)32 * Npad * 4, hipMemcpyDeviceToDevice, st));
+    } else HIPCHK(hipMemcpyAsync(dev_out, out, (size_t)32 * (epi == EPI_SILU ? Npad / 2 : Npad) * 2, hipMemcpyDeviceToDevice, st));
+    unsigned long long h[2] = {0, 0};
+    HIPCHK(hipMemcpyAsync(h, cnt, 16, hipMemcpyDeviceToHost, st));
+    HIPCHK(hipStreamSynchronize(st));
+    if (out2) { out2[0] = (int64_t)h[0]; out2[1] = (int64_t)h[1]; }
+    return MTTS_OK;
+}
+
+int32_t mtts_k_gemm_sealed_bench(const void* dev_w, int32_t N, int32_t K, int32_t epi, int32_t ksplit, int32_t copies, int32_t iters,
+                                 int32_t sealed, int32_t head_form, float* avg_us, int64_t* out2) {
+    if (copies < 1 || iters < 1 || !avg_us) return fail(MTTS_EINVAL, "gemm_sealed_bench: bad argument");
+    GemmPlan p;
+    int Npad = 0;
+    TRY(wseal_hook_plan(epi, N, K, ksplit, &p, &Npad));
+    DevBufs hb;
+    const int ktw = p.kt_per_wave;
+    std::vector<uint16_t*> w(copies, nullptr);
+    std::vector<uint8_t*> ws(copies, nullptr);
+    unsigned long long* cnt = nullptr;
+    TRY(hb.get(&cnt, 2));
+    for (int c = 0; c < copies; ++c) {
+        TRY(hb.get(&w[c], (size_t)Npad * K));
+        if (dev_w) launch_pack_weight(dev_w, w[c], N, K, Npad, 1, 0, nullptr);
+        else HIPCHK(hipMemset(w[c], 0x3c, (size_t)Npad * K * 2));
+        TRY(hb.get(&ws[c], wseal_bytes(Npad, K, ktw)));
+        launch_wseal(w[c], ws[c], K, ktw, 0, Npad / 32, nullptr);
+    }
+    launch_wseal_count(ws[0], Npad, K, ktw, cnt, nullptr);
+    uint16_t *x = nullptr, *out = nullptr;
+    float* part = nullptr;
+    TRY(hb.get(&x, (size_t)32 * K, false));
+    HIPCHK(hipMemset(x, 0x3c, (size_t)32 * K * 2));
+    TRY(hb.get(&out, (size_t)32 * Npad));
+    if (epi == EPI_PARTIAL) TRY(hb.get(&part, (size_t)ksplit * MTTS_PFCAP * Npad));
+    HIPCHK(hipGetLastError());
+    bool refused = false;
+    auto go = [&](int i) {
+        if (!sealed) launch_gemm(epi, 1, p, w[i % copies], x, K, Npad, N, part, out, nullptr);
+        else if (!launch_gemm_sealed(epi, 1, p, ws[i % copies], w[i % copies], x, K, Npad, N, part, out, head_form, nullptr)) refused = true;
+    };
+    for (int i = 0; i < copies; ++i) go(i);
+    HIPCHK(hipDeviceSynchronize());
+    if (refused) return fail(MTTS_EINVAL, "gemm_sealed_bench: the sealed launch was refused");
+    hipEvent_t e0, e1;
+    hipEventCreate(&e0); hipEventCreate(&e1);
+    hipEventRecord(e0, nullptr);
+    for (int i = 0; i < iters; ++i) go(i);
+    hipEventRecord(e1, nullptr);
+    HIPCHK(hipEventSynchronize(e1));
+    float ms = 0;
+    hipEventElapsedTime(&ms, e0, e1);
+    *avg_us = ms * 1000.f / iters;
+    hipEventDestroy(e0); hipEventDestroy(e1);
+    unsigned long long h[2] = {0, 0};
+    HIPCHK(hipMemcpy(h, cnt, 16, hipMemcpyDeviceToHost));
+    if (out2) { out2[0] = (int64_t)h[0]; out2[1] = (int64_t)h[1]; }
+    HIPCHK(hipGetLastError());
+    return MTTS_OK;
+}
diff --git a/moss-ttsd_amd/csrc/launch.h b/moss-ttsd_amd/csrc/launch.h
--- a/moss-ttsd_amd/csrc/launch.h
+++ b/moss-ttsd_amd/csrc/launch.h
@@ -22,9 +22,19 @@
 void launch_gemv_small(int epi, int pro, const GemmPlan& p, const void* Wp, int K, int Npad, int n_valid, float* partial,
                        uint16_t* out, const SmallPro& pr, hipStream_t st);
 long long mtts_gemm_depth_launches();
+void mtts_gemm_depth_note();
 void launch_pack_weight(const void* src, void* dst, int rows, int cols, int rows_pad, int row_mul, int row_off, hipStream_t st);
 void launch_pack_rows(const void* src, void* dst, int R, int K, int tiles, hipStream_t st);
 void launch_reduce_partial_bf16(const float* partial, void* out, int ksplit, int Npad, int n_valid, int R, hipStream_t st);
+
+enum { WSEAL_GU = 0, WSEAL_DOWN = 1, WSEAL_HEAD0 = 2, WSEAL_HEADS = 3, WSEAL_KINDS = 4 };
+bool wseal_shape(const GemmPlan& p, int K, int Npad, int epi);
+size_t wseal_bytes(int Npad, int K, int ktw);
+void launch_wseal(const void* Wp, void* Ws, int K, int ktw, int nt0, int ntiles, hipStream_t st);
+void launch_wseal_count(const void* Ws, int Npad, int K, int ktw, unsigned long long* out2, hipStream_t st);
+bool launch_gemm_sealed(int epi, int mb, const GemmPlan& p, const void* Ws, const void* Wp, const void* Xp, int K, int Npad,
+                        int n_valid, float* partial, uint16_t* out, int head_form, hipStream_t st);
+long long mtts_wseal_launches();
 
 void launch_embed_norm(const int32_t* tokens, const RowMeta* meta, const uint16_t* const* tables, const void* norm_w,
                        void* x, void* xn_packed, int R, int H, float eps, hipStream_t st);
diff --git a/moss-ttsd_amd/csrc/seal.h b/moss-ttsd_amd/csrc/seal.h
--- /dev/null
+++ b/moss-ttsd_amd/csrc/seal.h
@@ -0,0 +1,83 @@
+#pragma once
+#include "common.h"
+
+__device__ __forceinline__ uint32_t u4c(const u32x4_t& v, int c) { return c == 0 ? v.x : c == 1 ? v.y : c == 2 ? v.z : v.w; }
+__device__ __forceinline__ void pk_unit(const u32x4_t* pk, int j, uint32_t w[4]) {
+    const uint32_t L0 = u4c(pk[j >> 1], 2 * (j & 1)), L1 = u4c(pk[j >> 1], 2 * (j & 1) + 1);
+    const uint32_t N = u4c(pk[8 + (j >> 2)], j & 3);
+    const uint32_t lo = pk[12].x, hi = pk[12].y;
+    const uint32_t HA = ((N & 0x08080808u) << 4) | __builtin_amdgcn_perm(hi, lo, N & 0x07070707u);
+    const uint32_t HB = (N & 0x80808080u) | __builtin_amdgcn_perm(hi, lo, (N >> 4) & 0x07070707u);
+    w[0] = __builtin_amdgcn_perm(HA, L0, 0x05010400u);
+    w[1] = __builtin_amdgcn_perm(HA, L0, 0x07030602u);
+    w[2] = __builtin_amdgcn_perm(HB, L1, 0x05010400u);
+    w[3] = __builtin_amdgcn_perm(HB, L1, 0x07030602u);
+}
+
+__host__ __device__ constexpr int pk_order(int i) { return i == 0 ? 12 : (i - 1) % 3 == 0 ? 8 + (i - 1) / 3 : 2 * ((i - 1) / 3) + (i - 1) % 3 - 1; }
+template <int NT>
+__device__ bool seal_encode(const u32x4_t (&v)[NT], u32x4_t* __restrict__ pk, uint32_t spare, bool unfit) {
+    static_assert(NT == 16 || NT == 12, "a sealed group is 16 or 12 units");
+    constexpr int DU = NT / 2 + NT / 4;
+    unsigned long long b0 = 0ull, b1 = 0ull;
+#pragma unroll
+    for (int j = 0; j < NT; ++j)
+#pragma unroll
+        for (int c = 0; c < 4; ++c)
+#pragma unroll
+            for (int h = 0; h < 2; ++h) {
+                const uint32_t e = (u4c(v[j], c) >> (8 + 16 * h)) & 0x7fu;
+                if (e & 64u) b1 |= 1ull << (e & 63u);
+                else b0 |= 1ull << e;
+            }
+    const int n0 = __popcll(b0), n = n0 + __popcll(b1);
+    if (n > 8 || unfit) {
+        pk[DU * 64] = u32x4_t{0u, 0u, spare, 1u};
+        return false;
+    }
+    unsigned long long dict = 0ull;
+    {
+        unsigned long long t0 = b0, t1 = b1;
+        for (int i = 0; i < n; ++i) {
+            uint32_t e;
+            if (t0) { e = __ffsll((long long)t0) - 1; t0 &= t0 - 1; }
+            else { e = 64 + __ffsll((long long)t1) - 1; t1 &= t1 - 1; }
+            dict |= (unsigned long long)e << (8 * i);
+        }
+    }
+    auto code = [&](uint32_t half) -> uint32_t {
+        const uint32_t e = (half >> 8) & 0x7fu;
+        const uint32_t rank = (e & 64u) ? n0 + __popcll(b1 & ((1ull << (e & 63u)) - 1ull)) : __popcll(b0 & ((1ull << e) - 1ull));
+        return ((half >> 12) & 8u) | rank;
+    };
+    uint32_t lowp[2 * NT], nib[NT];
+#pragma unroll
+    for (int j = 0; j < NT; ++j) {
+        uint32_t N = 0u;
+#pragma unroll
+        for (int g = 0; g < 2; ++g) {
+            uint32_t L = 0u;
+#pragma unroll
+            for (int k = 0; k < 4; ++k) {
+                const uint32_t half = (u4c(v[j], 2 * g + (k >> 1)) >> (16 * (k & 1))) & 0xffffu;
+                L |= (half & 0xffu) << (8 * k);
+                N |= code(half) << (8 * k + 4 * g);
+            }
+            lowp[2 * j + g] = L;
+        }
+        nib[j] = N;
+    }
+#pragma unroll
+    for (int u = 0; u < NT / 2; ++u) pk[u * 64] = u32x4_t{lowp[4 * u], lowp[4 * u + 1], lowp[4 * u + 2], lowp[4 * u + 3]};
+#pragma unroll
+    for (int u = 0; u < NT / 4; ++u) pk[(NT / 2 + u) * 64] = u32x4_t{nib[4 * u], nib[4 * u + 1], nib[4 * u + 2], nib[4 * u + 3]};
+    pk[DU * 64] = u32x4_t{(uint32_t)dict, (uint32_t)(dict >> 32), spare, 0u};
+    return true;
+}
+template <int NT = 16>
+__device__ bool seal_lane(const u32x4_t* __restrict__ raw, u32x4_t* __restrict__ pk) {
+    u32x4_t v[NT];
+#pragma unroll
+    for (int j = 0; j < NT; ++j) v[j] = raw[j * 64];
+    return seal_encode(v, pk, 0u, false);
+}
diff --git a/moss-ttsd_amd/mtts/capi.py b/moss-ttsd_amd/mtts/capi.py
--- a/moss-ttsd_amd/mtts/capi.py
+++ b/moss-ttsd_amd/mtts/capi.py
@@ -105,6 +105,11 @@
     "mtts_k_gemm_bf16": (C.c_int32, [C.c_void_p, C.c_void_p, C.c_void_p, C.c_int32, C.c_int32, C.c_int32,
                                      C.c_int32, C.c_void_p]),
     "mtts_debug_gemm_depth_launches": (C.c_int64, []),
+    "mtts_debug_wseal_launches": (C.c_int64, []),
+    "mtts_debug_wseal_stats": (C.c_int32, [C.c_void_p, C.c_void_p]),
+    "mtts_k_wseal": (C.c_int32, [C.c_void_p, C.c_int32, C.c_int32, C.c_int32, C.c_void_p, C.c_void_p]),
+    "mtts_k_gemm_sealed": (C.c_int32, [C.c_void_p, C.c_void_p, C.c_void_p] + [C.c_int32] * 7 + [C.c_void_p, C.c_void_p]),
+    "mtts_k_gemm_sealed_bench": (C.c_int32, [C.c_void_p] + [C.c_int32] * 8 + [C.POINTER(C.c_float), C.c_void_p]),
     "mtts_debug_attn_row_launches": (C.c_int64, []),
     "mtts_k_attn_section": (C.c_int32, [C.c_void_p, C.c_int32] + [C.c_void_p] * 4 + [C.c_float] + [C.c_void_p] * 4 +
                             [C.c_int32] * 6 + [C.c_void_p] * 6),
diff --git a/moss-ttsd_amd/mtts/engine.py b/moss-ttsd_amd/mtts/engine.py
--- a/moss-ttsd_amd/mtts/engine.py
+++ b/moss-ttsd_amd/mtts/engine.py
@@ -315,6 +315,12 @@
         capi.check(self.lib.mtts_debug_kv_pack_stats(self._h, o.ctypes.data))
         return dict(zip(("k_pages", "k_unsealed", "v_pages", "v_unsealed", "k_layers_on", "v_layers_on"), (int(x) for x in o)))
 
+    def wseal_stats(self):
+        o = np.zeros(12, dtype=np.int64)
+        capi.check(self.lib.mtts_debug_wseal_stats(self._h, o.ctypes.data))
+        return {k: dict(groups=int(o[3 * i]), unsealed=int(o[3 * i + 1]), on=bool(o[3 * i + 2]))
+                for i, k in enumerate(("gate_up", "down", "head0", "heads17"))}
+
     def debug_set_kv_len(self, n):
         capi.check(self.lib.mtts_debug_set_kv_len(self._h, int(n)))
 
```
